# uma-pi1/kge

Measured on NVIDIA H100. Metric: triples scored/sec 1vsAll ComplEx d=512, higher is better.
Workload: dtype f32 (fp16 hi/lo split products hi*hi + hi*lo + lo*hi on wgmma, fp32 accumulate)

## Files before the change

kge_b200/csrc/capi.cu:

```cuda
#include <cstdarg>
#include <cstdio>
#include <cstring>
#include <cstdlib>
#include "fold.cuh"
#include "tc_common.cuh"

namespace b200kge {

static thread_local char g_err[512] = "";
static thread_local int64_t g_launches = 0;

void set_error(const char* fmt, ...) {
  va_list ap;
  va_start(ap, fmt);
  vsnprintf(g_err, sizeof(g_err), fmt, ap);
  va_end(ap);
}
void count_launch(int n) { g_launches += n; }

int check_cuda(cudaError_t e, const char* what) {
  if (e == cudaSuccess) return 0;
  if (e == cudaErrorMemoryAllocation)
    set_error("CUDA out of memory (%s)", what);
  else
    set_error("CUDA error %d (%s) at %s", (int)e, cudaGetErrorString(e), what);
  return B200KGE_ERR_CUDA;
}

static thread_local int g_prof_on = 0;
static thread_local cudaEvent_t g_ev0 = nullptr, g_ev1 = nullptr;
static thread_local int g_prof_valid = 0;

void profile_begin(cudaStream_t st) {
  if (!g_prof_on) return;
  if (!g_ev0) { cudaEventCreate(&g_ev0); cudaEventCreate(&g_ev1); }
  cudaEventRecord(g_ev0, st);
}
void profile_end(cudaStream_t st) {
  if (!g_prof_on || !g_ev0) return;
  cudaEventRecord(g_ev1, st);
  g_prof_valid = 1;
}

namespace {

struct Arena {
  uint8_t* base;
  size_t cap, off;
  void* take(size_t bytes) {
    size_t a = (off + 255) & ~size_t(255);
    if (a + bytes > cap) return nullptr;
    off = a + bytes;
    return base + a;
  }
};

inline int64_t round_up(int64_t x, int64_t m) { return (x + m - 1) / m * m; }

int validate_model(int model, const Rows& ent_like, const Rows& rel_like) {
  if (model < 0 || model > B200KGE_ROTATE) { set_error("unknown model %d", model); return B200KGE_ERR_INVALID; }
  const int D = ent_like.dim;
  if (D <= 0) { set_error("entity dim must be positive"); return B200KGE_ERR_INVALID; }
  if ((model == B200KGE_COMPLEX || model == B200KGE_SIMPLE || model == B200KGE_CP || model == B200KGE_ROTATE) && (D & 1)) {
    set_error("model %d requires embeddings of even dimensionality (got %d)", model, D);
    return B200KGE_ERR_INVALID;
  }
  const int want = relation_dim(model, D);
  if (rel_like.dim != want) {
    set_error("relation dim %d does not match model %d with entity dim %d (expected %d)", rel_like.dim, model, D, want);
    return B200KGE_ERR_INVALID;
  }
  return 0;
}

int validate_norm(int model, float l_norm) {
  if ((model == B200KGE_TRANSE || model == B200KGE_ROTATE) && !(l_norm > 0.f && l_norm < 1e30f)) {
    set_error("l_norm must be a positive finite number (got %g)", (double)l_norm);
    return B200KGE_ERR_INVALID;
  }
  return 0;
}

int check_tables(int model, float l_norm, const b200kge_rows_t* ent, const b200kge_rows_t* rel) {
  if (!ent || !rel) { set_error("null operand"); return B200KGE_ERR_INVALID; }
  if (ent->idx || rel->idx) { set_error("ent/rel must be plain tables (idx == NULL)"); return B200KGE_ERR_INVALID; }
  int rc = validate_model(model, to_rows(ent), to_rows(rel));
  return rc ? rc : validate_norm(model, l_norm);
}

int check_loss_kind(int loss_kind) {
  if (loss_kind != B200KGE_LOSS_BCE && loss_kind != B200KGE_LOSS_KL) { set_error("unknown loss kind %d", loss_kind); return B200KGE_ERR_INVALID; }
  return 0;
}

int check_grad_ld(const b200kge_rows_t* ent, int64_t lde, const b200kge_rows_t* rel, int64_t ldr) {
  if (lde < ent->dim || ldr < rel->dim) { set_error("gradient leading dimensions are smaller than the table widths"); return B200KGE_ERR_INVALID; }
  return 0;
}

EpiParams empty_epi() {
  EpiParams P;
  memset(&P, 0, sizeof(P));
  return P;
}

bool take_planes(Arena& ws, SplitSet& S) {
  S.hi = ws.take((size_t)S.rows * S.Kp * 2);
  S.lo = ws.take((size_t)S.rows * S.Kp * 2);
  S.inv_scale = (float*)ws.take((size_t)S.rows_pad * 4);
  return S.hi && S.lo && S.inv_scale;
}
size_t planes_bytes(int64_t rows, int64_t rows_pad, int64_t Kp) {
  return 2 * ((size_t)rows * Kp * 2 + 256) + (size_t)rows_pad * 4 + 256;
}

int gemm_planes(const SplitSet& A, const SplitSet& B, float* C, int64_t ldc, cudaStream_t st) {
  EpiParams P = empty_epi();
  P.out = C; P.ldo = ldc;
  if (A.Kp > 512) {
    P.accumulate_out = 1;
    cudaError_t e = cudaMemset2DAsync(C, (size_t)ldc * 4, 0, (size_t)B.rows * 4, (size_t)A.rows, st);
    if (e != cudaSuccess) return check_cuda(e, "cudaMemset2DAsync(gemm output)");
  }
  return launch_pairwise_tc3(EPI_STORE, A, B, P, st);
}

struct Block {
  int model, combine;
  const Rows* q0; const Rows* q1;
  const Rows* p;
  const Rows* cand;
  int64_t n;
  const float* Qpre = nullptr;
  bool same_fold = false;
};

int fold_block(const Block& B, int64_t ldq, Arena& ws, cudaStream_t st, const float** Q) {
  *Q = B.Qpre;
  if (*Q) return 0;
  const int64_t n = B.n;
  float* Qw = (float*)ws.take((size_t)(B.q1 ? 2 * n : n) * ldq * 4);
  if (!Qw) { set_error("workspace too small for folded queries"); return B200KGE_ERR_WORKSPACE; }
  int rc = launch_fold_queries(B.model, B.combine, *B.q0, *B.p, n, 0, Qw, ldq, st);
  if (rc) return rc;
  if (B.q1 && (rc = launch_fold_queries(B.model, B.same_fold ? B.combine : 1 - B.combine, *B.q1, *B.p, n, n, Qw, ldq, st)))
    return rc;
  *Q = Qw;
  return 0;
}

int take_partials(int epi_kind, int64_t nq, int nch, EpiParams& P, Arena& ws, int* nchunks_out, float** part_out) {
  const int loss_epi = epi_loss_base(epi_kind);
  if (loss_epi == EPI_BCE || loss_epi == EPI_KL) {
    const int F = (loss_epi == EPI_BCE) ? 2 : 5;
    P.part = (float*)ws.take((size_t)nq * nch * F * 4);
    if (!P.part) { set_error("workspace too small for loss partials"); return B200KGE_ERR_WORKSPACE; }
    if (part_out) *part_out = P.part;
  }
  P.nchunks = nch;
  if (nchunks_out) *nchunks_out = nch;
  return 0;
}

int run_block(const Block& B, float l_norm, int precision, int epi_kind, EpiParams P, Arena& ws,
              cudaStream_t st, int* nchunks_out, float** part_out = nullptr) {
  const int64_t n = B.n, nq = B.q1 ? 2 * n : n, m = B.cand->rows;
  const int D = B.q0->dim;
  Folded f0 = folded_problem(B.model, B.combine, D, l_norm);
  Folded f1 = f0;
  if (B.q1 && !B.same_fold) f1 = folded_problem(B.model, 1 - B.combine, D, l_norm);
  const bool cols_differ = B.q1 && (f0.col_off != f1.col_off);
  const int K = f0.K;
  const int64_t ldq = round_up(K, 32);

  int tc_kind = 0;
  if (f0.pair_op == PAIR_DOT && precision != B200KGE_PREC_FP32 && !cols_differ) {
    if (precision == B200KGE_PREC_AUTO) {
      if (K >= 32 && K <= 1024 && n >= 16 && m < (1ll << 31)) tc_kind = 3;
    } else if (precision == B200KGE_PREC_F16X3) {
      if (K < 16 || m >= (1ll << 31)) { set_error("the pre-split tensor-core path needs K >= 16"); return B200KGE_ERR_UNSUPPORTED; }
      tc_kind = 3;
    } else {
      if (!tc_supported(f0.pair_op, K, *B.cand, f0.col_off)) { set_error("tensor-core path needs K>=32, 16-byte aligned tables with ld%%4==0"); return B200KGE_ERR_UNSUPPORTED; }
      tc_kind = 1;
    }
  } else if (precision != B200KGE_PREC_AUTO && precision != B200KGE_PREC_FP32) {
    if (f0.pair_op != PAIR_DOT) { set_error("tensor-core precision modes apply to dot-product scorers only"); return B200KGE_ERR_UNSUPPORTED; }
  }

  if (epi_kind == EPI_RANK_EVAL) {
    if (B.cand->idx || tc_kind == 1) {
      set_error("the evaluation ranking runs on the pre-split tensor-core or the CUDA-core kernel over a plain table");
      return B200KGE_ERR_UNSUPPORTED;
    }
  } else if (P.csr_off && (cols_differ || B.cand->idx || tc_kind == 1 || (tc_kind == 0 && epi_kind != EPI_RANK))) {
    set_error("this CSR side input is not consumed by the kernel serving this call (losses: pre-split tensor-core path; "
              "rank: that path or the CUDA-core kernel; plain candidate table)");
    return B200KGE_ERR_UNSUPPORTED;
  }

  if (cols_differ) {
    Block h0 = B; h0.q1 = nullptr;
    Block h1 = B; h1.q0 = B.q1; h1.q1 = nullptr; h1.combine = 1 - B.combine;
    EpiParams P0 = P, P1 = P;
    P0.n_rows_out = 0; P1.n_rows_out = 0;
    if (epi_kind == EPI_STORE) { P1.out = P.out + P.col_block; }
    else if (epi_kind == EPI_RANK_EVAL) {
      P1.true_score += n; P1.csr_skip += n; P1.csr_off += n; P1.own_score += n; P1.rank += n; P1.ties += n;
      if (P1.csr2_off) P1.csr2_off += n;
    }
    else { set_error("stacked fused epilogues are not available for CP"); return B200KGE_ERR_UNSUPPORTED; }
    int rc = run_block(h0, l_norm, precision, epi_kind, P0, ws, st, nchunks_out);
    if (rc) return rc;
    return run_block(h1, l_norm, precision, epi_kind, P1, ws, st, nchunks_out);
  }

  const float* Q = nullptr;
  int rc = fold_block(B, ldq, ws, st, &Q);
  if (rc) return rc;
  if (tc_kind == 3) {
    const int Kp = (int)round_up(K, 64);
    SplitSet SQ{Q, ldq, nullptr, 0, nq, nq, K, Kp, nullptr, nullptr, nullptr};
    SplitSet ST{B.cand->base, B.cand->ld, B.cand->idx, f0.col_off, m, m + 32, K, Kp, nullptr, nullptr, nullptr};
    if (!take_planes(ws, SQ) || !take_planes(ws, ST)) {
      set_error("workspace too small for the pre-split operand planes");
      return B200KGE_ERR_WORKSPACE;
    }
    if ((rc = take_partials(epi_kind, nq, tc_nchunks(nq, m), P, ws, nchunks_out, part_out))) return rc;
    if ((rc = launch_presplit(ST, SQ, st))) return rc;
    return launch_pairwise_tc3(epi_kind, SQ, ST, P, st);
  }
  if (tc_kind == 1) {
    const int passes = (precision == B200KGE_PREC_TF32) ? 1 : (precision == B200KGE_PREC_3XTF32 ? 3 : 2);
    const float* T = B.cand->base + f0.col_off;
    int64_t ldt = B.cand->ld;
    if (B.cand->idx) {
      float* G = (float*)ws.take((size_t)m * ldq * 4);
      if (!G) { set_error("workspace too small to gather the candidate subset"); return B200KGE_ERR_WORKSPACE; }
      if ((rc = launch_gather_rows(*B.cand, f0.col_off, K, G, ldq, st))) return rc;
      T = G; ldt = ldq;
    }
    if ((rc = take_partials(epi_kind, nq, tc_nchunks(nq, m), P, ws, nchunks_out, part_out))) return rc;
    return launch_pairwise_tc(epi_kind, passes, Q, ldq, nq, T, ldt, m, K, P, st);
  }
  if ((rc = take_partials(epi_kind, nq, pairwise_simt_nchunks(nq, m), P, ws, nchunks_out, part_out))) return rc;
  return launch_pairwise_simt(epi_kind, f0.pair_op, l_norm, Q, ldq, nq, *B.cand, f0.col_off, K, P, st);
}

int check_1vsN_args(int model, int combine, const b200kge_rows_t* q, const b200kge_rows_t* p,
                    const b200kge_rows_t* cand, int64_t n) {
  if (!q || !p || !cand) { set_error("null operand"); return B200KGE_ERR_INVALID; }
  if (combine != B200KGE_SP_ && combine != B200KGE__PO) {
    set_error("cannot handle combine=%d", combine);
    return B200KGE_ERR_INVALID;
  }
  if (n < 0 || q->rows < n || p->rows < n) { set_error("operand has fewer than n=%lld rows", (long long)n); return B200KGE_ERR_INVALID; }
  if (cand->dim != q->dim) { set_error("candidate dim %d != query entity dim %d", cand->dim, q->dim); return B200KGE_ERR_INVALID; }
  return validate_model(model, to_rows(q), to_rows(p));
}

__global__ void unpack_triples_kernel(const int64_t* __restrict__ tri, int64_t n, int64_t* s, int64_t* p,
                                      int64_t* o, int64_t* labels2n) {
  int64_t i = blockIdx.x * (int64_t)blockDim.x + threadIdx.x;
  if (i < n) {
    const int64_t a = tri[3 * i], b = tri[3 * i + 1], c = tri[3 * i + 2];
    s[i] = a; p[i] = b; o[i] = c;
    labels2n[i] = c;
    labels2n[n + i] = a;
  }
}

int unpack_triples(const int64_t* triples, int64_t n, int64_t* sidx, int64_t* pidx, int64_t* oidx, int64_t* lab,
                   const Rows& E, const Rows& R, Rows& S, Rows& O, Rows& P, cudaStream_t st) {
  unpack_triples_kernel<<<(unsigned)((n + 255) / 256), 256, 0, st>>>(triples, n, sidx, pidx, oidx, lab);
  B2K_LAUNCH_CHECK("unpack_triples_kernel");
  S = E; S.idx = sidx; S.rows = n;
  O = E; O.idx = oidx; O.rows = n;
  P = R; P.idx = pidx; P.rows = n;
  return 0;
}

__global__ void pack_triples_kernel(const int64_t* __restrict__ q, const int64_t* __restrict__ p, int64_t n, int combine,
                                    int64_t* __restrict__ tri) {
  const int64_t i = blockIdx.x * (int64_t)blockDim.x + threadIdx.x;
  if (i >= n) return;
  tri[3 * i + 1] = p[i];
  tri[3 * i + (combine == B200KGE_SP_ ? 0 : 2)] = q[i];
  tri[3 * i + (combine == B200KGE_SP_ ? 2 : 0)] = 0;
}

__global__ void offset_index_kernel(const int64_t* __restrict__ idx, int64_t n, int64_t off, int64_t* __restrict__ out) {
  const int64_t i = blockIdx.x * (int64_t)blockDim.x + threadIdx.x;
  if (i < n) out[i] = idx[i] + off;
}

int check_reciprocal(const b200kge_rows_t* rel, int64_t num_rel) {
  if (num_rel <= 0 || rel->rows != 2 * num_rel) {
    set_error("reciprocal relations need rel->rows == 2 * num_relations (got %lld rows, num_relations %lld)",
              (long long)rel->rows, (long long)num_rel);
    return B200KGE_ERR_INVALID;
  }
  return 0;
}

__global__ void __launch_bounds__(128)
shard_gather_rows_kernel(Rows shard, int64_t lo, const int64_t* __restrict__ idx, float* __restrict__ out, int64_t ldo) {
  const int64_t i = blockIdx.x;
  const int64_t g = idx[i] - lo;
  const bool mine = g >= 0 && g < shard.rows;
  const float* __restrict__ src = shard.base + (mine ? g : 0) * shard.ld;
  float* __restrict__ dst = out + i * ldo;
  for (int k = threadIdx.x; k < shard.dim; k += blockDim.x) dst[k] = mine ? src[k] : 0.f;
}

}
}

using namespace b200kge;

extern "C" {

int b200kge_version(void) { return B200KGE_VERSION; }
const char* b200kge_last_error(void) { return g_err; }
int64_t b200kge_launch_count(int reset) {
  int64_t v = g_launches;
  if (reset) g_launches = 0;
  return v;
}

int b200kge_profile_enable(int on) { g_prof_on = on; g_prof_valid = 0; return 0; }
int b200kge_profile_last_ms(float* ms) {
  if (!ms) { set_error("null operand"); return B200KGE_ERR_INVALID; }
  if (!g_prof_valid) { set_error("no profiled kernel yet"); return B200KGE_ERR_INVALID; }
  B2K_CUDA(cudaEventSynchronize(g_ev1));
  B2K_CUDA(cudaEventElapsedTime(ms, g_ev0, g_ev1));
  return 0;
}

int b200kge_device_ok(void) {
  int dev = 0, major = 0, minor = 0;
  if (cudaGetDevice(&dev) != cudaSuccess ||
      cudaDeviceGetAttribute(&major, cudaDevAttrComputeCapabilityMajor, dev) != cudaSuccess ||
      cudaDeviceGetAttribute(&minor, cudaDevAttrComputeCapabilityMinor, dev) != cudaSuccess) {
    cudaGetLastError();
    set_error("no CUDA device available: libb200kge has no CPU fallback");
    return B200KGE_ERR_NO_DEVICE;
  }
  if (major != 9 || minor != 0) {
    set_error("device compute capability %d.%d is not sm_90 (H100)", major, minor);
    return B200KGE_ERR_NO_DEVICE;
  }
  return 0;
}

size_t b200kge_workspace_bytes(int model, int64_t n, int64_t m, int32_t D, int cand_has_idx) {
  (void)model;
  const int64_t ldq = round_up(D, 32);
  const int64_t nq = 2 * n;
  size_t b = 0;
  b += 2 * ((size_t)nq * ldq * 4 + 256);
  if (cand_has_idx) b += (size_t)m * ldq * 4 + 256;
  int64_t nch = pairwise_simt_nchunks(nq, m);
  if (nch < 320) nch = 320;
  b += (size_t)nq * nch * 5 * 4 + 256;
  b += (size_t)n * 3 * 8 + (size_t)n * 5 * 8 + 4096;
  {
    const int64_t Kp = round_up(D, 64);
    b += 2 * ((size_t)nq * Kp * 2 + 256) + 2 * ((size_t)m * Kp * 2 + 256) + (size_t)(nq + m + 32) * 4 + 512;
  }
  return b + 4096;
}

int b200kge_score_spo(int model, float l_norm, const b200kge_rows_t* s, const b200kge_rows_t* p,
                      const b200kge_rows_t* o, int64_t n, float* out, b200kge_stream_t stream) {
  if (!s || !p || !o || (!out && n > 0)) { set_error("null operand"); return B200KGE_ERR_INVALID; }
  int rc = validate_model(model, to_rows(s), to_rows(p)); if (rc) return rc;
  if ((rc = validate_norm(model, l_norm))) return rc;
  if (s->rows < n || p->rows < n || o->rows < n) { set_error("operand has fewer than n rows"); return B200KGE_ERR_INVALID; }
  return launch_spo(model, l_norm, to_rows(s), to_rows(p), to_rows(o), n, out, 1, (cudaStream_t)stream);
}

int b200kge_score_1vsN(int model, int combine, float l_norm, int precision,
                       const b200kge_rows_t* q, const b200kge_rows_t* p,
                       const b200kge_rows_t* cand, int64_t n, float* out, int64_t ldo,
                       void* workspace, size_t workspace_bytes, b200kge_stream_t stream) {
  int rc = check_1vsN_args(model, combine, q, p, cand, n); if (rc) return rc;
  if ((rc = validate_norm(model, l_norm))) return rc;
  Rows Q = to_rows(q), Pr = to_rows(p), C = to_rows(cand);
  Arena ws{(uint8_t*)workspace, workspace_bytes, 0};
  EpiParams P = empty_epi();
  P.out = out; P.ldo = ldo;
  Block B{model, combine, &Q, nullptr, &Pr, &C, n};
  return run_block(B, l_norm, precision, EPI_STORE, P, ws, (cudaStream_t)stream, nullptr);
}

int b200kge_score_sp_po(int model, float l_norm, int precision, const b200kge_rows_t* s,
                        const b200kge_rows_t* p, const b200kge_rows_t* o,
                        const b200kge_rows_t* cand, int64_t n, float* out, int64_t ldo,
                        void* workspace, size_t workspace_bytes, b200kge_stream_t stream) {
  int rc = check_1vsN_args(model, B200KGE_SP_, s, p, cand, n); if (rc) return rc;
  if ((rc = check_1vsN_args(model, B200KGE__PO, o, p, cand, n))) return rc;
  if ((rc = validate_norm(model, l_norm))) return rc;
  Rows Sr = to_rows(s), Pr = to_rows(p), Or = to_rows(o), C = to_rows(cand);
  Arena ws{(uint8_t*)workspace, workspace_bytes, 0};
  EpiParams P = empty_epi();
  P.out = out; P.ldo = ldo; P.n_rows_out = n; P.col_block = cand->rows;
  Block B{model, B200KGE_SP_, &Sr, &Or, &Pr, &C, n};
  return run_block(B, l_norm, precision, EPI_STORE, P, ws, (cudaStream_t)stream, nullptr);
}

int b200kge_score_sp_po_bcast(int model, float l_norm, int precision, const b200kge_rows_t* s,
                              const b200kge_rows_t* p, const b200kge_rows_t* o, const b200kge_rows_t* cand,
                              int64_t n, float* out, float* const* peer_out, int n_peers, int64_t ldo,
                              int64_t col_block, void* workspace, size_t workspace_bytes,
                              b200kge_stream_t stream) {
  int rc = check_1vsN_args(model, B200KGE_SP_, s, p, cand, n); if (rc) return rc;
  if ((rc = check_1vsN_args(model, B200KGE__PO, o, p, cand, n))) return rc;
  if ((rc = validate_norm(model, l_norm))) return rc;
  if (n_peers < 0 || n_peers > 7 || (n_peers > 0 && !peer_out)) { set_error("0..7 peer buffers"); return B200KGE_ERR_INVALID; }
  if (col_block < cand->rows) { set_error("col_block smaller than the number of candidates"); return B200KGE_ERR_INVALID; }
  Rows Sr = to_rows(s), Pr = to_rows(p), Or = to_rows(o), C = to_rows(cand);
  Arena ws{(uint8_t*)workspace, workspace_bytes, 0};
  EpiParams P = empty_epi();
  P.out = out; P.ldo = ldo; P.n_rows_out = n; P.col_block = col_block;
  P.n_peers = n_peers;
  for (int g = 0; g < n_peers; ++g) P.out_peer[g] = peer_out[g];
  if (model == B200KGE_CP) { set_error("the broadcast store is not offered for CP"); return B200KGE_ERR_UNSUPPORTED; }
  Block B{model, B200KGE_SP_, &Sr, &Or, &Pr, &C, n};
  return run_block(B, l_norm, precision, EPI_STORE, P, ws, (cudaStream_t)stream, nullptr);
}

int b200kge_score_1vsN_loss(int model, int combine, float l_norm, int precision,
                            const b200kge_rows_t* q, const b200kge_rows_t* p,
                            const b200kge_rows_t* cand, int64_t n, const b200kge_labels_t* labels,
                            int loss_kind, float offset, float* loss_out, float* row_loss_out,
                            void* workspace, size_t workspace_bytes, b200kge_stream_t stream) {
  int rc = check_1vsN_args(model, combine, q, p, cand, n); if (rc) return rc;
  if ((rc = validate_norm(model, l_norm))) return rc;
  if (!labels || (!labels->idx) == (!labels->dense)) { set_error("exactly one of labels.idx / labels.dense must be given"); return B200KGE_ERR_INVALID; }
  if ((rc = check_loss_kind(loss_kind))) return rc;
  if (!loss_out) { set_error("loss_out is null"); return B200KGE_ERR_INVALID; }
  cudaStream_t st = (cudaStream_t)stream;
  Rows Q = to_rows(q), Pr = to_rows(p), C = to_rows(cand);
  Arena ws{(uint8_t*)workspace, workspace_bytes, 0};
  EpiParams P = empty_epi();
  P.label_idx = labels->idx; P.label_dense = labels->dense; P.ldl = labels->ldl;
  P.offset = (loss_kind == B200KGE_LOSS_BCE) ? offset : 0.f;
  Block B{model, combine, &Q, nullptr, &Pr, &C, n};
  int nch = 0;
  const int epi = (loss_kind == B200KGE_LOSS_BCE) ? EPI_BCE : EPI_KL;
  float* part = nullptr;
  rc = run_block(B, l_norm, precision, epi, P, ws, st, &nch, &part);
  if (rc) return rc;
  if (n == 0 || C.rows == 0) { B2K_CUDA(cudaMemsetAsync(loss_out, 0, 4, st)); return 0; }
  void* scratch = ws.take(1024);
  if (!scratch) { set_error("workspace too small"); return B200KGE_ERR_WORKSPACE; }
  return launch_loss_finalize(loss_kind, part, nch, n, loss_out, row_loss_out, 1.0f, 0, scratch, 0, st);
}

int b200kge_score_1vsN_rank(int model, int combine, float l_norm, int precision,
                            const b200kge_rows_t* q, const b200kge_rows_t* p,
                            const b200kge_rows_t* cand, int64_t n, const float* true_score,
                            const float* filter, int64_t ldf, float rtol, float atol,
                            int64_t* rank, int64_t* ties, void* workspace, size_t workspace_bytes,
                            b200kge_stream_t stream) {
  int rc = check_1vsN_args(model, combine, q, p, cand, n); if (rc) return rc;
  if ((rc = validate_norm(model, l_norm))) return rc;
  if (!true_score || !rank || !ties) { set_error("null rank operand"); return B200KGE_ERR_INVALID; }
  Rows Q = to_rows(q), Pr = to_rows(p), C = to_rows(cand);
  Arena ws{(uint8_t*)workspace, workspace_bytes, 0};
  EpiParams P = empty_epi();
  P.true_score = true_score; P.filter = filter; P.ldf = ldf; P.rtol = rtol; P.atol = atol;
  P.rank = reinterpret_cast<unsigned long long*>(rank);
  P.ties = reinterpret_cast<unsigned long long*>(ties);
  Block B{model, combine, &Q, nullptr, &Pr, &C, n};
  return run_block(B, l_norm, precision, EPI_RANK, P, ws, (cudaStream_t)stream, nullptr);
}

int b200kge_rank_sp_po(int model, float l_norm, int precision, const b200kge_rows_t* s,
                       const b200kge_rows_t* p, const b200kge_rows_t* o, const b200kge_rows_t* cand,
                       int64_t n, const float* true_score, const float* filter, int64_t ldf, float rtol,
                       float atol, int64_t* rank, int64_t* ties, void* workspace, size_t workspace_bytes,
                       b200kge_stream_t stream) {
  int rc = check_1vsN_args(model, B200KGE_SP_, s, p, cand, n); if (rc) return rc;
  if ((rc = check_1vsN_args(model, B200KGE__PO, o, p, cand, n))) return rc;
  if ((rc = validate_norm(model, l_norm))) return rc;
  if (!true_score || !rank || !ties) { set_error("null rank operand"); return B200KGE_ERR_INVALID; }
  Rows Sr = to_rows(s), Pr = to_rows(p), Or = to_rows(o), C = to_rows(cand);
  Arena ws{(uint8_t*)workspace, workspace_bytes, 0};
  EpiParams P = empty_epi();
  P.true_score = true_score; P.filter = filter; P.ldf = ldf; P.rtol = rtol; P.atol = atol;
  P.rank = reinterpret_cast<unsigned long long*>(rank);
  P.ties = reinterpret_cast<unsigned long long*>(ties);
  Block B{model, B200KGE_SP_, &Sr, &Or, &Pr, &C, n};
  return run_block(B, l_norm, precision, EPI_RANK, P, ws, (cudaStream_t)stream, nullptr);
}

int b200kge_rank_sp_po_csr(int model, float l_norm, int precision, const b200kge_rows_t* s,
                           const b200kge_rows_t* p, const b200kge_rows_t* o, const b200kge_rows_t* cand,
                           int64_t n, const float* true_score, const int64_t* filter_off,
                           const int64_t* filter_col, const int64_t* own_col, float rtol, float atol,
                           int64_t* rank, int64_t* ties, void* workspace, size_t workspace_bytes,
                           b200kge_stream_t stream) {
  int rc = check_1vsN_args(model, B200KGE_SP_, s, p, cand, n); if (rc) return rc;
  if ((rc = check_1vsN_args(model, B200KGE__PO, o, p, cand, n))) return rc;
  if ((rc = validate_norm(model, l_norm))) return rc;
  if (!true_score || !rank || !ties || !filter_off) { set_error("null rank operand"); return B200KGE_ERR_INVALID; }
  Rows Sr = to_rows(s), Pr = to_rows(p), Or = to_rows(o), C = to_rows(cand);
  Arena ws{(uint8_t*)workspace, workspace_bytes, 0};
  EpiParams P = empty_epi();
  P.true_score = true_score; P.rtol = rtol; P.atol = atol;
  P.rank = reinterpret_cast<unsigned long long*>(rank);
  P.ties = reinterpret_cast<unsigned long long*>(ties);
  P.csr_off = filter_off; P.csr_col = filter_col; P.csr_skip = own_col;
  Block B{model, B200KGE_SP_, &Sr, &Or, &Pr, &C, n};
  return run_block(B, l_norm, precision, EPI_RANK, P, ws, (cudaStream_t)stream, nullptr);
}

int b200kge_rank_sp_po_eval(int model, float l_norm, int precision, const b200kge_rows_t* ent,
                            const b200kge_rows_t* rel, int64_t num_relations, const int64_t* s, const int64_t* p,
                            const int64_t* o, int64_t n, const float* true_score, const int64_t* own_col,
                            const int64_t* filter_off, const int64_t* filter_col, const int64_t* test_off,
                            const int64_t* test_col, float rtol, float atol, int64_t* rank, int64_t* ties,
                            float* own_score, void* workspace, size_t workspace_bytes, b200kge_stream_t stream) {
  if (!s || !p || !o || !true_score || !own_col || !filter_off || !rank || !ties || !own_score) {
    set_error("null rank operand");
    return B200KGE_ERR_INVALID;
  }
  if (n < 0) { set_error("negative batch size"); return B200KGE_ERR_INVALID; }
  if (num_relations < 0) { set_error("num_relations must be >= 0"); return B200KGE_ERR_INVALID; }
  int rc = check_tables(model, l_norm, ent, rel); if (rc) return rc;
  if (num_relations > 0 && (rc = check_reciprocal(rel, num_relations))) return rc;
  if (precision == B200KGE_PREC_TF32 || precision == B200KGE_PREC_3XTF32 || precision == B200KGE_PREC_TF32_BF16X2) {
    set_error("the evaluation ranking does not run the in-kernel split precision modes");
    return B200KGE_ERR_UNSUPPORTED;
  }
  if (n == 0) return 0;
  cudaStream_t st = (cudaStream_t)stream;
  const Rows E = to_rows(ent), R = to_rows(rel);
  Rows S = E, O = E, Pr = R;
  S.idx = s; S.rows = n; O.idx = o; O.rows = n; Pr.idx = p; Pr.rows = n;
  Arena ws{(uint8_t*)workspace, workspace_bytes, 0};
  EpiParams P = empty_epi();
  P.true_score = true_score; P.rtol = rtol; P.atol = atol;
  P.rank = reinterpret_cast<unsigned long long*>(rank);
  P.ties = reinterpret_cast<unsigned long long*>(ties);
  P.csr_off = filter_off; P.csr_col = filter_col; P.csr_skip = own_col;
  P.csr2_off = test_off; P.csr2_col = test_col;
  P.rank_ld = 2 * n; P.n_rank = test_off ? 3 : 2;
  P.own_score = own_score;
  Block B{model, B200KGE_SP_, &S, &O, &Pr, &E, n};
  if (num_relations > 0) {
    const Folded f = folded_problem(model, B200KGE_SP_, E.dim, l_norm);
    const int64_t ldq = round_up(f.K, 32);
    float* Q = (float*)ws.take((size_t)2 * n * ldq * 4);
    int64_t* p2 = (int64_t*)ws.take((size_t)n * 8);
    if (!Q || !p2) { set_error("workspace too small for folded queries"); return B200KGE_ERR_WORKSPACE; }
    offset_index_kernel<<<(unsigned)((n + 255) / 256), 256, 0, st>>>(p, n, num_relations, p2);
    B2K_LAUNCH_CHECK("offset_index_kernel");
    Rows P2 = R; P2.idx = p2; P2.rows = n;
    if ((rc = launch_fold_queries(model, B200KGE_SP_, S, Pr, n, 0, Q, ldq, st))) return rc;
    if ((rc = launch_fold_queries(model, B200KGE_SP_, O, P2, n, n, Q, ldq, st))) return rc;
    B.Qpre = Q;
    B.same_fold = true;
  }
  return run_block(B, l_norm, precision, EPI_RANK_EVAL, P, ws, st, nullptr);
}

int b200kge_shard_gather_rows(const b200kge_rows_t* shard, int64_t lo, const int64_t* idx, int64_t n,
                              float* out, int64_t ldo, b200kge_stream_t stream) {
  if (!shard || (!idx && n > 0) || (!out && n > 0)) { set_error("null operand"); return B200KGE_ERR_INVALID; }
  if (shard->idx) { set_error("shard must be a plain table (idx == NULL)"); return B200KGE_ERR_INVALID; }
  if (ldo < shard->dim) { set_error("output row stride smaller than the row width"); return B200KGE_ERR_INVALID; }
  if (n <= 0) return 0;
  shard_gather_rows_kernel<<<(unsigned)n, 128, 0, (cudaStream_t)stream>>>(to_rows(shard), lo, idx, out, ldo);
  B2K_LAUNCH_CHECK("shard_gather_rows_kernel");
  return 0;
}

int b200kge_loss_dense(const float* scores, int64_t lds, int64_t n, int64_t m,
                       const b200kge_labels_t* labels, int loss_kind, float offset,
                       float* loss_out, float* row_loss_out, void* workspace,
                       size_t workspace_bytes, b200kge_stream_t stream) {
  if (!scores || !labels || !loss_out) { set_error("null operand"); return B200KGE_ERR_INVALID; }
  if ((!labels->idx) == (!labels->dense)) { set_error("exactly one of labels.idx / labels.dense must be given"); return B200KGE_ERR_INVALID; }
  if (loss_kind >= B200KGE_LOSS_BCE_MEAN && loss_kind <= B200KGE_LOSS_SE) { set_error("loss kind %d is row-wise with one positive per row: use b200kge_ns_loss", loss_kind); return B200KGE_ERR_UNSUPPORTED; }
  int rc = check_loss_kind(loss_kind); if (rc) return rc;
  cudaStream_t st = (cudaStream_t)stream;
  if (n == 0 || m == 0) { B2K_CUDA(cudaMemsetAsync(loss_out, 0, 4, st)); return 0; }
  Arena ws{(uint8_t*)workspace, workspace_bytes, 0};
  const int nch = loss_dense_nchunks(m);
  const int F = (loss_kind == B200KGE_LOSS_BCE) ? 2 : 5;
  EpiParams P = empty_epi();
  P.label_idx = labels->idx; P.label_dense = labels->dense; P.ldl = labels->ldl;
  P.offset = (loss_kind == B200KGE_LOSS_BCE) ? offset : 0.f;
  P.nchunks = nch;
  P.part = (float*)ws.take((size_t)n * nch * F * 4);
  if (!P.part) { set_error("workspace too small for loss partials (need %zu bytes)", (size_t)n * nch * F * 4); return B200KGE_ERR_WORKSPACE; }
  void* scratch = ws.take(1024);
  if (!scratch) { set_error("workspace too small"); return B200KGE_ERR_WORKSPACE; }
  if ((rc = launch_loss_dense(loss_kind, scores, lds, n, m, P, st))) return rc;
  return launch_loss_finalize(loss_kind, P.part, nch, n, loss_out, row_loss_out, 1.0f, 0, scratch, 0, st);
}

int b200kge_rank_dense(const float* scores, int64_t lds, int64_t n, int64_t m,
                       const float* true_score, const float* filter, int64_t ldf, float rtol,
                       float atol, int64_t* rank, int64_t* ties, b200kge_stream_t stream) {
  if (!scores || !true_score || !rank || !ties) { set_error("null operand"); return B200KGE_ERR_INVALID; }
  EpiParams P = empty_epi();
  P.true_score = true_score; P.filter = filter; P.ldf = ldf; P.rtol = rtol; P.atol = atol;
  P.rank = reinterpret_cast<unsigned long long*>(rank);
  P.ties = reinterpret_cast<unsigned long long*>(ties);
  return launch_rank_dense(scores, lds, n, m, P, (cudaStream_t)stream);
}

int b200kge_ns_score(int model, float l_norm, const b200kge_rows_t* s, const b200kge_rows_t* p,
                     const b200kge_rows_t* o, const b200kge_rows_t* slot_table, int slot,
                     const int64_t* neg, int64_t n, int64_t K, int with_positive, float* out,
                     int64_t ldo, b200kge_stream_t stream) {
  if (n == 0 || (K == 0 && !with_positive)) return 0;
  if (!s || !p || !o || !slot_table || (!neg && n * K > 0) || !out) { set_error("null operand"); return B200KGE_ERR_INVALID; }
  if (slot < 0 || slot > 2) { set_error("slot must be 0 (S), 1 (P) or 2 (O)"); return B200KGE_ERR_INVALID; }
  int rc = validate_model(model, to_rows(s), to_rows(p)); if (rc) return rc;
  if ((rc = validate_norm(model, l_norm))) return rc;
  if (slot_table->idx) { set_error("slot_table must be a plain table (idx == NULL)"); return B200KGE_ERR_INVALID; }
  if (slot_table->dim != (slot == 1 ? p->dim : s->dim)) { set_error("slot_table width does not match the slot"); return B200KGE_ERR_INVALID; }
  cudaStream_t st = (cudaStream_t)stream;
  const int col0 = with_positive ? 1 : 0;
  if (with_positive) {
    rc = launch_spo(model, l_norm, to_rows(s), to_rows(p), to_rows(o), n, out, ldo, st);
    if (rc) return rc;
  }
  return launch_ns(model, l_norm, to_rows(s), to_rows(p), to_rows(o), to_rows(slot_table), slot, neg, n, K,
                   out, ldo, col0, st);
}

int b200kge_sample_uniform(uint64_t seed, uint64_t offset, int64_t vocab, int64_t n, int64_t K, int64_t* out,
                           b200kge_stream_t stream) {
  if (vocab <= 0) { set_error("vocabulary size must be positive"); return B200KGE_ERR_INVALID; }
  if (n < 0 || K < 0 || (!out && n * K > 0)) { set_error("null operand"); return B200KGE_ERR_INVALID; }
  return launch_sample_uniform(seed, offset, vocab, n * K, out, (cudaStream_t)stream);
}

static int train_1vsall_forward_impl(int model, float l_norm, int precision,
                                     const b200kge_rows_t* ent, const b200kge_rows_t* rel,
                                     const int64_t* triples, int64_t n, int loss_kind, float offset,
                                     float* loss_out, void* workspace, size_t workspace_bytes,
                                     b200kge_stream_t stream, int64_t num_rel) {
  if (!triples || !loss_out) { set_error("null operand"); return B200KGE_ERR_INVALID; }
  int rc = check_tables(model, l_norm, ent, rel); if (rc) return rc;
  if ((rc = check_loss_kind(loss_kind))) return rc;
  cudaStream_t st = (cudaStream_t)stream;
  if (n <= 0) { B2K_CUDA(cudaMemsetAsync(loss_out, 0, 4, st)); return 0; }
  Arena ws{(uint8_t*)workspace, workspace_bytes, 0};
  Rows E = to_rows(ent), R = to_rows(rel);
  const int epi = (loss_kind == B200KGE_LOSS_BCE) ? EPI_BCE : EPI_KL;
  const float scale = 1.0f / (float)n;
  Folded f0 = folded_problem(model, B200KGE_SP_, E.dim, l_norm),
         f1 = folded_problem(model, num_rel > 0 ? B200KGE_SP_ : B200KGE__PO, E.dim, l_norm);
  const int K = f0.K;
  const bool presplit = f0.col_off == f1.col_off && f0.pair_op == PAIR_DOT && (model != B200KGE_CP || num_rel > 0) &&
                        (precision == B200KGE_PREC_AUTO || precision == B200KGE_PREC_F16X3) && K >= 32 && K <= 1024 &&
                        n >= 16 && E.rows < (1ll << 31) &&
                        ((size_t)round_up(K, 64) + (model == B200KGE_RESCAL ? E.dim : 0)) * 4 <= 48 * 1024;
  if (presplit) {
    const int64_t nq = 2 * n, m = E.rows;
    const int Kp = (int)round_up(K, 64);
    SplitSet SQ{nullptr, 0, nullptr, 0, nq, nq, K, Kp, nullptr, nullptr, nullptr};
    SplitSet ST{E.base, E.ld, nullptr, f0.col_off, m, m + 32, K, Kp, nullptr, nullptr, nullptr};
    const bool planes = take_planes(ws, SQ) && take_planes(ws, ST);
    int64_t* lab = (int64_t*)ws.take((size_t)n * 2 * 8);
    uint8_t* scratch = (uint8_t*)ws.take(1024);
    const int nch = tc_nchunks(nq, m);
    const int F = (loss_kind == B200KGE_LOSS_BCE) ? 2 : 5;
    float* part = (float*)ws.take((size_t)nq * nch * F * 4);
    if (!planes || !lab || !scratch || !part) { set_error("workspace too small"); return B200KGE_ERR_WORKSPACE; }
    unsigned int* ticket = reinterpret_cast<unsigned int*>(scratch + 512);
    if ((rc = launch_prep_split_1vsall(model, E, R, triples, n, SQ, ST, lab, ticket, st, num_rel))) return rc;
    EpiParams P = empty_epi();
    P.label_idx = lab;
    P.offset = (loss_kind == B200KGE_LOSS_BCE) ? offset : 0.f;
    P.part = part; P.nchunks = nch;
    if ((rc = launch_pairwise_tc3(epi, SQ, ST, P, st))) return rc;
    return launch_loss_finalize(loss_kind, part, nch, nq, loss_out, nullptr, scale, 0, scratch, 1, st);
  }
  if (f0.col_off == f1.col_off) {
    const int64_t ldq = round_up(f0.K, 32);
    float* Q = (float*)ws.take((size_t)(2 * n) * ldq * 4);
    int64_t* lab = (int64_t*)ws.take((size_t)n * 2 * 8);
    uint8_t* scratch = (uint8_t*)ws.take(1024);
    if (!Q || !lab || !scratch) { set_error("workspace too small"); return B200KGE_ERR_WORKSPACE; }
    rc = launch_prep_1vsall(model, E, R, triples, n, Q, ldq, lab, reinterpret_cast<unsigned int*>(scratch + 512), st,
                            num_rel);
    if (rc) return rc;
    Rows S = E; S.idx = lab; S.rows = n;
    Rows Pr = R; Pr.idx = lab; Pr.rows = n;
    EpiParams P = empty_epi();
    P.label_idx = lab;
    P.offset = (loss_kind == B200KGE_LOSS_BCE) ? offset : 0.f;
    Block B{model, B200KGE_SP_, &S, &S, &Pr, &E, n};
    B.Qpre = Q;
    B.same_fold = num_rel > 0;
    int nch = 0;
    float* part = nullptr;
    rc = run_block(B, l_norm, precision, epi, P, ws, st, &nch, &part);
    if (rc) return rc;
    return launch_loss_finalize(loss_kind, part, nch, 2 * n, loss_out, nullptr, scale, 0, scratch, 1, st);
  }
  int64_t* sidx = (int64_t*)ws.take((size_t)n * 8);
  int64_t* pidx = (int64_t*)ws.take((size_t)n * 8);
  int64_t* oidx = (int64_t*)ws.take((size_t)n * 8);
  int64_t* lab = (int64_t*)ws.take((size_t)n * 2 * 8);
  if (!sidx || !pidx || !oidx || !lab) { set_error("workspace too small"); return B200KGE_ERR_WORKSPACE; }
  Rows S, O, Pr;
  if ((rc = unpack_triples(triples, n, sidx, pidx, oidx, lab, E, R, S, O, Pr, st))) return rc;
  EpiParams P = empty_epi();
  P.label_idx = lab;
  P.offset = (loss_kind == B200KGE_LOSS_BCE) ? offset : 0.f;
  for (int dir = 0; dir < 2; ++dir) {
    Arena w2 = ws;
    EpiParams Pd = P;
    Pd.label_idx = lab + dir * n;
    Block B{model, dir, dir == 0 ? &S : &O, nullptr, &Pr, &E, n};
    int nch = 0;
    float* part = nullptr;
    rc = run_block(B, l_norm, precision, epi, Pd, w2, st, &nch, &part);
    if (rc) return rc;
    void* scratch = w2.take(1024);
    if (!scratch) { set_error("workspace too small"); return B200KGE_ERR_WORKSPACE; }
    rc = launch_loss_finalize(loss_kind, part, nch, n, loss_out, nullptr, scale, dir, scratch, 0, st);
    if (rc) return rc;
  }
  return 0;
}

int b200kge_train_1vsall_forward(int model, float l_norm, int precision,
                                 const b200kge_rows_t* ent, const b200kge_rows_t* rel,
                                 const int64_t* triples, int64_t n, int loss_kind, float offset,
                                 float* loss_out, void* workspace, size_t workspace_bytes,
                                 b200kge_stream_t stream) {
  return train_1vsall_forward_impl(model, l_norm, precision, ent, rel, triples, n, loss_kind, offset, loss_out,
                                   workspace, workspace_bytes, stream, 0);
}

int b200kge_train_1vsall_forward_host(int model, float l_norm, int precision,
                                      const b200kge_rows_t* ent, const b200kge_rows_t* rel,
                                      const int64_t* triples_host, int64_t n, int loss_kind,
                                      float offset, float* loss_host, void* workspace,
                                      size_t workspace_bytes, b200kge_stream_t stream) {
  if (!triples_host || !loss_host) { set_error("null operand"); return B200KGE_ERR_INVALID; }
  if (n <= 0) { *loss_host = 0.f; return 0; }
  cudaStream_t st = (cudaStream_t)stream;
  Arena ws{(uint8_t*)workspace, workspace_bytes, 0};
  int64_t* tri = (int64_t*)ws.take((size_t)n * 3 * 8);
  float* loss_dev = (float*)ws.take(256);
  if (!tri || !loss_dev) { set_error("workspace too small"); return B200KGE_ERR_WORKSPACE; }
  B2K_CUDA(cudaMemcpyAsync(tri, triples_host, (size_t)n * 3 * 8, cudaMemcpyHostToDevice, st));
  size_t used = (ws.off + 255) & ~size_t(255);
  int rc = b200kge_train_1vsall_forward(model, l_norm, precision, ent, rel, tri, n, loss_kind, offset, loss_dev,
                                        ws.base + used, workspace_bytes - used, stream);
  if (rc) return rc;
  B2K_CUDA(cudaMemcpyAsync(loss_host, loss_dev, 4, cudaMemcpyDeviceToHost, st));
  B2K_CUDA(cudaStreamSynchronize(st));
  return 0;
}

}

namespace {

struct GradSpec {
  const int64_t* lab = nullptr;
  int loss_kind = B200KGE_LOSS_BCE;
  float offset = 0.f;
  const int64_t* csr_off = nullptr;
  const int64_t* csr_col = nullptr;
  float csr_a = 1.f, csr_b = 0.f, inv_batch = 0.f;
  const float* G = nullptr;
  int64_t ldg = 0;
};

GradSpec csr_grad(const int64_t* q_idx, const int64_t* csr_off, const int64_t* csr_col, float label_smoothing, int64_t m,
                  int64_t batch_size, int loss_kind, float offset) {
  GradSpec g;
  g.lab = q_idx;
  g.loss_kind = loss_kind; g.offset = offset;
  g.csr_off = csr_off; g.csr_col = csr_col;
  g.csr_a = 1.0f - label_smoothing; g.csr_b = label_smoothing > 0.f ? 1.0f / (float)m : 0.f;
  g.inv_batch = 1.0f / (float)batch_size;
  return g;
}

int backward_block(int model, const Rows& E, const Rows& R, int64_t n, int dir, bool same_fold, const float* Q,
                   int64_t ldq, int col_off, int K, const GradSpec& g, float* d_ent, int64_t lde, float* dQ, Arena ws,
                   cudaStream_t st) {
  const int64_t nq = dir < 0 ? 2 * n : n, m = E.rows;
  const int64_t ldz = round_up(m, 4), Ep = round_up(m, 64), Np = round_up(nq, 64);
  const int64_t ldE = round_up(m, 4), ldN = round_up(nq, 4);
  int rc;
  SplitSet SG{nullptr, 0, nullptr, 0, nq, nq, (int)m, (int)Ep, nullptr, nullptr, nullptr};
  SplitSet SGT{nullptr, 0, nullptr, 0, m, m, (int)nq, (int)Np, nullptr, nullptr, nullptr};
  if (g.G) {
    float* Gt = (float*)ws.take((size_t)m * ldN * 4);
    if (!Gt) { set_error("workspace too small for the transposed gradient"); return B200KGE_ERR_WORKSPACE; }
    if ((rc = launch_transpose(g.G, g.ldg, nq, m, Gt, ldN, st))) return rc;
    SG.src = g.G; SG.ld = g.ldg;
    SGT.src = Gt; SGT.ld = ldN;
    if (!take_planes(ws, SG) || !take_planes(ws, SGT)) { set_error("workspace too small for the gradient planes"); return B200KGE_ERR_WORKSPACE; }
    if ((rc = launch_presplit(SGT, SG, st))) return rc;
  } else {
    float* z = (float*)ws.take((size_t)nq * ldz * 4);
    if (!z) { set_error("workspace too small for the score matrix"); return B200KGE_ERR_WORKSPACE; }
    {
      Rows S = E; S.idx = g.lab; S.rows = n;
      Rows Pr = R; Pr.idx = g.lab; Pr.rows = n;
      EpiParams P = empty_epi();
      P.out = z; P.ldo = ldz;
      Block B{model, dir <= 0 ? B200KGE_SP_ : B200KGE__PO, &S, dir < 0 ? &S : nullptr, &Pr, &E, n};
      B.Qpre = Q;
      B.same_fold = same_fold;
      if ((rc = run_block(B, 1.0f, B200KGE_PREC_AUTO, EPI_STORE, P, ws, st, nullptr))) return rc;
    }
    if (!take_planes(ws, SG) || !take_planes(ws, SGT)) { set_error("workspace too small for the gradient planes"); return B200KGE_ERR_WORKSPACE; }
    float* row_stat = nullptr;
    if (g.loss_kind == B200KGE_LOSS_KL) {
      row_stat = (float*)ws.take((size_t)nq * 2 * 4);
      if (!row_stat) { set_error("workspace too small for the row statistics"); return B200KGE_ERR_WORKSPACE; }
    }
    const float off = g.loss_kind == B200KGE_LOSS_KL ? 0.f : g.offset;
    if (g.csr_off)
      rc = launch_grad_planes_csr(z, ldz, nq, m, g.csr_off, g.csr_col, g.csr_a, g.csr_b, row_stat, off, g.inv_batch,
                                  SG.hi, SG.lo, Ep, SGT.hi, SGT.lo, Np, SG.inv_scale, SGT.inv_scale, st);
    else
      rc = launch_grad_planes(z, ldz, nq, m, g.lab, nullptr, 0, row_stat, off, 1.0f / (float)n, SG.hi, SG.lo, Ep,
                              SGT.hi, SGT.lo, Np, SG.inv_scale, SGT.inv_scale, st);
    if (rc) return rc;
  }
  float* Tt = (float*)ws.take((size_t)K * ldE * 4);
  float* Qt = (float*)ws.take((size_t)K * ldN * 4);
  if (!Tt || !Qt) { set_error("workspace too small for the transposed operands"); return B200KGE_ERR_WORKSPACE; }
  if ((rc = launch_transpose(E.base + col_off, E.ld, m, K, Tt, ldE, st))) return rc;
  if ((rc = launch_transpose(Q, ldq, nq, K, Qt, ldN, st))) return rc;
  SplitSet STt{Tt, ldE, nullptr, 0, K, K + 32, (int)m, (int)Ep, nullptr, nullptr, nullptr};
  SplitSet SQt{Qt, ldN, nullptr, 0, K, K + 32, (int)nq, (int)Np, nullptr, nullptr, nullptr};
  if (!take_planes(ws, STt) || !take_planes(ws, SQt)) { set_error("workspace too small for the operand planes"); return B200KGE_ERR_WORKSPACE; }
  if ((rc = launch_presplit(STt, SQt, st))) return rc;
  if ((rc = gemm_planes(SGT, SQt, d_ent + col_off, lde, st))) return rc;
  return gemm_planes(SG, STt, dQ, ldq, st);
}

int distance_rowgrads(int pair_op, const float* Q, int64_t ldq, int64_t nq, const Rows& T, int K, const float* W,
                      int64_t ldw, float* Wt, float* dQ, float* dT, int64_t ldt, cudaStream_t st) {
  const int64_t m = T.rows, ldN = round_up(nq, 4);
  int rc;
  if ((rc = launch_transpose(W, ldw, nq, m, Wt, ldN, st))) return rc;
  if ((rc = launch_pair_rowgrad(pair_op, Q, ldq, nq, T.base, T.ld, m, K, Wt, ldN, dQ, ldq, st))) return rc;
  return launch_pair_rowgrad(pair_op, T.base, T.ld, m, Q, ldq, nq, K, W, ldw, dT, ldt, st);
}

int distance_backward(const Block& B, float l_norm, const GradSpec& g, float* dQ, float* dT, int64_t ldt, Arena& ws,
                      cudaStream_t st) {
  const Folded f = folded_problem(B.model, B.combine, B.cand->dim, l_norm);
  const int64_t nq = B.q1 ? 2 * B.n : B.n, m = B.cand->rows, ldz = round_up(m, 4), ldN = round_up(nq, 4);
  const bool kl = g.loss_kind == B200KGE_LOSS_KL;
  float* z = (float*)ws.take((size_t)nq * ldz * 4);
  float* G = (float*)ws.take((size_t)nq * ldz * 4);
  float* Gt = (float*)ws.take((size_t)m * ldN * 4);
  float* row_stat = kl ? (float*)ws.take((size_t)nq * 2 * 4) : nullptr;
  if (!z || !G || !Gt || (kl && !row_stat)) { set_error("workspace too small"); return B200KGE_ERR_WORKSPACE; }
  EpiParams P = empty_epi();
  P.out = z; P.ldo = ldz;
  int rc;
  if ((rc = run_block(B, l_norm, B200KGE_PREC_AUTO, EPI_STORE, P, ws, st, nullptr))) return rc;
  const int64_t* lab = g.csr_off ? nullptr : g.lab;
  if (kl && (rc = launch_row_lse(z, ldz, nq, m, lab, row_stat, st))) return rc;
  if (g.csr_off)
    rc = launch_grad_csr(z, ldz, nq, m, g.csr_off, g.csr_col, g.csr_a, g.csr_b, row_stat, kl ? 0.f : g.offset,
                         g.inv_batch, f.pair_op == PAIR_L2, G, ldz, st);
  else
    rc = launch_grad_dense(z, ldz, nq, m, g.lab, row_stat, kl ? 0.f : g.offset, 1.0f / (float)B.n,
                           f.pair_op == PAIR_L2, G, ldz, st);
  if (rc) return rc;
  return distance_rowgrads(f.pair_op, B.Qpre, round_up(f.K, 32), nq, *B.cand, f.K, G, ldz, Gt, dQ, dT, ldt, st);
}

int check_distance_pair(int pair_op) {
  if (pair_op != PAIR_L1 && pair_op != PAIR_L2 && pair_op != PAIR_CMOD_L1) {
    set_error("the distance-family backward covers l_norm 1 and 2 (TransE) and 1 (RotatE)");
    return B200KGE_ERR_UNSUPPORTED;
  }
  return 0;
}

size_t backward_block_bytes(int64_t nq, int64_t m, int64_t K, int64_t ldq) {
  const int64_t Ep = round_up(m, 64), Np = round_up(nq, 64);
  size_t b = (size_t)nq * round_up(m, 4) * 4 + 256;
  b += b200kge_workspace_bytes(0, nq, m, (int32_t)K, 0);
  b += planes_bytes(nq, nq, Ep) + planes_bytes(m, m, Np);
  b += (size_t)K * round_up(m, 4) * 4 + (size_t)K * round_up(nq, 4) * 4 + 2 * (size_t)nq * ldq * 4 + (size_t)nq * 8 + 5 * 256;
  b += planes_bytes(K, K + 32, Ep) + planes_bytes(K, K + 32, Np);
  return b;
}

}

extern "C" {

size_t b200kge_gemm_nt_workspace_bytes(int64_t M, int64_t N, int64_t K) {
  const int64_t Kp = round_up(K, 64);
  return planes_bytes(M, M, Kp) + planes_bytes(N, N + 32, Kp) + 1024;
}

int b200kge_gemm_nt(const float* A, int64_t lda, const float* B, int64_t ldb, int64_t M, int64_t N, int64_t K,
                      float* C, int64_t ldc, void* workspace, size_t workspace_bytes, b200kge_stream_t stream) {
  if (!A || !B || !C) { set_error("null operand"); return B200KGE_ERR_INVALID; }
  if (M < 0 || N < 0 || K <= 0 || N >= (1ll << 31)) { set_error("bad GEMM shape"); return B200KGE_ERR_INVALID; }
  if (M == 0 || N == 0) return 0;
  cudaStream_t st = (cudaStream_t)stream;
  Arena ws{(uint8_t*)workspace, workspace_bytes, 0};
  const int Kp = (int)round_up(K, 64);
  SplitSet SA{A, lda, nullptr, 0, M, M, (int)K, Kp, nullptr, nullptr, nullptr};
  SplitSet SB{B, ldb, nullptr, 0, N, N + 32, (int)K, Kp, nullptr, nullptr, nullptr};
  if (!take_planes(ws, SA) || !take_planes(ws, SB)) { set_error("workspace too small for the operand planes"); return B200KGE_ERR_WORKSPACE; }
  int rc = launch_presplit(SB, SA, st);
  if (rc) return rc;
  return gemm_planes(SA, SB, C, ldc, st);
}

size_t b200kge_train_1vsall_backward_workspace_bytes(int model, int64_t n, int64_t E, int32_t D) {
  const int64_t K = (model == B200KGE_CP) ? D / 2 : D;
  const int64_t nq = 2 * n, ldq = round_up(K, 32);
  if (model == B200KGE_TRANSE || model == B200KGE_ROTATE)
    return 2 * (size_t)nq * ldq * 4 + (size_t)nq * 8 + 2 * (size_t)nq * round_up(E, 4) * 4 + 2 * (size_t)E * round_up(nq, 4) * 4 +
           (size_t)nq * 8 + 16 * 256 + b200kge_workspace_bytes(model, n, E, D, 0);
  return (size_t)nq * ldq * 4 + (size_t)n * 5 * 8 + 4096 + backward_block_bytes(nq, E, K, ldq);
}

static int train_1vsall_backward_impl(int model, float l_norm, const b200kge_rows_t* ent, const b200kge_rows_t* rel,
                                      const int64_t* triples, int64_t n, int loss_kind, float offset, float* d_ent,
                                      int64_t lde, float* d_rel, int64_t ldr, void* workspace, size_t workspace_bytes,
                                      b200kge_stream_t stream, int64_t num_rel) {
  if (!triples || !d_ent || !d_rel) { set_error("null operand"); return B200KGE_ERR_INVALID; }
  int rc = check_tables(model, l_norm, ent, rel); if (rc) return rc;
  if ((rc = check_loss_kind(loss_kind))) return rc;
  if ((rc = check_grad_ld(ent, lde, rel, ldr))) return rc;
  cudaStream_t st = (cudaStream_t)stream;
  Rows E = to_rows(ent), R = to_rows(rel);
  B2K_CUDA(cudaMemsetAsync(d_rel, 0, (size_t)R.rows * ldr * 4, st));
  if (n <= 0) { B2K_CUDA(cudaMemsetAsync(d_ent, 0, (size_t)E.rows * lde * 4, st)); return 0; }
  Arena ws{(uint8_t*)workspace, workspace_bytes, 0};
  if (model == B200KGE_TRANSE || model == B200KGE_ROTATE) {
    Folded f = folded_problem(model, B200KGE_SP_, E.dim, l_norm);
    if ((rc = check_distance_pair(f.pair_op))) return rc;
    const int64_t nq = 2 * n, ldq = round_up(f.K, 32);
    float* Q = (float*)ws.take((size_t)nq * ldq * 4);
    float* dQ = (float*)ws.take((size_t)nq * ldq * 4);
    int64_t* lab = (int64_t*)ws.take((size_t)nq * 8);
    if (!Q || !dQ || !lab) { set_error("workspace too small"); return B200KGE_ERR_WORKSPACE; }
    if ((rc = launch_prep_1vsall(model, E, R, triples, n, Q, ldq, lab, nullptr, st, num_rel))) return rc;
    Rows S = E; S.idx = lab; S.rows = n;
    Rows Pr = R; Pr.idx = lab; Pr.rows = n;
    Block B{model, B200KGE_SP_, &S, &S, &Pr, &E, n};
    B.Qpre = Q;
    B.same_fold = num_rel > 0;
    GradSpec g;
    g.lab = lab; g.loss_kind = loss_kind; g.offset = offset;
    if ((rc = distance_backward(B, l_norm, g, dQ, d_ent, lde, ws, st))) return rc;
    return launch_unfold_distance(model, E, R, triples, n, -1, dQ, ldq, d_ent, lde, d_rel, ldr, st, num_rel);
  }
  Folded f0 = folded_problem(model, B200KGE_SP_, E.dim, 1.0f),
         f1 = folded_problem(model, num_rel > 0 ? B200KGE_SP_ : B200KGE__PO, E.dim, 1.0f);
  const int64_t ldq = round_up(f0.K, 32);
  GradSpec g;
  g.loss_kind = loss_kind; g.offset = offset;
  if (f0.col_off == f1.col_off) {
    float* Q = (float*)ws.take((size_t)(2 * n) * ldq * 4);
    int64_t* lab = (int64_t*)ws.take((size_t)n * 2 * 8);
    if (!Q || !lab) { set_error("workspace too small"); return B200KGE_ERR_WORKSPACE; }
    float* dQ = (float*)ws.take((size_t)(2 * n) * ldq * 4);
    if (!dQ) { set_error("workspace too small"); return B200KGE_ERR_WORKSPACE; }
    if ((rc = launch_prep_1vsall(model, E, R, triples, n, Q, ldq, lab, nullptr, st, num_rel))) return rc;
    if (f0.col_off > 0) B2K_CUDA(cudaMemset2DAsync(d_ent, (size_t)lde * 4, 0, (size_t)f0.col_off * 4, (size_t)E.rows, st));
    g.lab = lab;
    if ((rc = backward_block(model, E, R, n, -1, num_rel > 0, Q, ldq, f0.col_off, f0.K, g, d_ent, lde, dQ, ws, st))) return rc;
    return launch_unfold(model, E, R, triples, n, -1, dQ, ldq, d_ent, lde, d_rel, ldr, st, num_rel);
  }
  int64_t* sidx = (int64_t*)ws.take((size_t)n * 8);
  int64_t* pidx = (int64_t*)ws.take((size_t)n * 8);
  int64_t* oidx = (int64_t*)ws.take((size_t)n * 8);
  int64_t* lab = (int64_t*)ws.take((size_t)n * 2 * 8);
  float* Q = (float*)ws.take((size_t)n * ldq * 4);
  float* dQ2 = (float*)ws.take((size_t)(2 * n) * ldq * 4);
  if (!sidx || !pidx || !oidx || !lab || !Q || !dQ2) { set_error("workspace too small"); return B200KGE_ERR_WORKSPACE; }
  Rows S, O, Pr;
  if ((rc = unpack_triples(triples, n, sidx, pidx, oidx, lab, E, R, S, O, Pr, st))) return rc;
  for (int dir = 0; dir < 2; ++dir) {
    const Folded& f = dir == 0 ? f0 : f1;
    if ((rc = launch_fold_queries(model, dir, dir == 0 ? S : O, Pr, n, 0, Q, ldq, st))) return rc;
    g.lab = lab + dir * n;
    if ((rc = backward_block(model, E, R, n, dir, false, Q, ldq, f.col_off, f.K, g, d_ent, lde,
                             dQ2 + (size_t)dir * n * ldq, ws, st))) return rc;
  }
  for (int dir = 0; dir < 2; ++dir)
    if ((rc = launch_unfold(model, E, R, triples, n, dir, dQ2 + (size_t)dir * n * ldq, ldq, d_ent, lde, d_rel, ldr, st))) return rc;
  return 0;
}

int b200kge_train_1vsall_backward(int model, float l_norm, const b200kge_rows_t* ent, const b200kge_rows_t* rel,
                                    const int64_t* triples, int64_t n, int loss_kind, float offset, float* d_ent,
                                    int64_t lde, float* d_rel, int64_t ldr, void* workspace, size_t workspace_bytes,
                                    b200kge_stream_t stream) {
  return train_1vsall_backward_impl(model, l_norm, ent, rel, triples, n, loss_kind, offset, d_ent, lde, d_rel, ldr,
                                    workspace, workspace_bytes, stream, 0);
}


size_t b200kge_score_1vsN_backward_workspace_bytes(int model, int64_t n, int64_t E, int32_t D) {
  const int64_t K = (model == B200KGE_CP) ? D / 2 : D;
  const int64_t ldq = round_up(K, 32);
  if (model == B200KGE_TRANSE || model == B200KGE_ROTATE)
    return 2 * (size_t)n * ldq * 4 + (size_t)n * 4 * 8 + 2 * (size_t)n * round_up(E, 4) * 4 + (size_t)E * round_up(n, 4) * 4 +
           16 * 256 + b200kge_workspace_bytes(model, n, E, D, 0);
  return 2 * (size_t)n * ldq * 4 + (size_t)n * 4 * 8 + (size_t)E * round_up(n, 4) * 4 + 8192 + backward_block_bytes(n, E, K, ldq);
}

int b200kge_score_1vsN_backward(int model, int combine, float l_norm, const b200kge_rows_t* ent, const b200kge_rows_t* rel,
                                const int64_t* q_idx, const int64_t* p_idx, int64_t n, const float* grad_scores,
                                int64_t ldg, float* d_ent, int64_t lde, float* d_rel, int64_t ldr, void* workspace,
                                size_t workspace_bytes, b200kge_stream_t stream) {
  if (!q_idx || !p_idx || !grad_scores || !d_ent || !d_rel) { set_error("null operand"); return B200KGE_ERR_INVALID; }
  if (combine != B200KGE_SP_ && combine != B200KGE__PO) { set_error("cannot handle combine=%d", combine); return B200KGE_ERR_INVALID; }
  int rc = check_tables(model, l_norm, ent, rel); if (rc) return rc;
  if ((rc = check_grad_ld(ent, lde, rel, ldr))) return rc;
  if (ldg < ent->rows) { set_error("grad_scores is narrower than the entity table"); return B200KGE_ERR_INVALID; }
  const bool distance = (model == B200KGE_TRANSE || model == B200KGE_ROTATE);
  cudaStream_t st = (cudaStream_t)stream;
  Rows E = to_rows(ent), R = to_rows(rel);
  Folded f = folded_problem(model, combine, E.dim, l_norm);
  if (distance && (rc = check_distance_pair(f.pair_op))) return rc;
  B2K_CUDA(cudaMemsetAsync(d_rel, 0, (size_t)R.rows * ldr * 4, st));
  B2K_CUDA(cudaMemsetAsync(d_ent, 0, (size_t)E.rows * lde * 4, st));
  if (n <= 0) return 0;
  Arena ws{(uint8_t*)workspace, workspace_bytes, 0};
  const int64_t ldq = round_up(f.K, 32);
  float* Q = (float*)ws.take((size_t)n * ldq * 4);
  float* dQ = (float*)ws.take((size_t)n * ldq * 4);
  int64_t* tri = (int64_t*)ws.take((size_t)n * 3 * 8);
  if (!Q || !dQ || !tri) { set_error("workspace too small"); return B200KGE_ERR_WORKSPACE; }
  pack_triples_kernel<<<(unsigned)((n + 255) / 256), 256, 0, st>>>(q_idx, p_idx, n, combine, tri);
  B2K_LAUNCH_CHECK("pack_triples_kernel");
  Rows A = E; A.idx = q_idx; A.rows = n;
  Rows Pr = R; Pr.idx = p_idx; Pr.rows = n;
  if ((rc = launch_fold_queries(model, combine, A, Pr, n, 0, Q, ldq, st))) return rc;
  if (distance) {
    const int64_t m = E.rows, ldz = round_up(m, 4), ldN = round_up(n, 4);
    const float* W = grad_scores;
    int64_t ldw = ldg;
    if (f.pair_op == PAIR_L2) {
      float* z = (float*)ws.take((size_t)n * ldz * 4);
      float* Wd = (float*)ws.take((size_t)n * ldz * 4);
      if (!z || !Wd) { set_error("workspace too small"); return B200KGE_ERR_WORKSPACE; }
      EpiParams P = empty_epi();
      P.out = z; P.ldo = ldz;
      Block B{model, combine, &A, nullptr, &Pr, &E, n};
      B.Qpre = Q;
      if ((rc = run_block(B, l_norm, B200KGE_PREC_AUTO, EPI_STORE, P, ws, st, nullptr))) return rc;
      if ((rc = launch_div_scores(grad_scores, ldg, z, ldz, n, m, Wd, ldz, st))) return rc;
      W = Wd; ldw = ldz;
    }
    float* Wt = (float*)ws.take((size_t)m * ldN * 4);
    if (!Wt) { set_error("workspace too small"); return B200KGE_ERR_WORKSPACE; }
    if ((rc = distance_rowgrads(f.pair_op, Q, ldq, n, E, f.K, W, ldw, Wt, dQ, d_ent, lde, st))) return rc;
    return launch_unfold_distance(model, E, R, tri, n, combine, dQ, ldq, d_ent, lde, d_rel, ldr, st);
  }
  GradSpec g;
  g.G = grad_scores; g.ldg = ldg;
  if ((rc = backward_block(model, E, R, n, combine, false, Q, ldq, f.col_off, f.K, g, d_ent, lde, dQ, ws, st))) return rc;
  return launch_unfold(model, E, R, tri, n, combine, dQ, ldq, d_ent, lde, d_rel, ldr, st);
}

int b200kge_score_1vsN_loss_csr_backward_norm(int model, int combine, float l_norm, const b200kge_rows_t* ent,
                                              const b200kge_rows_t* rel, const int64_t* q_idx, const int64_t* p_idx,
                                              int64_t n, const int64_t* csr_off, const int64_t* csr_col,
                                              float label_smoothing, int loss_kind, float offset, int64_t batch_size,
                                              float* d_ent, int64_t lde, float* d_rel, int64_t ldr, void* workspace,
                                              size_t workspace_bytes, b200kge_stream_t stream) {
  if (!q_idx || !p_idx || !csr_off || !d_ent || !d_rel) { set_error("null operand"); return B200KGE_ERR_INVALID; }
  if (combine != B200KGE_SP_ && combine != B200KGE__PO) { set_error("cannot handle combine=%d", combine); return B200KGE_ERR_INVALID; }
  int rc = check_tables(model, l_norm, ent, rel); if (rc) return rc;
  const bool distance = (model == B200KGE_TRANSE || model == B200KGE_ROTATE);
  Folded f = folded_problem(model, combine, ent->dim, distance ? l_norm : 1.0f);
  if (distance && (rc = check_distance_pair(f.pair_op))) return rc;
  if ((rc = check_loss_kind(loss_kind))) return rc;
  if (batch_size <= 0 || !(label_smoothing >= 0.f && label_smoothing < 1.f)) { set_error("bad batch_size / label_smoothing"); return B200KGE_ERR_INVALID; }
  if ((rc = check_grad_ld(ent, lde, rel, ldr))) return rc;
  cudaStream_t st = (cudaStream_t)stream;
  Rows E = to_rows(ent), R = to_rows(rel);
  B2K_CUDA(cudaMemsetAsync(d_rel, 0, (size_t)R.rows * ldr * 4, st));
  B2K_CUDA(cudaMemsetAsync(d_ent, 0, (size_t)E.rows * lde * 4, st));
  if (n <= 0) return 0;
  Arena ws{(uint8_t*)workspace, workspace_bytes, 0};
  const int64_t ldq = round_up(f.K, 32);
  float* Q = (float*)ws.take((size_t)n * ldq * 4);
  float* dQ = (float*)ws.take((size_t)n * ldq * 4);
  int64_t* tri = (int64_t*)ws.take((size_t)n * 3 * 8);
  if (!Q || !dQ || !tri) { set_error("workspace too small"); return B200KGE_ERR_WORKSPACE; }
  pack_triples_kernel<<<(unsigned)((n + 255) / 256), 256, 0, st>>>(q_idx, p_idx, n, combine, tri);
  B2K_LAUNCH_CHECK("pack_triples_kernel");
  Rows A = E; A.idx = q_idx; A.rows = n;
  Rows Pr = R; Pr.idx = p_idx; Pr.rows = n;
  if ((rc = launch_fold_queries(model, combine, A, Pr, n, 0, Q, ldq, st))) return rc;
  const GradSpec g = csr_grad(q_idx, csr_off, csr_col, label_smoothing, E.rows, batch_size, loss_kind, offset);
  if (distance) {
    Block B{model, combine, &A, nullptr, &Pr, &E, n};
    B.Qpre = Q;
    if ((rc = distance_backward(B, l_norm, g, dQ, d_ent, lde, ws, st))) return rc;
    return launch_unfold_distance(model, E, R, tri, n, combine, dQ, ldq, d_ent, lde, d_rel, ldr, st);
  }
  if ((rc = backward_block(model, E, R, n, combine, false, Q, ldq, f.col_off, f.K, g, d_ent, lde, dQ, ws, st))) return rc;
  return launch_unfold(model, E, R, tri, n, combine, dQ, ldq, d_ent, lde, d_rel, ldr, st);
}

int b200kge_score_1vsN_loss_csr_backward(int model, int combine, const b200kge_rows_t* ent, const b200kge_rows_t* rel,
                                         const int64_t* q_idx, const int64_t* p_idx, int64_t n, const int64_t* csr_off,
                                         const int64_t* csr_col, float label_smoothing, int loss_kind, float offset,
                                         int64_t batch_size, float* d_ent, int64_t lde, float* d_rel, int64_t ldr,
                                         void* workspace, size_t workspace_bytes, b200kge_stream_t stream) {
  return b200kge_score_1vsN_loss_csr_backward_norm(model, combine, 1.0f, ent, rel, q_idx, p_idx, n, csr_off, csr_col,
                                                   label_smoothing, loss_kind, offset, batch_size, d_ent, lde, d_rel,
                                                   ldr, workspace, workspace_bytes, stream);
}

int b200kge_lookup_penalty(const b200kge_rows_t* rows, const float* counts, float p, int complex_abs, float scale,
                             float* out, void* workspace, size_t workspace_bytes, b200kge_stream_t stream) {
  if (!rows || !out) { set_error("null operand"); return B200KGE_ERR_INVALID; }
  if (!(p > 0.f)) { set_error("p must be positive (got %g)", (double)p); return B200KGE_ERR_INVALID; }
  if (complex_abs && (rows->dim & 1)) { set_error("complex-space penalty needs an even embedding width"); return B200KGE_ERR_INVALID; }
  return launch_penalty(to_rows(rows), counts, p, complex_abs, scale, (float*)workspace, workspace_bytes / 4, out,
                        (cudaStream_t)stream);
}

int b200kge_normalize_rows(float* weight, int64_t ld, int64_t rows, int32_t dim, float p, b200kge_stream_t stream) {
  if (!weight && rows > 0) { set_error("null operand"); return B200KGE_ERR_INVALID; }
  return launch_normalize_rows(weight, ld, rows, dim, p, (cudaStream_t)stream);
}


int b200kge_ns_backward(int model, float l_norm, const b200kge_rows_t* ent, const b200kge_rows_t* rel,
                          const int64_t* triples, int slot, const int64_t* neg, int64_t n, int64_t K, float offset,
                          int64_t batch_size, float* d_ent, int64_t lde, float* d_rel, int64_t ldr, void* workspace,
                          size_t workspace_bytes, b200kge_stream_t stream) {
  if (!triples || (!neg && n * K > 0) || !d_ent || !d_rel) { set_error("null operand"); return B200KGE_ERR_INVALID; }
  int rc = check_tables(model, l_norm, ent, rel); if (rc) return rc;
  if (batch_size <= 0) { set_error("batch_size must be positive"); return B200KGE_ERR_INVALID; }
  if ((rc = check_grad_ld(ent, lde, rel, ldr))) return rc;
  Rows E = to_rows(ent), R = to_rows(rel);
  Folded f = folded_problem(model, B200KGE_SP_, E.dim, l_norm);
  const int64_t ldq = round_up(f.K, 32);
  Arena ws{(uint8_t*)workspace, workspace_bytes, 0};
  float* dQ = (float*)ws.take((size_t)n * ldq * 4);
  if (!dQ && n > 0) { set_error("workspace too small (need n * round_up(K,32) floats)"); return B200KGE_ERR_WORKSPACE; }
  return launch_ns_backward(model, l_norm, E, R, triples, slot, neg, n, K, offset, 1.0f / (float)batch_size, nullptr, 0,
                            d_ent, lde, d_rel, ldr, dQ, ldq, (cudaStream_t)stream);
}

int b200kge_ns_backward_grad(int model, float l_norm, const b200kge_rows_t* ent, const b200kge_rows_t* rel,
                             const int64_t* triples, int slot, const int64_t* neg, int64_t n, int64_t K,
                             const float* grad_scores, int64_t ldg, float* d_ent, int64_t lde, float* d_rel,
                             int64_t ldr, void* workspace, size_t workspace_bytes, b200kge_stream_t stream) {
  if (!triples || (!neg && n * K > 0) || (!grad_scores && n > 0) || !d_ent || !d_rel) { set_error("null operand"); return B200KGE_ERR_INVALID; }
  int rc = check_tables(model, l_norm, ent, rel); if (rc) return rc;
  if (ldg < K + 1) { set_error("grad_scores is narrower than the 1 + K columns of the block"); return B200KGE_ERR_INVALID; }
  if ((rc = check_grad_ld(ent, lde, rel, ldr))) return rc;
  Rows E = to_rows(ent), R = to_rows(rel);
  Folded f = folded_problem(model, B200KGE_SP_, E.dim, l_norm);
  const int64_t ldq = round_up(f.K, 32);
  Arena ws{(uint8_t*)workspace, workspace_bytes, 0};
  float* dQ = (float*)ws.take((size_t)n * ldq * 4);
  if (!dQ && n > 0) { set_error("workspace too small (need n * round_up(K,32) floats)"); return B200KGE_ERR_WORKSPACE; }
  return launch_ns_backward(model, l_norm, E, R, triples, slot, neg, n, K, 0.f, 1.f, grad_scores, ldg, d_ent, lde,
                            d_rel, ldr, dQ, ldq, (cudaStream_t)stream);
}

size_t b200kge_ns_loss_workspace_bytes(int64_t n) { return (size_t)n * 2 * 4 + 256 + 1024; }

int b200kge_ns_loss(const float* scores, int64_t lds, int64_t n, int64_t m, const int64_t* label_idx,
                    int loss_kind, float arg, float temperature, float scale, float* loss_out,
                    float* row_loss_out, float* grad_out, int64_t ldg, void* workspace,
                    size_t workspace_bytes, b200kge_stream_t stream) {
  if ((!scores && n * m > 0) || !loss_out) { set_error("null operand"); return B200KGE_ERR_INVALID; }
  if (loss_kind < B200KGE_LOSS_BCE || loss_kind > B200KGE_LOSS_SE) { set_error("unknown loss kind %d", loss_kind); return B200KGE_ERR_INVALID; }
  if (n > 0 && m < (loss_kind >= B200KGE_LOSS_BCE_MEAN && loss_kind <= B200KGE_LOSS_MARGIN_RANKING ? 2 : 1)) {
    set_error("loss kind %d needs a positive and at least one negative per row (m = %lld)", loss_kind, (long long)m);
    return B200KGE_ERR_INVALID;
  }
  if (lds < m || (grad_out && ldg < m)) { set_error("row stride smaller than the row width"); return B200KGE_ERR_INVALID; }
  cudaStream_t st = (cudaStream_t)stream;
  if (n == 0) { B2K_CUDA(cudaMemsetAsync(loss_out, 0, 4, st)); return 0; }
  Arena ws{(uint8_t*)workspace, workspace_bytes, 0};
  float* part = (float*)ws.take((size_t)n * 2 * 4);
  void* scratch = ws.take(1024);
  if (!part || !scratch) { set_error("workspace too small (need b200kge_ns_loss_workspace_bytes(n) = %zu bytes)", b200kge_ns_loss_workspace_bytes(n)); return B200KGE_ERR_WORKSPACE; }
  int rc = launch_ns_loss(loss_kind, scores, lds, n, m, label_idx, arg, temperature, scale, part, grad_out, ldg, st);
  if (rc) return rc;
  return launch_loss_finalize(B200KGE_LOSS_BCE, part, 1, n, loss_out, row_loss_out, scale, 0, scratch, 0, st);
}


size_t b200kge_score_1vsN_loss_csr_workspace_bytes(int model, int64_t n, int64_t m, int32_t D, int64_t nnz) {
  const int64_t ldq = round_up(D, 32), tot = nnz + n;
  size_t b = b200kge_workspace_bytes(model, n, m, D, 0);
  b += (size_t)n * 8 + 3 * ((size_t)tot * 8 + 256) + (size_t)tot * 4 + 4 * ((size_t)n * 4 + 256) + 2048;
  b += (size_t)n * ldq * 4 + ((size_t)((m + 1023) / 1024) + 1) * ldq * 4 + 512;
  if (model == B200KGE_TRANSE || model == B200KGE_ROTATE)
    b += (size_t)n * pairwise_simt_nchunks(n, m) * 4 + 256;
  return b;
}

int b200kge_score_1vsN_loss_csr(int model, int combine, float l_norm, int precision, const b200kge_rows_t* q,
                                  const b200kge_rows_t* p, const b200kge_rows_t* cand, int64_t n,
                                  const int64_t* csr_off, const int64_t* csr_col, int64_t nnz, float label_smoothing,
                                  int loss_kind, float offset, float* loss_out, float* row_loss_out, void* workspace,
                                  size_t workspace_bytes, b200kge_stream_t stream) {
  int rc = check_1vsN_args(model, combine, q, p, cand, n); if (rc) return rc;
  if ((rc = validate_norm(model, l_norm))) return rc;
  if (!csr_off || (!csr_col && nnz > 0) || !loss_out || nnz < 0) { set_error("null operand"); return B200KGE_ERR_INVALID; }
  if (cand->idx) { set_error("CSR labels address the columns of a plain candidate table (cand.idx must be NULL)"); return B200KGE_ERR_INVALID; }
  if ((rc = check_loss_kind(loss_kind))) return rc;
  if (!(label_smoothing >= 0.f && label_smoothing < 1.f)) { set_error("label_smoothing must be in [0, 1)"); return B200KGE_ERR_INVALID; }
  const bool dot = model <= B200KGE_RESCAL;
  cudaStream_t st = (cudaStream_t)stream;
  if (n == 0 || cand->rows == 0) { B2K_CUDA(cudaMemsetAsync(loss_out, 0, 4, st)); return 0; }
  Rows Q = to_rows(q), Pr = to_rows(p), C = to_rows(cand);
  const int64_t m = C.rows, tot = nnz + (loss_kind == B200KGE_LOSS_KL ? n : 0);
  Arena ws{(uint8_t*)workspace, workspace_bytes, 0};
  int64_t* lab = (int64_t*)ws.take((size_t)n * 8);
  int64_t* qsel = (int64_t*)ws.take((size_t)tot * 8 + 8);
  int64_t* psel = (int64_t*)ws.take((size_t)tot * 8 + 8);
  int64_t* esel = (int64_t*)ws.take((size_t)tot * 8 + 8);
  float* zpos = (float*)ws.take((size_t)tot * 4 + 8);
  float* fused = (float*)ws.take((size_t)n * 4);
  float* rows = row_loss_out ? row_loss_out : (float*)ws.take((size_t)n * 4);
  float* total = (float*)ws.take(256);
  void* scratch = ws.take(1024);
  const bool zsum_fused = label_smoothing > 0.f && !dot;
  const int zch = zsum_fused ? pairwise_simt_nchunks(n, m) : 1;
  float* zsum = zsum_fused ? (float*)ws.take((size_t)n * zch * 4) : nullptr;
  if (!lab || !qsel || !psel || !esel || !zpos || !fused || !rows || !total || !scratch || (zsum_fused && !zsum)) { set_error("workspace too small"); return B200KGE_ERR_WORKSPACE; }
  B2K_CUDA(cudaMemsetAsync(lab, loss_kind == B200KGE_LOSS_BCE ? 0xFF : 0, (size_t)n * 8, st));
  bool emitted = false;
  {
    const int epi = (loss_kind == B200KGE_LOSS_BCE) ? (zsum_fused ? EPI_BCE_ZSUM : EPI_BCE)
                                                    : (zsum_fused ? EPI_KL_ZSUM : EPI_KL);
    for (int attempt = 0; attempt < 2; ++attempt) {
      EpiParams P = empty_epi();
      P.label_idx = lab;
      P.offset = (loss_kind == B200KGE_LOSS_BCE) ? offset : 0.f;
      P.zsum_part = zsum;
      if (attempt == 0) {
        P.csr_off = csr_off; P.csr_col = csr_col; P.csr_out = zpos; P.csr_nnz = nnz;
        P.csr_extra = (loss_kind == B200KGE_LOSS_KL) ? 1 : 0;
      }
      Block B{model, combine, &Q, nullptr, &Pr, &C, n};
      int nch = 0;
      float* part = nullptr;
      Arena w2 = ws;
      rc = run_block(B, l_norm, precision, epi, P, w2, st, &nch, &part);
      if (rc == B200KGE_ERR_UNSUPPORTED && attempt == 0) continue;
      if (rc) return rc;
      emitted = (attempt == 0);
      if ((rc = launch_loss_finalize(loss_kind, part, nch, n, total, fused, 1.0f, 0, scratch, 0, st))) return rc;
      break;
    }
  }
  if (!emitted) {
    if ((rc = launch_csr_expand(csr_off, csr_col, n, nnz, loss_kind == B200KGE_LOSS_KL ? 1 : 0, Q.idx, Pr.idx, qsel, psel,
                                esel, st))) return rc;
    if (tot > 0) {
      Rows Qs = Q; Qs.idx = qsel; Qs.rows = tot;
      Rows Ps = Pr; Ps.idx = psel; Ps.rows = tot;
      Rows Es = C; Es.idx = esel; Es.rows = tot;
      if (combine == B200KGE_SP_) rc = launch_spo(model, l_norm, Qs, Ps, Es, tot, zpos, 1, st);
      else                        rc = launch_spo(model, l_norm, Es, Ps, Qs, tot, zpos, 1, st);
      if (rc) return rc;
    }
  }
  if (label_smoothing > 0.f && dot) {
    Folded f = folded_problem(model, combine, Q.dim, l_norm);
    const int64_t ldq = round_up(f.K, 32);
    float* Qf = (float*)ws.take((size_t)n * ldq * 4);
    float* cs = (float*)ws.take(((size_t)((m + 1023) / 1024) + 1) * ldq * 4);
    zsum = (float*)ws.take((size_t)n * 4);
    if (!Qf || !cs || !zsum) { set_error("workspace too small"); return B200KGE_ERR_WORKSPACE; }
    if ((rc = launch_fold_queries(model, combine, Q, Pr, n, 0, Qf, ldq, st))) return rc;
    if ((rc = launch_row_score_sums(Qf, ldq, n, C.base + f.col_off, C.ld, m, f.K, cs, zsum, st))) return rc;
  }
  const float a = 1.0f - label_smoothing, b = label_smoothing > 0.f ? 1.0f / (float)m : 0.f;
  if ((rc = launch_csr_rows(loss_kind, csr_off, csr_col, zpos, n, nnz, fused, zsum, zch, a, b, (float)m,
                            loss_kind == B200KGE_LOSS_BCE ? offset : 0.f, rows, st))) return rc;
  return launch_rows_sum(rows, n, 1.0f, loss_out, st);
}

}

namespace {

int validate_dropout(const b200kge_dropout_t* d, int64_t n, int64_t E, int D, int Dr) {
  if (!d) { set_error("null dropout key"); return B200KGE_ERR_INVALID; }
  if (!(d->p_ent >= 0.f && d->p_ent < 1.f) || !(d->p_rel >= 0.f && d->p_rel < 1.f)) {
    set_error("dropout rates must lie in [0, 1) (got %g, %g)", (double)d->p_ent, (double)d->p_rel);
    return B200KGE_ERR_INVALID;
  }
  const double lim = 281474976710656.0;
  if (d->row_base < 0 || (double)(d->row_base + n) * D > lim || (double)(d->row_base + n) * Dr > lim ||
      (double)E * D > lim) {
    set_error("dropout rows out of range: row_base >= 0 and row * dim + k < 2^48 are required");
    return B200KGE_ERR_INVALID;
  }
  return 0;
}

DropMask drop_mask(float p, uint64_t seed, uint64_t call, int stream, int64_t row_base) {
  DropMask m;
  m.seed = seed; m.call = call; m.stream = stream; m.row_base = row_base;
  m.thresh = (uint64_t)floor((1.0 - (double)p) * 4294967296.0);
  m.scale = (float)(1.0 / (1.0 - (double)p));
  return m;
}

struct DirMasks { DropMask q, r, t; };
DirMasks dir_masks(const b200kge_dropout_t& d, int dir) {
  DirMasks m;
  m.q = drop_mask(d.p_ent, d.seed, d.call, dir == 0 ? B200KGE_DROP_SP_ENT : B200KGE_DROP_PO_ENT, d.row_base);
  m.r = drop_mask(d.p_rel, d.seed, d.call, dir == 0 ? B200KGE_DROP_SP_REL : B200KGE_DROP_PO_REL, d.row_base);
  m.t = drop_mask(d.p_ent, d.seed, d.call, dir == 0 ? B200KGE_DROP_SP_TABLE : B200KGE_DROP_PO_TABLE, 0);
  return m;
}

struct MaskedOps { float *Qm, *Pm, *Tm; };
bool take_masked(Arena& ws, int64_t n, int64_t E, int D, int Dr, MaskedOps& o) {
  o.Qm = (float*)ws.take((size_t)n * D * 4);
  o.Pm = (float*)ws.take((size_t)n * Dr * 4);
  o.Tm = (float*)ws.take((size_t)E * D * 4);
  return o.Qm && o.Pm && o.Tm;
}
int gather_masked(const DirMasks& m, const Rows& E, const Rows& R, const int64_t* q_idx, const int64_t* p_idx, int64_t n,
                  const MaskedOps& o, Rows& Qr, Rows& Pr, Rows& Tr, cudaStream_t st) {
  Rows qs = E; qs.idx = q_idx; qs.rows = n;
  Rows ps = R; ps.idx = p_idx; ps.rows = n;
  Rows ts = E; ts.idx = nullptr;
  int rc;
  if ((rc = launch_dropout_gather(m.q, qs, o.Qm, E.dim, st))) return rc;
  if ((rc = launch_dropout_gather(m.r, ps, o.Pm, R.dim, st))) return rc;
  if ((rc = launch_dropout_gather(m.t, ts, o.Tm, E.dim, st))) return rc;
  Qr = Rows{o.Qm, nullptr, n, E.dim, E.dim};
  Pr = Rows{o.Pm, nullptr, n, R.dim, R.dim};
  Tr = Rows{o.Tm, nullptr, E.rows, E.dim, E.dim};
  return 0;
}

size_t masked_bytes(int model, int64_t n, int64_t E, int32_t D) {
  const int64_t Dr = relation_dim(model, D), ldq = round_up(D, 32);
  return 2 * ((size_t)E * D * 4 + 256)
         + 2 * ((size_t)n * D * 4 + (size_t)n * Dr * 4 + 512)
         + 2 * ((size_t)n * ldq * 4 + 256)
         + (size_t)n * 10 * 8 + 5 * 256
         + (size_t)n * 2 * 4 + 4096;
}

struct BackBufs { MaskedOps o; float *Q, *dQ, *dT, *dQe, *dPr; int64_t* tri; };
bool take_back(Arena& ws, int64_t n, int64_t E, int D, int Dr, int64_t ldq, BackBufs& b) {
  if (!take_masked(ws, n, E, D, Dr, b.o)) return false;
  b.Q = (float*)ws.take((size_t)n * ldq * 4);
  b.dQ = (float*)ws.take((size_t)n * ldq * 4);
  b.dT = (float*)ws.take((size_t)E * D * 4);
  b.dQe = (float*)ws.take((size_t)n * D * 4);
  b.dPr = (float*)ws.take((size_t)n * Dr * 4);
  b.tri = (int64_t*)ws.take((size_t)n * 3 * 8);
  return b.Q && b.dQ && b.dT && b.dQe && b.dPr && b.tri;
}

int dropout_backward_dir(int model, float l_norm, int dir, int mask_dir, const Rows& E, const Rows& R, const int64_t* q_idx,
                         const int64_t* p_idx, int64_t n, const b200kge_dropout_t& d, const GradSpec& g,
                         const BackBufs& b, Arena ws, float* d_ent, int64_t lde, float* d_rel, int64_t ldr, cudaStream_t st) {
  const DirMasks m = dir_masks(d, mask_dir);
  const Folded f = folded_problem(model, dir, E.dim, l_norm);
  const int64_t ldq = round_up(f.K, 32), mE = E.rows;
  const int D = E.dim, Dr = R.dim;
  Rows Qr, Pr, Tr;
  int rc = gather_masked(m, E, R, q_idx, p_idx, n, b.o, Qr, Pr, Tr, st);
  if (rc) return rc;
  if ((rc = launch_fold_queries(model, dir, Qr, Pr, n, 0, b.Q, ldq, st))) return rc;
  B2K_CUDA(cudaMemsetAsync(b.dQe, 0, (size_t)n * D * 4, st));
  B2K_CUDA(cudaMemsetAsync(b.dPr, 0, (size_t)n * Dr * 4, st));
  if (f.pair_op == PAIR_DOT) {
    if ((rc = backward_block(model, Tr, Pr, n, dir, false, b.Q, ldq, f.col_off, f.K, g, b.dT, D, b.dQ, ws, st))) return rc;
    if ((rc = launch_unfold(model, Qr, Pr, b.tri, n, dir, b.dQ, ldq, b.dQe, D, b.dPr, Dr, st))) return rc;
  } else {
    Block B{model, dir, &Qr, nullptr, &Pr, &Tr, n};
    B.Qpre = b.Q;
    if ((rc = distance_backward(B, l_norm, g, b.dQ, b.dT, D, ws, st))) return rc;
    if ((rc = launch_unfold_distance(model, Qr, Pr, b.tri, n, dir, b.dQ, ldq, b.dQe, D, b.dPr, Dr, st))) return rc;
  }
  if ((rc = launch_dropout_add_cols(m.t, b.dT, D, mE, D, f.col_off, f.col_off + f.K, d_ent, lde, st))) return rc;
  if ((rc = launch_dropout_scatter(m.q, b.dQe, D, n, D, q_idx, d_ent, lde, st))) return rc;
  return launch_dropout_scatter(m.r, b.dPr, Dr, n, Dr, p_idx, d_rel, ldr, st);
}

Arena rest_of(const Arena& ws) {
  const size_t used = (ws.off + 255) & ~size_t(255);
  return Arena{ws.base + used, used < ws.cap ? ws.cap - used : 0, 0};
}

}

extern "C" {

int b200kge_dropout_mask(float p, uint64_t seed, uint64_t call, int mask_stream, int64_t row_base, int64_t rows,
                         int32_t dim, uint8_t* out, b200kge_stream_t stream) {
  if (!out && rows > 0 && dim > 0) { set_error("null operand"); return B200KGE_ERR_INVALID; }
  if (rows < 0 || dim < 0 || mask_stream < 0 || mask_stream >= (1 << 18)) { set_error("bad mask shape or stream"); return B200KGE_ERR_INVALID; }
  b200kge_dropout_t d{p, 0.f, seed, call, row_base};
  int rc = validate_dropout(&d, rows, 0, dim, 0); if (rc) return rc;
  return launch_dropout_mask(drop_mask(p, seed, call, mask_stream, row_base), rows, dim, out, (cudaStream_t)stream);
}

size_t b200kge_train_1vsall_dropout_workspace_bytes(int model, int64_t n, int64_t E, int32_t D) {
  size_t dir = b200kge_score_1vsN_backward_workspace_bytes(model, n, E, D) + (size_t)n * 2 * 4 + 1024;
  const size_t fwd = b200kge_workspace_bytes(model, n, E, D, 0);
  return masked_bytes(model, n, E, D) + (dir > fwd ? dir : fwd);
}

static int train_1vsall_forward_dropout_impl(int model, float l_norm, int precision, const b200kge_rows_t* ent,
                                             const b200kge_rows_t* rel, const int64_t* triples, int64_t n,
                                             int loss_kind, float offset, const b200kge_dropout_t* drop,
                                             float* loss_out, void* workspace, size_t workspace_bytes,
                                             cudaStream_t st, int64_t num_rel) {
  if (!triples || !loss_out) { set_error("null operand"); return B200KGE_ERR_INVALID; }
  int rc = check_tables(model, l_norm, ent, rel); if (rc) return rc;
  if ((rc = check_loss_kind(loss_kind))) return rc;
  if ((rc = validate_dropout(drop, n > 0 ? n : 0, ent->rows, ent->dim, rel->dim))) return rc;
  if (n <= 0) { B2K_CUDA(cudaMemsetAsync(loss_out, 0, 4, st)); return 0; }
  Arena ws{(uint8_t*)workspace, workspace_bytes, 0};
  Rows E = to_rows(ent), R = to_rows(rel);
  int64_t* sidx = (int64_t*)ws.take((size_t)n * 8);
  int64_t* pidx = (int64_t*)ws.take((size_t)n * 8);
  int64_t* oidx = (int64_t*)ws.take((size_t)n * 8);
  int64_t* pinv = num_rel > 0 ? (int64_t*)ws.take((size_t)n * 8) : nullptr;
  int64_t* lab = (int64_t*)ws.take((size_t)n * 2 * 8);
  float* dir_loss = (float*)ws.take(256);
  MaskedOps o;
  if (!sidx || !pidx || !oidx || (num_rel > 0 && !pinv) || !lab || !dir_loss ||
      !take_masked(ws, n, E.rows, E.dim, R.dim, o)) {
    set_error("workspace too small (see b200kge_train_1vsall_%s_workspace_bytes)", num_rel > 0 ? "reciprocal" : "dropout");
    return B200KGE_ERR_WORKSPACE;
  }
  Rows S, O, P;
  if ((rc = unpack_triples(triples, n, sidx, pidx, oidx, lab, E, R, S, O, P, st))) return rc;
  if (num_rel > 0) {
    offset_index_kernel<<<(unsigned)((n + 255) / 256), 256, 0, st>>>(pidx, n, num_rel, pinv);
    B2K_LAUNCH_CHECK("offset_index_kernel");
  }
  const Arena rest = rest_of(ws);
  for (int dir = 0; dir < 2; ++dir) {
    Rows Qr, Pr, Tr;
    if ((rc = gather_masked(dir_masks(*drop, dir), E, R, dir == 0 ? sidx : oidx, dir == 1 && pinv ? pinv : pidx, n, o,
                            Qr, Pr, Tr, st))) return rc;
    const b200kge_rows_t q{Qr.base, nullptr, n, Qr.ld, Qr.dim}, p{Pr.base, nullptr, n, Pr.ld, Pr.dim},
        c{Tr.base, nullptr, Tr.rows, Tr.ld, Tr.dim};
    const b200kge_labels_t labels{lab + dir * n, nullptr, 0};
    if ((rc = b200kge_score_1vsN_loss(model, num_rel > 0 ? B200KGE_SP_ : dir, l_norm, precision, &q, &p, &c, n, &labels,
                                      loss_kind, offset, dir_loss + dir, nullptr, rest.base, rest.cap, st))) return rc;
  }
  return launch_rows_sum(dir_loss, 2, 1.0f / (float)n, loss_out, st);
}

static int train_1vsall_backward_dropout_impl(int model, float l_norm, const b200kge_rows_t* ent,
                                              const b200kge_rows_t* rel, const int64_t* triples, int64_t n,
                                              int loss_kind, float offset, const b200kge_dropout_t* drop, float* d_ent,
                                              int64_t lde, float* d_rel, int64_t ldr, void* workspace,
                                              size_t workspace_bytes, cudaStream_t st, int64_t num_rel) {
  if (!triples || !d_ent || !d_rel) { set_error("null operand"); return B200KGE_ERR_INVALID; }
  int rc = check_tables(model, l_norm, ent, rel); if (rc) return rc;
  if ((rc = check_loss_kind(loss_kind))) return rc;
  if ((rc = check_grad_ld(ent, lde, rel, ldr))) return rc;
  if ((rc = validate_dropout(drop, n > 0 ? n : 0, ent->rows, ent->dim, rel->dim))) return rc;
  const Folded f = folded_problem(model, B200KGE_SP_, ent->dim, l_norm);
  if (f.pair_op != PAIR_DOT && (rc = check_distance_pair(f.pair_op))) return rc;
  Rows E = to_rows(ent), R = to_rows(rel);
  B2K_CUDA(cudaMemsetAsync(d_rel, 0, (size_t)R.rows * ldr * 4, st));
  B2K_CUDA(cudaMemsetAsync(d_ent, 0, (size_t)E.rows * lde * 4, st));
  if (n <= 0) return 0;
  Arena ws{(uint8_t*)workspace, workspace_bytes, 0};
  int64_t* sidx = (int64_t*)ws.take((size_t)n * 8);
  int64_t* pidx = (int64_t*)ws.take((size_t)n * 8);
  int64_t* oidx = (int64_t*)ws.take((size_t)n * 8);
  int64_t* pinv = num_rel > 0 ? (int64_t*)ws.take((size_t)n * 8) : nullptr;
  int64_t* lab = (int64_t*)ws.take((size_t)n * 2 * 8);
  BackBufs b;
  if (!sidx || !pidx || !oidx || (num_rel > 0 && !pinv) || !lab ||
      !take_back(ws, n, E.rows, E.dim, R.dim, round_up(f.K, 32), b)) {
    set_error("workspace too small (see b200kge_train_1vsall_%s_workspace_bytes)", num_rel > 0 ? "reciprocal" : "dropout");
    return B200KGE_ERR_WORKSPACE;
  }
  Rows S, O, P;
  if ((rc = unpack_triples(triples, n, sidx, pidx, oidx, lab, E, R, S, O, P, st))) return rc;
  if (num_rel > 0) {
    offset_index_kernel<<<(unsigned)((n + 255) / 256), 256, 0, st>>>(pidx, n, num_rel, pinv);
    B2K_LAUNCH_CHECK("offset_index_kernel");
  }
  if ((rc = launch_identity_triples(n, b.tri, st))) return rc;
  const Arena rest = rest_of(ws);
  GradSpec g;
  g.loss_kind = loss_kind; g.offset = offset;
  for (int dir = 0; dir < 2; ++dir) {
    g.lab = lab + dir * n;
    if ((rc = dropout_backward_dir(model, l_norm, num_rel > 0 ? B200KGE_SP_ : dir, dir, E, R, dir == 0 ? sidx : oidx,
                                   dir == 1 && pinv ? pinv : pidx, n, *drop, g, b, rest, d_ent, lde, d_rel, ldr, st)))
      return rc;
  }
  return 0;
}

int b200kge_train_1vsall_forward_dropout(int model, float l_norm, int precision, const b200kge_rows_t* ent,
                                         const b200kge_rows_t* rel, const int64_t* triples, int64_t n, int loss_kind,
                                         float offset, const b200kge_dropout_t* drop, float* loss_out, void* workspace,
                                         size_t workspace_bytes, b200kge_stream_t stream) {
  return train_1vsall_forward_dropout_impl(model, l_norm, precision, ent, rel, triples, n, loss_kind, offset, drop,
                                           loss_out, workspace, workspace_bytes, (cudaStream_t)stream, 0);
}

int b200kge_train_1vsall_backward_dropout(int model, float l_norm, const b200kge_rows_t* ent, const b200kge_rows_t* rel,
                                          const int64_t* triples, int64_t n, int loss_kind, float offset,
                                          const b200kge_dropout_t* drop, float* d_ent, int64_t lde, float* d_rel,
                                          int64_t ldr, void* workspace, size_t workspace_bytes, b200kge_stream_t stream) {
  return train_1vsall_backward_dropout_impl(model, l_norm, ent, rel, triples, n, loss_kind, offset, drop, d_ent, lde,
                                            d_rel, ldr, workspace, workspace_bytes, (cudaStream_t)stream, 0);
}

size_t b200kge_train_1vsall_reciprocal_workspace_bytes(int model, int64_t n, int64_t E, int32_t D) {
  const size_t fwd = b200kge_workspace_bytes(model, n, E, D, 0);
  const size_t bwd = b200kge_train_1vsall_backward_workspace_bytes(model, n, E, D);
  const size_t drop = b200kge_train_1vsall_dropout_workspace_bytes(model, n, E, D) + (size_t)n * 8 + 256;
  const size_t m = fwd > bwd ? fwd : bwd;
  return m > drop ? m : drop;
}

int b200kge_train_1vsall_reciprocal_forward(int model, float l_norm, int precision, const b200kge_rows_t* ent,
                                            const b200kge_rows_t* rel, int64_t num_relations, const int64_t* triples,
                                            int64_t n, int loss_kind, float offset, const b200kge_dropout_t* drop,
                                            float* loss_out, void* workspace, size_t workspace_bytes,
                                            b200kge_stream_t stream) {
  if (!ent || !rel || !triples || !loss_out) { set_error("null operand"); return B200KGE_ERR_INVALID; }
  int rc = check_reciprocal(rel, num_relations); if (rc) return rc;
  if (!drop)
    return train_1vsall_forward_impl(model, l_norm, precision, ent, rel, triples, n, loss_kind, offset, loss_out,
                                     workspace, workspace_bytes, stream, num_relations);
  return train_1vsall_forward_dropout_impl(model, l_norm, precision, ent, rel, triples, n, loss_kind, offset, drop,
                                           loss_out, workspace, workspace_bytes, (cudaStream_t)stream, num_relations);
}

int b200kge_train_1vsall_reciprocal_backward(int model, float l_norm, const b200kge_rows_t* ent,
                                             const b200kge_rows_t* rel, int64_t num_relations, const int64_t* triples,
                                             int64_t n, int loss_kind, float offset, const b200kge_dropout_t* drop,
                                             float* d_ent, int64_t lde, float* d_rel, int64_t ldr, void* workspace,
                                             size_t workspace_bytes, b200kge_stream_t stream) {
  if (!ent || !rel || !triples || !d_ent || !d_rel) { set_error("null operand"); return B200KGE_ERR_INVALID; }
  int rc = check_reciprocal(rel, num_relations); if (rc) return rc;
  if (!drop)
    return train_1vsall_backward_impl(model, l_norm, ent, rel, triples, n, loss_kind, offset, d_ent, lde, d_rel, ldr,
                                      workspace, workspace_bytes, stream, num_relations);
  return train_1vsall_backward_dropout_impl(model, l_norm, ent, rel, triples, n, loss_kind, offset, drop, d_ent, lde,
                                            d_rel, ldr, workspace, workspace_bytes, (cudaStream_t)stream, num_relations);
}

size_t b200kge_score_1vsN_loss_csr_dropout_workspace_bytes(int model, int64_t n, int64_t E, int32_t D, int64_t nnz) {
  const size_t fwd = b200kge_score_1vsN_loss_csr_workspace_bytes(model, n, E, D, nnz);
  const size_t bwd = b200kge_score_1vsN_backward_workspace_bytes(model, n, E, D) + 1024;
  return masked_bytes(model, n, E, D) + (fwd > bwd ? fwd : bwd);
}

int b200kge_score_1vsN_loss_csr_dropout_dir(int model, int combine, int mask_dir, float l_norm, int precision,
                                            const b200kge_rows_t* ent, const b200kge_rows_t* rel, const int64_t* q_idx,
                                            const int64_t* p_idx, int64_t n, const int64_t* csr_off,
                                            const int64_t* csr_col, int64_t nnz, float label_smoothing, int loss_kind,
                                            float offset, const b200kge_dropout_t* drop, float* loss_out,
                                            float* row_loss_out, void* workspace, size_t workspace_bytes,
                                            b200kge_stream_t stream) {
  if ((!q_idx && n > 0) || (!p_idx && n > 0) || !loss_out) { set_error("null operand"); return B200KGE_ERR_INVALID; }
  if (combine != B200KGE_SP_ && combine != B200KGE__PO) { set_error("cannot handle combine=%d", combine); return B200KGE_ERR_INVALID; }
  if (mask_dir != B200KGE_SP_ && mask_dir != B200KGE__PO) { set_error("bad mask direction %d", mask_dir); return B200KGE_ERR_INVALID; }
  int rc = check_tables(model, 1.0f, ent, rel); if (rc) return rc;
  if ((rc = validate_dropout(drop, n > 0 ? n : 0, ent->rows, ent->dim, rel->dim))) return rc;
  cudaStream_t st = (cudaStream_t)stream;
  if (n <= 0) { B2K_CUDA(cudaMemsetAsync(loss_out, 0, 4, st)); return 0; }
  Arena ws{(uint8_t*)workspace, workspace_bytes, 0};
  Rows E = to_rows(ent), R = to_rows(rel);
  MaskedOps o;
  if (!take_masked(ws, n, E.rows, E.dim, R.dim, o)) {
    set_error("workspace too small (see b200kge_score_1vsN_loss_csr_dropout_workspace_bytes)");
    return B200KGE_ERR_WORKSPACE;
  }
  Rows Qr, Pr, Tr;
  if ((rc = gather_masked(dir_masks(*drop, mask_dir), E, R, q_idx, p_idx, n, o, Qr, Pr, Tr, st))) return rc;
  const b200kge_rows_t q{Qr.base, nullptr, n, Qr.ld, Qr.dim}, p{Pr.base, nullptr, n, Pr.ld, Pr.dim},
      c{Tr.base, nullptr, Tr.rows, Tr.ld, Tr.dim};
  const Arena rest = rest_of(ws);
  return b200kge_score_1vsN_loss_csr(model, combine, l_norm, precision, &q, &p, &c, n, csr_off, csr_col, nnz,
                                     label_smoothing, loss_kind, offset, loss_out, row_loss_out, rest.base, rest.cap,
                                     stream);
}

int b200kge_score_1vsN_loss_csr_dropout(int model, int combine, float l_norm, int precision, const b200kge_rows_t* ent,
                                        const b200kge_rows_t* rel, const int64_t* q_idx, const int64_t* p_idx, int64_t n,
                                        const int64_t* csr_off, const int64_t* csr_col, int64_t nnz,
                                        float label_smoothing, int loss_kind, float offset,
                                        const b200kge_dropout_t* drop, float* loss_out, float* row_loss_out,
                                        void* workspace, size_t workspace_bytes, b200kge_stream_t stream) {
  return b200kge_score_1vsN_loss_csr_dropout_dir(model, combine, combine, l_norm, precision, ent, rel, q_idx, p_idx, n,
                                                 csr_off, csr_col, nnz, label_smoothing, loss_kind, offset, drop,
                                                 loss_out, row_loss_out, workspace, workspace_bytes, stream);
}

int b200kge_score_1vsN_loss_csr_backward_dropout_norm(int model, int combine, int mask_dir, float l_norm,
                                                      const b200kge_rows_t* ent, const b200kge_rows_t* rel,
                                                      const int64_t* q_idx, const int64_t* p_idx, int64_t n,
                                                      const int64_t* csr_off, const int64_t* csr_col,
                                                      float label_smoothing, int loss_kind, float offset,
                                                      int64_t batch_size, const b200kge_dropout_t* drop, float* d_ent,
                                                      int64_t lde, float* d_rel, int64_t ldr, void* workspace,
                                                      size_t workspace_bytes, b200kge_stream_t stream) {
  if (!q_idx || !p_idx || !csr_off || !d_ent || !d_rel) { set_error("null operand"); return B200KGE_ERR_INVALID; }
  if (combine != B200KGE_SP_ && combine != B200KGE__PO) { set_error("cannot handle combine=%d", combine); return B200KGE_ERR_INVALID; }
  if (mask_dir != B200KGE_SP_ && mask_dir != B200KGE__PO) { set_error("bad mask direction %d", mask_dir); return B200KGE_ERR_INVALID; }
  int rc = check_tables(model, l_norm, ent, rel); if (rc) return rc;
  const bool distance = (model == B200KGE_TRANSE || model == B200KGE_ROTATE);
  if (!distance) l_norm = 1.0f;
  const Folded f = folded_problem(model, combine, ent->dim, l_norm);
  if (distance && (rc = check_distance_pair(f.pair_op))) return rc;
  if ((rc = check_loss_kind(loss_kind))) return rc;
  if (batch_size <= 0 || !(label_smoothing >= 0.f && label_smoothing < 1.f)) { set_error("bad batch_size / label_smoothing"); return B200KGE_ERR_INVALID; }
  if ((rc = check_grad_ld(ent, lde, rel, ldr))) return rc;
  if ((rc = validate_dropout(drop, n > 0 ? n : 0, ent->rows, ent->dim, rel->dim))) return rc;
  cudaStream_t st = (cudaStream_t)stream;
  Rows E = to_rows(ent), R = to_rows(rel);
  B2K_CUDA(cudaMemsetAsync(d_rel, 0, (size_t)R.rows * ldr * 4, st));
  B2K_CUDA(cudaMemsetAsync(d_ent, 0, (size_t)E.rows * lde * 4, st));
  if (n <= 0) return 0;
  Arena ws{(uint8_t*)workspace, workspace_bytes, 0};
  BackBufs b;
  if (!take_back(ws, n, E.rows, E.dim, R.dim, round_up(f.K, 32), b)) {
    set_error("workspace too small (see b200kge_score_1vsN_loss_csr_dropout_workspace_bytes)");
    return B200KGE_ERR_WORKSPACE;
  }
  if ((rc = launch_identity_triples(n, b.tri, st))) return rc;
  const GradSpec g = csr_grad(q_idx, csr_off, csr_col, label_smoothing, E.rows, batch_size, loss_kind, offset);
  return dropout_backward_dir(model, l_norm, combine, mask_dir, E, R, q_idx, p_idx, n, *drop, g, b, rest_of(ws), d_ent,
                              lde, d_rel, ldr, st);
}

int b200kge_score_1vsN_loss_csr_backward_dropout_dir(int model, int combine, int mask_dir, const b200kge_rows_t* ent,
                                                     const b200kge_rows_t* rel, const int64_t* q_idx,
                                                     const int64_t* p_idx, int64_t n, const int64_t* csr_off,
                                                     const int64_t* csr_col, float label_smoothing, int loss_kind,
                                                     float offset, int64_t batch_size, const b200kge_dropout_t* drop,
                                                     float* d_ent, int64_t lde, float* d_rel, int64_t ldr,
                                                     void* workspace, size_t workspace_bytes, b200kge_stream_t stream) {
  return b200kge_score_1vsN_loss_csr_backward_dropout_norm(model, combine, mask_dir, 1.0f, ent, rel, q_idx, p_idx, n,
                                                           csr_off, csr_col, label_smoothing, loss_kind, offset,
                                                           batch_size, drop, d_ent, lde, d_rel, ldr, workspace,
                                                           workspace_bytes, stream);
}

int b200kge_score_1vsN_loss_csr_backward_dropout(int model, int combine, const b200kge_rows_t* ent,
                                                 const b200kge_rows_t* rel, const int64_t* q_idx, const int64_t* p_idx,
                                                 int64_t n, const int64_t* csr_off, const int64_t* csr_col,
                                                 float label_smoothing, int loss_kind, float offset, int64_t batch_size,
                                                 const b200kge_dropout_t* drop, float* d_ent, int64_t lde, float* d_rel,
                                                 int64_t ldr, void* workspace, size_t workspace_bytes,
                                                 b200kge_stream_t stream) {
  return b200kge_score_1vsN_loss_csr_backward_dropout_dir(model, combine, combine, ent, rel, q_idx, p_idx, n, csr_off,
                                                          csr_col, label_smoothing, loss_kind, offset, batch_size, drop,
                                                          d_ent, lde, d_rel, ldr, workspace, workspace_bytes, stream);
}

}

namespace {

int validate_ns_dropout(int model, float l_norm, const b200kge_rows_t* ent, const b200kge_rows_t* rel,
                        const int64_t* triples, int slot, const int64_t* neg, int64_t n, int64_t K, int impl,
                        const b200kge_dropout_t* drop) {
  if ((!triples && n > 0) || (!neg && n * K > 0)) { set_error("null operand"); return B200KGE_ERR_INVALID; }
  if (n < 0 || K < 0) { set_error("negative sizes"); return B200KGE_ERR_INVALID; }
  int rc = check_tables(model, l_norm, ent, rel); if (rc) return rc;
  if (impl != B200KGE_NS_TRIPLE && impl != B200KGE_NS_BATCH) { set_error("impl must be B200KGE_NS_TRIPLE or B200KGE_NS_BATCH"); return B200KGE_ERR_INVALID; }
  if (slot != 0 && slot != 2) { set_error("negative-sampling dropout covers the S and O slots"); return B200KGE_ERR_UNSUPPORTED; }
  if ((model == B200KGE_TRANSE && l_norm != 1.0f && l_norm != 2.0f) || (model == B200KGE_ROTATE && l_norm != 1.0f)) {
    set_error("negative-sampling dropout covers l_norm 1 and 2 (TransE) / 1 (RotatE)");
    return B200KGE_ERR_UNSUPPORTED;
  }
  const int D = ent->dim;
  const bool halves = model == B200KGE_COMPLEX || model == B200KGE_SIMPLE || model == B200KGE_CP || model == B200KGE_ROTATE;
  if (D % (halves ? 8 : 4) != 0) {
    set_error("negative-sampling dropout needs D %% %d == 0 (got %d)", halves ? 8 : 4, D);
    return B200KGE_ERR_UNSUPPORTED;
  }
  if (!drop) { set_error("null dropout key"); return B200KGE_ERR_INVALID; }
  if (impl == B200KGE_NS_BATCH && model != B200KGE_RESCAL && D > 1024) {
    set_error("negative-sampling dropout with `batch` covers D <= 1024 (got %d)", D);
    return B200KGE_ERR_UNSUPPORTED;
  }
  if ((rc = validate_dropout(drop, n, ent->rows, D, rel->dim))) return rc;
  const double lim = 281474976710656.0;
  const double top = ((double)drop->row_base + (double)n) * (double)(K > 0 ? K : 1);
  if (impl == B200KGE_NS_TRIPLE && (top * ent->dim > lim || top * rel->dim > lim)) {
    set_error("dropout rows out of range: row * dim + k < 2^48 is required");
    return B200KGE_ERR_INVALID;
  }
  return 0;
}

NsDropKeys ns_drop_keys(const b200kge_dropout_t& d) {
  NsDropKeys k;
  k.ent = drop_mask(d.p_ent, d.seed, d.call, 0, 0);
  k.rel = drop_mask(d.p_rel, d.seed, d.call, 0, 0);
  k.row_base = d.row_base;
  return k;
}

}

extern "C" {

int b200kge_ns_score_dropout(int model, float l_norm, const b200kge_rows_t* ent, const b200kge_rows_t* rel,
                             const int64_t* triples, int slot, const int64_t* neg, int64_t n, int64_t K, int impl,
                             const b200kge_dropout_t* drop, float* out, int64_t ldo, b200kge_stream_t stream) {
  int rc = validate_ns_dropout(model, l_norm, ent, rel, triples, slot, neg, n, K, impl, drop); if (rc) return rc;
  if (n == 0) return 0;
  if (!out) { set_error("null operand"); return B200KGE_ERR_INVALID; }
  if (ldo < K + 1) { set_error("out is narrower than the 1 + K columns of the block"); return B200KGE_ERR_INVALID; }
  return launch_ns_dropout(model, l_norm, to_rows(ent), to_rows(rel), triples, slot, neg, n, K, impl, ns_drop_keys(*drop),
                           nullptr, 0, out, ldo, nullptr, 0, nullptr, 0, nullptr, 0, (cudaStream_t)stream);
}

size_t b200kge_ns_dropout_workspace_bytes(int model, int64_t n, int64_t K, int32_t D) {
  (void)K;
  return (n > 0 && D > 0) ? ns_dropout_workspace_bytes(model, n, D) : 0;
}

int b200kge_ns_backward_dropout(int model, float l_norm, const b200kge_rows_t* ent, const b200kge_rows_t* rel,
                                const int64_t* triples, int slot, const int64_t* neg, int64_t n, int64_t K, int impl,
                                const b200kge_dropout_t* drop, const float* grad_scores, int64_t ldg, float* d_ent,
                                int64_t lde, float* d_rel, int64_t ldr, void* workspace, size_t workspace_bytes,
                                b200kge_stream_t stream) {
  int rc = validate_ns_dropout(model, l_norm, ent, rel, triples, slot, neg, n, K, impl, drop); if (rc) return rc;
  if (n == 0) return 0;
  if (!grad_scores || !d_ent || !d_rel) { set_error("null operand"); return B200KGE_ERR_INVALID; }
  if (ldg < K + 1) { set_error("grad_scores is narrower than the 1 + K columns of the block"); return B200KGE_ERR_INVALID; }
  if ((rc = check_grad_ld(ent, lde, rel, ldr))) return rc;
  return launch_ns_dropout(model, l_norm, to_rows(ent), to_rows(rel), triples, slot, neg, n, K, impl, ns_drop_keys(*drop),
                           grad_scores, ldg, nullptr, 0, d_ent, lde, d_rel, ldr, workspace, workspace_bytes,
                           (cudaStream_t)stream);
}

}
```

kge_b200/csrc/pairwise_tc.cu:

```cuda
#include "tc_common.cuh"

namespace b200kge {

namespace {

enum Mode : int { MODE_F16X3 = 0, MODE_TF32 = 1, MODE_TF32X3 = 2, MODE_MIXED = 3 };

constexpr int TM = 128;
constexpr int TN = 128;
constexpr int NSTAGE = 3;
constexpr int STAGE_BYTES = 64 * 1024;
constexpr int BOX_BYTES = 16 * 1024;
constexpr int STATE_BYTES = 256 * 4 * (int)sizeof(RowState<EPI_KL>);
static_assert(sizeof(RowState<EPI_RANK_EVAL>) <= sizeof(RowState<EPI_KL>), "row state slots are sized for KL");
constexpr int SMEM_BYTES = 1024  + NSTAGE * STAGE_BYTES + 256  + STATE_BYTES;
static_assert(SMEM_BYTES <= 227 * 1024, "exceeds the H100's 227 KB of shared memory per block");

template <int MODE> struct ModeCfg {
  static constexpr bool SPLIT = MODE == MODE_TF32X3 || MODE == MODE_MIXED;
  static constexpr bool PP = !SPLIT;
  static constexpr int MH = PP ? 2 : 1;
  static constexpr int NTHREADS = (SPLIT ? 4 : 3) * 128;
  static constexpr int TK = MODE == MODE_F16X3 ? 64 : 32;
  static constexpr uint32_t TX = MODE == MODE_F16X3 ? 4 * BOX_BYTES : 2 * BOX_BYTES;
  static constexpr uint32_t STAGE_CONSUMERS = PP ? 4 : 8;
};

struct TcParams {
  int64_t nq, m;
  int nk;
  int q_tiles, e_tiles;
  int ksplit;
  int kseg;
  int64_t items;
  int grid;
  int nsl;
  const float* q_scale;
  const float* t_scale;
  EpiParams epi;
};

struct Item { int qt, et, k0, k1; };
__device__ __forceinline__ Item item_at(const TcParams& p, int64_t i) {
  Item it;
  int ks = 0;
  if (p.ksplit > 1) { ks = (int)(i % p.ksplit); i /= p.ksplit; }
  it.qt = (int)(i / p.e_tiles);
  it.et = (int)(i - (int64_t)it.qt * p.e_tiles);
  it.k0 = ks * p.kseg;
  it.k1 = it.k0 + p.kseg < p.nk ? it.k0 + p.kseg : p.nk;
  return it;
}

template <int MODE>
__device__ __forceinline__ void mma_chunk(float (&d)[64], uint32_t st, int h) {
  const uint32_t a = st + (uint32_t)h * (BOX_BYTES / 2), b = st + BOX_BYTES;
  if constexpr (MODE == MODE_F16X3) {
#pragma unroll
    for (int k = 0; k < 4; ++k) {
      const uint32_t o = k * 32;
      ptx::wgmma_f16(d, ptx::wg_desc_sw128(a + o), ptx::wg_desc_sw128(b + o));
      ptx::wgmma_f16(d, ptx::wg_desc_sw128(a + o), ptx::wg_desc_sw128(b + 2 * BOX_BYTES + o));
      ptx::wgmma_f16(d, ptx::wg_desc_sw128(a + 2 * BOX_BYTES + o), ptx::wg_desc_sw128(b + o));
    }
  } else {
#pragma unroll
    for (int k = 0; k < 4; ++k)
      ptx::wgmma_tf32(d, ptx::wg_desc_sw128(a + k * 32), ptx::wg_desc_sw128(b + k * 32));
    if constexpr (MODE == MODE_TF32X3) {
#pragma unroll
      for (int k = 0; k < 4; ++k) {
        ptx::wgmma_tf32(d, ptx::wg_desc_sw128(a + 2 * BOX_BYTES + k * 32), ptx::wg_desc_sw128(b + k * 32));
        ptx::wgmma_tf32(d, ptx::wg_desc_sw128(a + k * 32), ptx::wg_desc_sw128(b + 2 * BOX_BYTES + k * 32));
      }
    } else if constexpr (MODE == MODE_MIXED) {
      const uint32_t hq = st + 2 * BOX_BYTES + (uint32_t)h * (BOX_BYTES / 4);
      const uint32_t lq = hq + BOX_BYTES / 2;
      const uint32_t th = st + 3 * BOX_BYTES, tl = th + BOX_BYTES / 2;
#pragma unroll
      for (int k = 0; k < 2; ++k) {
        ptx::wgmma_bf16(d, ptx::wg_desc_sw64(lq + k * 32), ptx::wg_desc_sw64(th + k * 32));
        ptx::wgmma_bf16(d, ptx::wg_desc_sw64(hq + k * 32), ptx::wg_desc_sw64(tl + k * 32));
      }
    }
  }
}

template <int EPI, int MODE>
__global__ void __launch_bounds__(ModeCfg<MODE>::NTHREADS, 1)
pairwise_tc_kernel(const __grid_constant__ CUtensorMap tmQ, const __grid_constant__ CUtensorMap tmT,
                   const __grid_constant__ CUtensorMap tmQl, const __grid_constant__ CUtensorMap tmTl,
                   const TcParams prm) {
  using C = ModeCfg<MODE>;
  extern __shared__ uint8_t smem_raw[];
  uint8_t* smem = reinterpret_cast<uint8_t*>((reinterpret_cast<uintptr_t>(smem_raw) + 1023) & ~uintptr_t(1023));
  uint64_t* bars = reinterpret_cast<uint64_t*>(smem + NSTAGE * STAGE_BYTES);
  uint64_t* full = bars;
  uint64_t* split = bars + NSTAGE;
  uint64_t* empty = bars + 2 * NSTAGE;
  uint64_t* turn = bars + 3 * NSTAGE;

  const int warp = threadIdx.x >> 5, lane = threadIdx.x & 31;
  const int64_t i0 = (int64_t)blockIdx.x * prm.items / prm.grid, i1 = (int64_t)(blockIdx.x + 1) * prm.items / prm.grid;

  if (threadIdx.x == 0) {
    ptx::prefetch_tensormap(&tmQ);
    ptx::prefetch_tensormap(&tmT);
    if constexpr (MODE == MODE_F16X3) {
      ptx::prefetch_tensormap(&tmQl);
      ptx::prefetch_tensormap(&tmTl);
    }
    for (int s = 0; s < NSTAGE; ++s) {
      ptx::mbar_init(&full[s], 1);
      ptx::mbar_init(&split[s], 4);
      ptx::mbar_init(&empty[s], C::STAGE_CONSUMERS);
    }
    ptx::mbar_init(&turn[0], 1);
    ptx::mbar_init(&turn[1], 1);
    ptx::fence_barrier_init();
  }
  __syncthreads();

  if (warp < 4) {
    if constexpr (C::PP) ptx::setmaxnreg_dec<40>();
    if (warp == 0 && lane == 0) {
      uint32_t c = 0;
      for (int64_t i = i0; i < i1; ++i) {
        const Item it = item_at(prm, i);
        for (int kc = it.k0; kc < it.k1; ++kc, ++c) {
          const int s = (int)(c % NSTAGE);
          ptx::mbar_wait_bounded(&empty[s], ((c / NSTAGE) & 1) ^ 1);
          uint8_t* sp = smem + s * STAGE_BYTES;
          ptx::mbar_arrive_expect_tx(&full[s], C::TX);
          ptx::tma_load_2d(sp, &tmQ, &full[s], kc * C::TK, it.qt * TM);
          ptx::tma_load_2d(sp + BOX_BYTES, &tmT, &full[s], kc * C::TK, it.et * TN);
          if constexpr (MODE == MODE_F16X3) {
            ptx::tma_load_2d(sp + 2 * BOX_BYTES, &tmQl, &full[s], kc * C::TK, it.qt * TM);
            ptx::tma_load_2d(sp + 3 * BOX_BYTES, &tmTl, &full[s], kc * C::TK, it.et * TN);
          }
        }
      }
    }
  } else if (warp >= 12) {
    if constexpr (C::SPLIT) {
      const int t = threadIdx.x - 12 * 32;
      uint32_t c = 0;
      for (int64_t i = i0; i < i1; ++i) {
        const Item it = item_at(prm, i);
        for (int kc = it.k0; kc < it.k1; ++kc, ++c) {
          const int s = (int)(c % NSTAGE);
          ptx::mbar_wait_bounded(&full[s], (c / NSTAGE) & 1);
          const uint32_t sp = ptx::smem_u32(smem + s * STAGE_BYTES);
          if constexpr (MODE == MODE_TF32X3) {
            tc::split_tile<BOX_BYTES, 128>(sp, sp + 2 * BOX_BYTES, t);
            tc::split_tile<BOX_BYTES, 128>(sp + BOX_BYTES, sp + 3 * BOX_BYTES, t);
          } else {
            tc::split_tile_bf16<TM, 128>(sp, sp + 2 * BOX_BYTES, sp + 2 * BOX_BYTES + BOX_BYTES / 2, t);
            tc::split_tile_bf16<TN, 128>(sp + BOX_BYTES, sp + 3 * BOX_BYTES, sp + 3 * BOX_BYTES + BOX_BYTES / 2, t);
          }
          ptx::fence_proxy_async_smem();
          __syncwarp();
          if (lane == 0) ptx::mbar_arrive(&split[s]);
        }
      }
    }
  } else {
    if constexpr (C::PP) ptx::setmaxnreg_inc<232>();
    const int g = (warp - 4) >> 2;
    const int tg = threadIdx.x & 127, q = tg & 3;
    const int row_in_tile = (C::PP ? 0 : 64 * g) + 16 * (tg >> 5) + ((tg & 31) >> 2);
    const EpiParams& P = prm.epi;
    RowState<EPI>* st = reinterpret_cast<RowState<EPI>*>(smem + NSTAGE * STAGE_BYTES + 256) + (threadIdx.x - 128);
#pragma unroll
    for (int rr = 0; rr < 2 * C::MH; ++rr) st[256 * rr].init();
    uint32_t c = 0;
    for (int64_t i = i0; i < i1; ++i) {
      const Item it = item_at(prm, i);
      const int nkc = it.k1 - it.k0;
      if (!C::PP || (int)((i - i0) & 1) == g) {
        const uint32_t k = (uint32_t)((i - i0) >> 1);
        if (C::PP && (g == 1 || k > 0)) ptx::mbar_wait_bounded(&turn[g], (g == 1 ? k : k - 1) & 1);
        float d[C::MH][64];
#pragma unroll
        for (int h = 0; h < C::MH; ++h)
#pragma unroll
          for (int e = 0; e < 64; ++e) d[h][e] = 0.f;
        for (int kk = 0; kk < nkc; ++kk) {
          const uint32_t cc = c + kk;
          const int s = (int)(cc % NSTAGE);
          ptx::mbar_wait_bounded(&full[s], (cc / NSTAGE) & 1);
          if constexpr (C::SPLIT) ptx::mbar_wait_bounded(&split[s], (cc / NSTAGE) & 1);
          ptx::wg_fence();
#pragma unroll
          for (int h = 0; h < C::MH; ++h) mma_chunk<MODE>(d[h], ptx::smem_u32(smem + s * STAGE_BYTES), C::PP ? h : g);
          ptx::wg_commit();
          if (kk > 0) {
            ptx::wg_wait<1>();
            __syncwarp();
            if (lane == 0) ptx::mbar_arrive(&empty[(cc - 1) % NSTAGE]);
          }
        }
        if (C::PP && tg == 0) ptx::mbar_arrive(&turn[g ^ 1]);
        ptx::wg_wait<0>();
        __syncwarp();
        if (lane == 0) ptx::mbar_arrive(&empty[(c + nkc - 1) % NSTAGE]);

        const int64_t e0 = (int64_t)it.et * TN;
        if constexpr (MODE == MODE_F16X3) {
          float qs[2 * C::MH];
#pragma unroll
          for (int rr = 0; rr < 2 * C::MH; ++rr) {
            const int64_t row = (int64_t)it.qt * TM + row_in_tile + 64 * (rr >> 1) + 8 * (rr & 1);
            qs[rr] = row < prm.nq ? __ldg(prm.q_scale + row) : 0.f;
          }
#pragma unroll
          for (int j = 0; j < 16; ++j) {
            const int64_t col = e0 + 2 * q + 8 * j;
            const float2 ts = col < prm.m ? __ldg(reinterpret_cast<const float2*>(prm.t_scale + col)) : make_float2(0.f, 0.f);
#pragma unroll
            for (int rr = 0; rr < 2 * C::MH; ++rr) {
              float* a = &d[rr >> 1][4 * j + 2 * (rr & 1)];
              a[0] = a[0] * (qs[rr] * ts.x);
              a[1] = a[1] * (qs[rr] * ts.y);
            }
          }
        }
#pragma unroll
        for (int rr = 0; rr < 2 * C::MH; ++rr) {
          const int64_t row = (int64_t)it.qt * TM + row_in_tile + 64 * (rr >> 1) + 8 * (rr & 1);
          if (row < prm.nq) {
            float v[32];
#pragma unroll
            for (int j = 0; j < 16; ++j) {
              v[2 * j] = d[rr >> 1][4 * j + 2 * (rr & 1)];
              v[2 * j + 1] = d[rr >> 1][4 * j + 2 * (rr & 1) + 1];
            }
            RowState<EPI> rs = st[256 * rr];
            tc::epi_row<EPI>(P, rs, v, row, e0, prm.m, q);
            st[256 * rr] = rs;
          }
        }
      }
      c += nkc;
      if constexpr (EPI != EPI_STORE) {
        const bool ends_qt = (i + 1) % prm.e_tiles == 0;
        if (ends_qt || i + 1 == i1) {
          const int qt = (int)(i / prm.e_tiles);
          const int64_t first = (((int64_t)qt * prm.e_tiles + 1) * prm.grid - 1) / prm.items;
          const int j = (int)(blockIdx.x - first);
          const int h = C::PP ? g : (q >> 1);
          const bool writer = C::PP ? q == 0 : (q & 1) == 0;
#pragma unroll
          for (int rr = 0; rr < 2 * C::MH; ++rr) {
            RowState<EPI> rs = st[256 * rr];
            epi_lane_reduce<EPI>(rs, C::PP ? 4 : 2);
            const int64_t row = (int64_t)qt * TM + row_in_tile + 64 * (rr >> 1) + 8 * (rr & 1);
            if (writer && row < prm.nq) {
              epi_flush<EPI>(P, rs, row, 2 * j + h);
              if constexpr (EPI != EPI_RANK && EPI != EPI_RANK_EVAL) {
                if (ends_qt) {
                  RowState<EPI> z;
                  z.init();
                  for (int jj = j + 1; jj < prm.nsl; ++jj) epi_flush<EPI>(P, z, row, 2 * jj + h);
                }
              }
            }
            st[256 * rr].init();
          }
        }
      }
    }
  }
}

using tc::num_sms;

void schedule(int64_t nq, int64_t m, int ksplit, TcParams& prm) {
  prm.q_tiles = (int)((nq + TM - 1) / TM);
  if (prm.q_tiles < 1) prm.q_tiles = 1;
  prm.e_tiles = (int)((m + TN - 1) / TN);
  prm.ksplit = ksplit;
  prm.items = (int64_t)prm.q_tiles * prm.e_tiles * ksplit;
  prm.grid = prm.items < num_sms() ? (int)prm.items : num_sms();
  const int64_t per = prm.items / prm.grid;
  const int64_t nsl = (prm.e_tiles + per - 1) / per + 1;
  prm.nsl = nsl < prm.grid ? (int)nsl : prm.grid;
}

template <int EPI, int MODE>
int launch_k(const CUtensorMap (&maps)[4], const TcParams& prm, cudaStream_t st) {
  auto kern = pairwise_tc_kernel<EPI, MODE>;
  cudaError_t e = cudaFuncSetAttribute(kern, cudaFuncAttributeMaxDynamicSharedMemorySize, SMEM_BYTES);
  if (e != cudaSuccess) return check_cuda(e, "cudaFuncSetAttribute(pairwise_tc_kernel)");
  profile_begin(st);
  kern<<<prm.grid, ModeCfg<MODE>::NTHREADS, SMEM_BYTES, st>>>(maps[0], maps[1], maps[2], maps[3], prm);
  profile_end(st);
  B2K_LAUNCH_CHECK("pairwise_tc_kernel");
  return 0;
}

template <int MODE>
int launch_mode(int epi_kind, const CUtensorMap (&maps)[4], const TcParams& prm, cudaStream_t st) {
  switch (epi_kind) {
    case EPI_STORE: return launch_k<EPI_STORE, MODE>(maps, prm, st);
    case EPI_BCE:   return launch_k<EPI_BCE, MODE>(maps, prm, st);
    case EPI_KL:    return launch_k<EPI_KL, MODE>(maps, prm, st);
    case EPI_RANK:  return launch_k<EPI_RANK, MODE>(maps, prm, st);
    case EPI_RANK_EVAL:
      if constexpr (MODE == MODE_F16X3) return launch_k<EPI_RANK_EVAL, MODE>(maps, prm, st);
      break;
  }
  set_error("bad epilogue kind %d", epi_kind);
  return B200KGE_ERR_INVALID;
}

}

bool tc_supported(int pair_op, int K, const Rows& cand, int col_off) {
  if (pair_op != PAIR_DOT) return false;
  if (K < 32) return false;
  if (cand.ld % 4 != 0 || col_off % 4 != 0) return false;
  if ((reinterpret_cast<uintptr_t>(cand.base) & 15) != 0) return false;
  if (cand.rows >= (1ll << 31)) return false;
  return true;
}

int tc_nchunks(int64_t nq, int64_t m) {
  TcParams prm;
  schedule(nq, m, 1, prm);
  return 2 * prm.nsl;
}

int launch_pairwise_tc(int epi_kind, int passes, const float* Q, int64_t ldq,
                       int64_t nq, const float* T, int64_t ldt, int64_t m, int K,
                       const EpiParams& P, cudaStream_t st) {
  if (nq == 0 || m == 0) return 0;
  CUtensorMap maps[4];
  int rc;
  if ((rc = tc::make_map(&maps[0], Q, nq, K, ldq, 32, TM))) return rc;
  if ((rc = tc::make_map(&maps[1], T, m, K, ldt, 32, TN))) return rc;
  maps[2] = maps[0]; maps[3] = maps[1];
  TcParams prm;
  prm.nq = nq; prm.m = m; prm.nk = (K + 31) / 32;
  schedule(nq, m, 1, prm);
  prm.kseg = prm.nk;
  prm.q_scale = nullptr; prm.t_scale = nullptr;
  prm.epi = P;
  prm.epi.nchunks = 2 * prm.nsl;
  if (passes == 3) return launch_mode<MODE_TF32X3>(epi_kind, maps, prm, st);
  if (passes == 2) return launch_mode<MODE_MIXED>(epi_kind, maps, prm, st);
  return launch_mode<MODE_TF32>(epi_kind, maps, prm, st);
}

int launch_pairwise_tc3(int epi_kind, const SplitSet& Q, const SplitSet& T, const EpiParams& P, cudaStream_t st) {
  const int64_t nq = Q.rows, m = T.rows;
  if (nq == 0 || m == 0) return 0;
  if (Q.Kp != T.Kp || Q.Kp % 64 != 0) { set_error("operand planes disagree on the padded reduction length"); return B200KGE_ERR_INVALID; }
  TcParams prm;
  prm.nq = nq; prm.m = m; prm.nk = Q.Kp / 64;
  prm.kseg = prm.nk;
  if (P.accumulate_out) {
    if (epi_kind != EPI_STORE) { set_error("split-K accumulation is a GEMM (store) mode"); return B200KGE_ERR_INVALID; }
    prm.kseg = 8;
  }
  schedule(nq, m, (prm.nk + prm.kseg - 1) / prm.kseg, prm);
  prm.q_scale = Q.inv_scale; prm.t_scale = T.inv_scale;
  CUtensorMap maps[4];
  int rc;
  if ((rc = tc::make_map_f16(&maps[0], Q.hi, nq, Q.Kp, Q.Kp, TM))) return rc;
  if ((rc = tc::make_map_f16(&maps[1], T.hi, m, T.Kp, T.Kp, TN))) return rc;
  if ((rc = tc::make_map_f16(&maps[2], Q.lo, nq, Q.Kp, Q.Kp, TM))) return rc;
  if ((rc = tc::make_map_f16(&maps[3], T.lo, m, T.Kp, T.Kp, TN))) return rc;
  prm.epi = P;
  prm.epi.nchunks = 2 * prm.nsl;
  return launch_mode<MODE_F16X3>(epi_kind, maps, prm, st);
}

}
```

kge_b200/csrc/presplit.cu:

```cuda
#include <cuda_fp16.h>
#include "fold.cuh"
#include "tc_common.cuh"

namespace b200kge {

namespace {

constexpr int PS_WARPS = 8;

__device__ __forceinline__ void presplit_row(const SplitSet& S, int64_t r, int lane) {
  if (r >= S.rows) {
    if (r < S.rows_pad && lane == 0) S.inv_scale[r] = 0.f;
    return;
  }
  const int64_t src_row = S.idx ? S.idx[r] : r;
  const float* __restrict__ x = S.src + src_row * S.ld + S.col_off;
  const int K = S.K, Kp = S.Kp;
  const bool vec = (K % 4 == 0) && ((reinterpret_cast<uintptr_t>(x) & 15) == 0);
  float amax = 0.f;
  bool bad = false;
  if (vec) {
    for (int k = lane * 4; k < K; k += 128) {
      const float4 v = __ldg(reinterpret_cast<const float4*>(x + k));
      amax = fmaxf(amax, fmaxf(fmaxf(fabsf(v.x), fabsf(v.y)), fmaxf(fabsf(v.z), fabsf(v.w))));
      bad |= !(isfinite(v.x) && isfinite(v.y) && isfinite(v.z) && isfinite(v.w));
    }
  } else {
    for (int k = lane; k < K; k += 32) {
      const float v = __ldg(x + k);
      amax = fmaxf(amax, fabsf(v));
      bad |= !isfinite(v);
    }
  }
#pragma unroll
  for (int o = 16; o > 0; o >>= 1) amax = fmaxf(amax, __shfl_xor_sync(0xffffffffu, amax, o));
  bad = __any_sync(0xffffffffu, bad);
  int e = 13;
  if (amax > 0.f && !bad) {
    e = ilogbf(amax);
    e = e < -60 ? -60 : (e > 60 ? 60 : e);
  }
  const float mul = scalbnf(1.f, 13 - e), inv = scalbnf(1.f, e - 13);
  __half* __restrict__ hi = reinterpret_cast<__half*>(S.hi) + r * Kp;
  __half* __restrict__ lo = reinterpret_cast<__half*>(S.lo) + r * Kp;
  if (vec) {
    for (int k = lane * 4; k < Kp; k += 128) {
      float4 v = make_float4(0.f, 0.f, 0.f, 0.f);
      if (k < K) v = __ldg(reinterpret_cast<const float4*>(x + k));
      const float s[4] = {v.x * mul, v.y * mul, v.z * mul, v.w * mul};
      __half h[4], l[4];
#pragma unroll
      for (int i = 0; i < 4; ++i) {
        h[i] = __float2half_rn(s[i]);
        l[i] = __float2half_rn(s[i] - __half2float(h[i]));
      }
      uint2 ph, pl;
      ph.x = (uint32_t)__half_as_ushort(h[0]) | ((uint32_t)__half_as_ushort(h[1]) << 16);
      ph.y = (uint32_t)__half_as_ushort(h[2]) | ((uint32_t)__half_as_ushort(h[3]) << 16);
      pl.x = (uint32_t)__half_as_ushort(l[0]) | ((uint32_t)__half_as_ushort(l[1]) << 16);
      pl.y = (uint32_t)__half_as_ushort(l[2]) | ((uint32_t)__half_as_ushort(l[3]) << 16);
      *reinterpret_cast<uint2*>(hi + k) = ph;
      *reinterpret_cast<uint2*>(lo + k) = pl;
    }
  } else {
    for (int k = lane; k < Kp; k += 32) {
      const float s = (k < K) ? __ldg(x + k) * mul : 0.f;
      const __half h = __float2half_rn(s);
      hi[k] = h;
      lo[k] = __float2half_rn(s - __half2float(h));
    }
  }
  if (lane == 0) S.inv_scale[r] = inv;
}

__global__ void __launch_bounds__(PS_WARPS * 32)
presplit_kernel(const SplitSet A, const SplitSet B, const int blocks_a) {
  const int warp = threadIdx.x >> 5, lane = threadIdx.x & 31;
  if ((int)blockIdx.x < blocks_a) presplit_row(A, (int64_t)blockIdx.x * PS_WARPS + warp, lane);
  else presplit_row(B, (int64_t)(blockIdx.x - blocks_a) * PS_WARPS + warp, lane);
}

__global__ void __launch_bounds__(PS_WARPS * 32)
presplit_longrow_kernel(const SplitSet A, const SplitSet B, const int rows_a) {
  __shared__ float red[PS_WARPS];
  __shared__ int bad_any;
  const bool first = (int)blockIdx.x < rows_a;
  const SplitSet& S = first ? A : B;
  const int64_t r = first ? blockIdx.x : blockIdx.x - rows_a;
  const int warp = threadIdx.x >> 5, lane = threadIdx.x & 31;
  if (r >= S.rows) {
    if (threadIdx.x == 0) S.inv_scale[r] = 0.f;
    return;
  }
  const int64_t src_row = S.idx ? S.idx[r] : r;
  const float* __restrict__ x = S.src + src_row * S.ld + S.col_off;
  const int K = S.K, Kp = S.Kp;
  if (threadIdx.x == 0) bad_any = 0;
  float amax = 0.f;
  bool bad = false;
  for (int k = threadIdx.x; k < K; k += blockDim.x) {
    const float v = __ldg(x + k);
    amax = fmaxf(amax, fabsf(v));
    bad |= !isfinite(v);
  }
#pragma unroll
  for (int o = 16; o > 0; o >>= 1) amax = fmaxf(amax, __shfl_xor_sync(0xffffffffu, amax, o));
  __syncthreads();
  if (__any_sync(0xffffffffu, bad) && lane == 0) bad_any = 1;
  if (lane == 0) red[warp] = amax;
  __syncthreads();
  amax = red[0];
#pragma unroll
  for (int w = 1; w < PS_WARPS; ++w) amax = fmaxf(amax, red[w]);
  int e = 13;
  if (amax > 0.f && !bad_any) {
    e = ilogbf(amax);
    e = e < -60 ? -60 : (e > 60 ? 60 : e);
  }
  const float mul = scalbnf(1.f, 13 - e);
  __half2* __restrict__ hi = reinterpret_cast<__half2*>(reinterpret_cast<__half*>(S.hi) + r * Kp);
  __half2* __restrict__ lo = reinterpret_cast<__half2*>(reinterpret_cast<__half*>(S.lo) + r * Kp);
  for (int k = threadIdx.x * 2; k < Kp; k += blockDim.x * 2) {
    const float s0 = (k < K) ? __ldg(x + k) * mul : 0.f, s1 = (k + 1 < K) ? __ldg(x + k + 1) * mul : 0.f;
    const __half h0 = __float2half_rn(s0), h1 = __float2half_rn(s1);
    hi[k >> 1] = __halves2half2(h0, h1);
    lo[k >> 1] = __halves2half2(__float2half_rn(s0 - __half2float(h0)), __float2half_rn(s1 - __half2float(h1)));
  }
  if (threadIdx.x == 0) S.inv_scale[r] = scalbnf(1.f, e - 13);
}

constexpr int PQ_THREADS = PS_WARPS * 32;

template <int MODEL, bool RECIP>
__global__ void __launch_bounds__(PQ_THREADS)
prep_split_1vsall_kernel(Rows ent, Rows rel, const int64_t* __restrict__ tri, int64_t n, const SplitSet Qs,
                         const SplitSet Ts, int64_t* __restrict__ labels2n, unsigned int* ticket, int K,
                         int64_t num_rel) {
  extern __shared__ float sh[];
  const int64_t b = blockIdx.x;
  const int warp = threadIdx.x >> 5, lane = threadIdx.x & 31;
  if (b >= 2 * n) {
    presplit_row(Ts, (b - 2 * n) * PS_WARPS + warp, lane);
    return;
  }
  __shared__ float red[PS_WARPS];
  __shared__ int bad_any;
  const bool first = b < n;
  const bool sp = RECIP || first;
  const int64_t i = first ? b : b - n;
  const int64_t si = tri[3 * i], pi = tri[3 * i + 1], oi = tri[3 * i + 2];
  const float* __restrict__ a = ent.base + (first ? si : oi) * ent.ld;
  const float* __restrict__ p = rel.base + (RECIP && !first ? pi + num_rel : pi) * rel.ld;
  const int D = ent.dim, h = D >> 1, Kp = Qs.Kp;
  if (threadIdx.x == 0) {
    labels2n[b] = first ? oi : si;
    bad_any = 0;
  }
  if (b == 0 && ticket && threadIdx.x == 0) *ticket = 0u;
  float* q = sh;
  if constexpr (MODEL == B200KGE_RESCAL) {
    float* sh_a = sh + Kp;
    for (int k = threadIdx.x; k < D; k += blockDim.x) sh_a[k] = a[k];
    __syncthreads();
    fold_rescal_block(sp, sh_a, p, D, [&](int k, float v) { q[k] = v; });
  } else {
    for (int k = threadIdx.x; k < K; k += blockDim.x) q[k] = fold_element<MODEL>(sp, a, p, k, h);
  }
  for (int k = K + threadIdx.x; k < Kp; k += blockDim.x) q[k] = 0.f;
  __syncthreads();
  float amax = 0.f;
  bool bad = false;
  for (int k = threadIdx.x; k < K; k += blockDim.x) { const float v = q[k]; amax = fmaxf(amax, fabsf(v)); bad |= !isfinite(v); }
#pragma unroll
  for (int o = 16; o > 0; o >>= 1) amax = fmaxf(amax, __shfl_xor_sync(0xffffffffu, amax, o));
  if (__any_sync(0xffffffffu, bad) && lane == 0) bad_any = 1;
  if (lane == 0) red[warp] = amax;
  __syncthreads();
  amax = red[0];
#pragma unroll
  for (int w = 1; w < PS_WARPS; ++w) amax = fmaxf(amax, red[w]);
  int e = 13;
  if (amax > 0.f && !bad_any) {
    e = ilogbf(amax);
    e = e < -60 ? -60 : (e > 60 ? 60 : e);
  }
  const float mul = scalbnf(1.f, 13 - e);
  __half* __restrict__ hi = reinterpret_cast<__half*>(Qs.hi) + b * Kp;
  __half* __restrict__ lo = reinterpret_cast<__half*>(Qs.lo) + b * Kp;
  for (int k = threadIdx.x * 4; k < Kp; k += blockDim.x * 4) {
    __half hh[4], ll[4];
#pragma unroll
    for (int j = 0; j < 4; ++j) {
      const float sv = q[k + j] * mul;
      hh[j] = __float2half_rn(sv);
      ll[j] = __float2half_rn(sv - __half2float(hh[j]));
    }
    uint2 ph, pl;
    ph.x = (uint32_t)__half_as_ushort(hh[0]) | ((uint32_t)__half_as_ushort(hh[1]) << 16);
    ph.y = (uint32_t)__half_as_ushort(hh[2]) | ((uint32_t)__half_as_ushort(hh[3]) << 16);
    pl.x = (uint32_t)__half_as_ushort(ll[0]) | ((uint32_t)__half_as_ushort(ll[1]) << 16);
    pl.y = (uint32_t)__half_as_ushort(ll[2]) | ((uint32_t)__half_as_ushort(ll[3]) << 16);
    *reinterpret_cast<uint2*>(hi + k) = ph;
    *reinterpret_cast<uint2*>(lo + k) = pl;
  }
  if (threadIdx.x == 0) Qs.inv_scale[b] = scalbnf(1.f, e - 13);
}

}

int launch_prep_split_1vsall(int model, const Rows& ent, const Rows& rel, const int64_t* triples, int64_t n,
                             const SplitSet& Qs, const SplitSet& Ts, int64_t* labels2n, unsigned int* ticket,
                             cudaStream_t st, int64_t num_rel) {
  if (n == 0) return 0;
  const int D = ent.dim;
  const int K = (model == B200KGE_CP) ? D / 2 : D;
  const int64_t tb = (Ts.rows_pad + PS_WARPS - 1) / PS_WARPS;
  if (2 * n + tb >= (1ll << 31)) { set_error("too many rows for the fused prologue"); return B200KGE_ERR_INVALID; }
  const size_t smem = ((size_t)Qs.Kp + (model == B200KGE_RESCAL ? D : 0)) * sizeof(float);
  if (smem > 48 * 1024) { set_error("embedding too wide for the fused prologue"); return B200KGE_ERR_UNSUPPORTED; }
  dim3 grid((unsigned)(2 * n + tb)), block(PQ_THREADS);
#define B2K_PS(M) case M: prep_split_1vsall_kernel<M, false><<<grid, block, smem, st>>>(ent, rel, triples, n, Qs, Ts, labels2n, ticket, K, 0); break;
#define B2K_PS_R(M) case M: prep_split_1vsall_kernel<M, true><<<grid, block, smem, st>>>(ent, rel, triples, n, Qs, Ts, labels2n, ticket, K, num_rel); break;
  if (num_rel > 0) {
    switch (model) {
      B2K_PS_R(B200KGE_COMPLEX) B2K_PS_R(B200KGE_DISTMULT) B2K_PS_R(B200KGE_SIMPLE) B2K_PS_R(B200KGE_CP)
      B2K_PS_R(B200KGE_RESCAL)
      default: set_error("model %d has no fused pre-split prologue", model); return B200KGE_ERR_UNSUPPORTED;
    }
  } else {
    switch (model) {
      B2K_PS(B200KGE_COMPLEX) B2K_PS(B200KGE_DISTMULT) B2K_PS(B200KGE_SIMPLE) B2K_PS(B200KGE_RESCAL)
      default: set_error("model %d has no fused pre-split prologue", model); return B200KGE_ERR_UNSUPPORTED;
    }
  }
#undef B2K_PS
#undef B2K_PS_R
  B2K_LAUNCH_CHECK("prep_split_1vsall_kernel");
  return 0;
}

int launch_presplit(const SplitSet& A, const SplitSet& B, cudaStream_t st) {
  const int64_t ba = (A.rows_pad + PS_WARPS - 1) / PS_WARPS, bb = (B.rows_pad + PS_WARPS - 1) / PS_WARPS;
  if (ba + bb == 0) return 0;
  if (ba + bb >= (1ll << 31)) { set_error("too many rows for the operand split"); return B200KGE_ERR_INVALID; }
  if ((A.K >= 4096 || (B.rows_pad > 0 && B.K >= 4096)) && A.rows_pad + B.rows_pad < (1ll << 31)) {
    presplit_longrow_kernel<<<(unsigned)(A.rows_pad + B.rows_pad), PS_WARPS * 32, 0, st>>>(A, B, (int)A.rows_pad);
    B2K_LAUNCH_CHECK("presplit_longrow_kernel");
    return 0;
  }
  presplit_kernel<<<(unsigned)(ba + bb), PS_WARPS * 32, 0, st>>>(A, B, (int)ba);
  B2K_LAUNCH_CHECK("presplit_kernel");
  return 0;
}

}
```

kge_b200/csrc/ptx.cuh:

```cuda
#pragma once
#include <cuda.h>
#include <cuda_runtime.h>
#include <stdint.h>

namespace b200kge {
namespace ptx {

__device__ __forceinline__ uint32_t smem_u32(const void* p) {
  return static_cast<uint32_t>(__cvta_generic_to_shared(p));
}

__device__ __forceinline__ bool elect_one() {
  uint32_t pred;
  asm volatile(
      "{\n\t.reg .pred p;\n\t"
      "elect.sync _|p, 0xffffffff;\n\t"
      "selp.u32 %0, 1, 0, p;\n\t}"
      : "=r"(pred));
  return pred != 0;
}

__device__ __forceinline__ void mbar_init(uint64_t* bar, uint32_t count) {
  asm volatile("mbarrier.init.shared::cta.b64 [%0], %1;" ::"r"(smem_u32(bar)), "r"(count) : "memory");
}
__device__ __forceinline__ void fence_barrier_init() {
  asm volatile("fence.mbarrier_init.release.cluster;" ::: "memory");
}
__device__ __forceinline__ void mbar_arrive(uint64_t* bar) {
  asm volatile("mbarrier.arrive.shared::cta.b64 _, [%0];" ::"r"(smem_u32(bar)) : "memory");
}
__device__ __forceinline__ void mbar_arrive_expect_tx(uint64_t* bar, uint32_t bytes) {
  asm volatile("mbarrier.arrive.expect_tx.shared::cta.b64 _, [%0], %1;" ::"r"(smem_u32(bar)), "r"(bytes)
               : "memory");
}
__device__ __forceinline__ bool mbar_try_wait(uint64_t* bar, uint32_t parity) {
  uint32_t ok;
  asm volatile(
      "{\n\t.reg .pred p;\n\t"
      "mbarrier.try_wait.parity.shared::cta.b64 p, [%1], %2;\n\t"
      "selp.u32 %0, 1, 0, p;\n\t}"
      : "=r"(ok) : "r"(smem_u32(bar)), "r"(parity) : "memory");
  return ok != 0;
}
__device__ __forceinline__ void mbar_wait_bounded(uint64_t* bar, uint32_t parity) {
  for (uint32_t polls = 0; !mbar_try_wait(bar, parity); ++polls)
    if (polls > (1u << 24)) __trap();
}

__device__ __forceinline__ void fence_proxy_async_smem() {
  asm volatile("fence.proxy.async.shared::cta;" ::: "memory");
}
__device__ __forceinline__ void bar_sync(uint32_t id, uint32_t nthreads) {
  asm volatile("bar.sync %0, %1;" ::"r"(id), "r"(nthreads) : "memory");
}

template <uint32_t N>
__device__ __forceinline__ void setmaxnreg_dec() { asm volatile("setmaxnreg.dec.sync.aligned.u32 %0;" ::"n"(N)); }
template <uint32_t N>
__device__ __forceinline__ void setmaxnreg_inc() { asm volatile("setmaxnreg.inc.sync.aligned.u32 %0;" ::"n"(N)); }

__device__ __forceinline__ void prefetch_tensormap(const CUtensorMap* m) {
  asm volatile("prefetch.tensormap [%0];" ::"l"(reinterpret_cast<uint64_t>(m)) : "memory");
}
__device__ __forceinline__ void tma_load_2d(void* smem_dst, const CUtensorMap* m, uint64_t* bar,
                                            int32_t c0, int32_t c1) {
  asm volatile(
      "cp.async.bulk.tensor.2d.shared::cluster.global.tile.mbarrier::complete_tx::bytes"
      " [%0], [%1, {%3, %4}], [%2];"
      ::"r"(smem_u32(smem_dst)), "l"(reinterpret_cast<uint64_t>(m)), "r"(smem_u32(bar)), "r"(c0), "r"(c1)
      : "memory");
}

__device__ __forceinline__ uint64_t wg_desc_sw128(uint32_t smem_addr) {
  return (uint64_t)((smem_addr & 0x3FFFFu) >> 4) | ((uint64_t)1 << 16) | ((uint64_t)(1024 >> 4) << 32) |
         ((uint64_t)1 << 62);
}
__device__ __forceinline__ uint64_t wg_desc_sw64(uint32_t smem_addr) {
  return (uint64_t)((smem_addr & 0x3FFFFu) >> 4) | ((uint64_t)1 << 16) | ((uint64_t)(512 >> 4) << 32) |
         ((uint64_t)2 << 62);
}

__device__ __forceinline__ void wg_fence() { asm volatile("wgmma.fence.sync.aligned;" ::: "memory"); }
__device__ __forceinline__ void wg_commit() { asm volatile("wgmma.commit_group.sync.aligned;" ::: "memory"); }
template <int N>
__device__ __forceinline__ void wg_wait() { asm volatile("wgmma.wait_group.sync.aligned %0;" ::"n"(N) : "memory"); }

#define B2K_WG_D64                                                                                               \
  "{%0, %1, %2, %3, %4, %5, %6, %7, %8, %9, %10, %11, %12, %13, %14, %15, "                                     \
  "%16, %17, %18, %19, %20, %21, %22, %23, %24, %25, %26, %27, %28, %29, %30, %31, "                            \
  "%32, %33, %34, %35, %36, %37, %38, %39, %40, %41, %42, %43, %44, %45, %46, %47, "                            \
  "%48, %49, %50, %51, %52, %53, %54, %55, %56, %57, %58, %59, %60, %61, %62, %63}"
#define B2K_WG_OUT64(d)                                                                                          \
  "+f"(d[0]), "+f"(d[1]), "+f"(d[2]), "+f"(d[3]), "+f"(d[4]), "+f"(d[5]), "+f"(d[6]), "+f"(d[7]),              \
  "+f"(d[8]), "+f"(d[9]), "+f"(d[10]), "+f"(d[11]), "+f"(d[12]), "+f"(d[13]), "+f"(d[14]), "+f"(d[15]),        \
  "+f"(d[16]), "+f"(d[17]), "+f"(d[18]), "+f"(d[19]), "+f"(d[20]), "+f"(d[21]), "+f"(d[22]), "+f"(d[23]),      \
  "+f"(d[24]), "+f"(d[25]), "+f"(d[26]), "+f"(d[27]), "+f"(d[28]), "+f"(d[29]), "+f"(d[30]), "+f"(d[31]),      \
  "+f"(d[32]), "+f"(d[33]), "+f"(d[34]), "+f"(d[35]), "+f"(d[36]), "+f"(d[37]), "+f"(d[38]), "+f"(d[39]),      \
  "+f"(d[40]), "+f"(d[41]), "+f"(d[42]), "+f"(d[43]), "+f"(d[44]), "+f"(d[45]), "+f"(d[46]), "+f"(d[47]),      \
  "+f"(d[48]), "+f"(d[49]), "+f"(d[50]), "+f"(d[51]), "+f"(d[52]), "+f"(d[53]), "+f"(d[54]), "+f"(d[55]),      \
  "+f"(d[56]), "+f"(d[57]), "+f"(d[58]), "+f"(d[59]), "+f"(d[60]), "+f"(d[61]), "+f"(d[62]), "+f"(d[63])

__device__ __forceinline__ void wgmma_f16(float (&d)[64], uint64_t adesc, uint64_t bdesc) {
  asm volatile("{\n\t.reg .pred p;\n\tsetp.ne.b32 p, 1, 0;\n\t"
               "wgmma.mma_async.sync.aligned.m64n128k16.f32.f16.f16 " B2K_WG_D64 ", %64, %65, p, 1, 1, 0, 0;\n\t}"
               : B2K_WG_OUT64(d) : "l"(adesc), "l"(bdesc) : "memory");
}
__device__ __forceinline__ void wgmma_bf16(float (&d)[64], uint64_t adesc, uint64_t bdesc) {
  asm volatile("{\n\t.reg .pred p;\n\tsetp.ne.b32 p, 1, 0;\n\t"
               "wgmma.mma_async.sync.aligned.m64n128k16.f32.bf16.bf16 " B2K_WG_D64 ", %64, %65, p, 1, 1, 0, 0;\n\t}"
               : B2K_WG_OUT64(d) : "l"(adesc), "l"(bdesc) : "memory");
}
__device__ __forceinline__ void wgmma_tf32(float (&d)[64], uint64_t adesc, uint64_t bdesc) {
  asm volatile("{\n\t.reg .pred p;\n\tsetp.ne.b32 p, 1, 0;\n\t"
               "wgmma.mma_async.sync.aligned.m64n128k8.f32.tf32.tf32 " B2K_WG_D64 ", %64, %65, p, 1, 1;\n\t}"
               : B2K_WG_OUT64(d) : "l"(adesc), "l"(bdesc) : "memory");
}
#undef B2K_WG_D64
#undef B2K_WG_OUT64

}
}
```

kge_b200/csrc/tc_common.cuh:

```cuda
#pragma once
#include <cuda.h>
#include <cstdlib>
#include "common.cuh"
#include "ptx.cuh"

namespace b200kge {
namespace tc {

__device__ __forceinline__ float tf32_rna(float x) {
  uint32_t u;
  asm("cvt.rna.tf32.f32 %0, %1;" : "=r"(u) : "f"(x));
  return __uint_as_float(u);
}

__device__ __forceinline__ float4 trunc_tf32_4(const float4 v) {
  return make_float4(__uint_as_float(__float_as_uint(v.x) & 0xFFFFE000u), __uint_as_float(__float_as_uint(v.y) & 0xFFFFE000u),
                     __uint_as_float(__float_as_uint(v.z) & 0xFFFFE000u), __uint_as_float(__float_as_uint(v.w) & 0xFFFFE000u));
}
__device__ __forceinline__ float4 split_lo4(const float4 v) {
  float4 l;
  l.x = tf32_rna(v.x - __uint_as_float(__float_as_uint(v.x) & 0xFFFFE000u));
  l.y = tf32_rna(v.y - __uint_as_float(__float_as_uint(v.y) & 0xFFFFE000u));
  l.z = tf32_rna(v.z - __uint_as_float(__float_as_uint(v.z) & 0xFFFFE000u));
  l.w = tf32_rna(v.w - __uint_as_float(__float_as_uint(v.w) & 0xFFFFE000u));
  return l;
}

__device__ __forceinline__ float4 lds128(uint32_t addr) {
  float4 v;
  asm volatile("ld.shared.v4.f32 {%0, %1, %2, %3}, [%4];" : "=f"(v.x), "=f"(v.y), "=f"(v.z), "=f"(v.w) : "r"(addr));
  return v;
}
__device__ __forceinline__ void sts128(uint32_t addr, const float4 v) {
  asm volatile("st.shared.v4.f32 [%0], {%1, %2, %3, %4};" ::"r"(addr), "f"(v.x), "f"(v.y), "f"(v.z), "f"(v.w) : "memory");
}

template <int NBYTES, int NTHR>
__device__ __forceinline__ void split_tile(uint32_t src, uint32_t dst, int t) {
  constexpr int PER = NBYTES / 16 / NTHR;
  static_assert(PER * NTHR * 16 == NBYTES, "tile must divide evenly");
  float4 v[PER];
#pragma unroll
  for (int i = 0; i < PER; ++i) v[i] = lds128(src + (uint32_t)(t + i * NTHR) * 16u);
#pragma unroll
  for (int i = 0; i < PER; ++i) {
    sts128(dst + (uint32_t)(t + i * NTHR) * 16u, split_lo4(v[i]));
    sts128(src + (uint32_t)(t + i * NTHR) * 16u, trunc_tf32_4(v[i]));
  }
}

__device__ __forceinline__ uint32_t pack_bf16x2(float a, float b) {
  uint32_t r;
  asm("cvt.rn.bf16x2.f32 %0, %1, %2;" : "=r"(r) : "f"(b), "f"(a));
  return r;
}
template <int ROWS, int NTHR>
__device__ __forceinline__ void split_tile_bf16(uint32_t src, uint32_t dst_hi, uint32_t dst_lo, int t) {
  constexpr int ITEMS = ROWS * 4, PER = ITEMS / NTHR, RSTEP = NTHR / 4;
  static_assert(PER * NTHR == ITEMS && RSTEP % 8 == 0, "tile must divide evenly; row step keeps the swizzle phase");
  const int r0 = t >> 2, c = t & 3;
  const uint32_t s0 = src + (uint32_t)r0 * 128u + (uint32_t)(((2 * c) ^ (r0 & 7)) * 16);
  const uint32_t s1 = src + (uint32_t)r0 * 128u + (uint32_t)(((2 * c + 1) ^ (r0 & 7)) * 16);
  const uint32_t doff = (uint32_t)r0 * 64u + (uint32_t)((c ^ ((r0 >> 1) & 3)) * 16);
  float4 v0[PER], v1[PER];
#pragma unroll
  for (int i = 0; i < PER; ++i) {
    v0[i] = lds128(s0 + (uint32_t)(i * RSTEP * 128));
    v1[i] = lds128(s1 + (uint32_t)(i * RSTEP * 128));
  }
#pragma unroll
  for (int i = 0; i < PER; ++i) {
    const float x[8] = {v0[i].x, v0[i].y, v0[i].z, v0[i].w, v1[i].x, v1[i].y, v1[i].z, v1[i].w};
    float lo[8];
#pragma unroll
    for (int k = 0; k < 8; ++k) lo[k] = x[k] - __uint_as_float(__float_as_uint(x[k]) & 0xFFFFE000u);
    const uint32_t roff = (uint32_t)(i * RSTEP * 128);
    sts128(s0 + roff, trunc_tf32_4(v0[i]));
    sts128(s1 + roff, trunc_tf32_4(v1[i]));
    const uint32_t off = doff + (uint32_t)(i * RSTEP * 64);
    asm volatile("st.shared.v4.b32 [%0], {%1, %2, %3, %4};" ::"r"(dst_hi + off), "r"(pack_bf16x2(x[0], x[1])),
                 "r"(pack_bf16x2(x[2], x[3])), "r"(pack_bf16x2(x[4], x[5])), "r"(pack_bf16x2(x[6], x[7])) : "memory");
    asm volatile("st.shared.v4.b32 [%0], {%1, %2, %3, %4};" ::"r"(dst_lo + off), "r"(pack_bf16x2(lo[0], lo[1])),
                 "r"(pack_bf16x2(lo[2], lo[3])), "r"(pack_bf16x2(lo[4], lo[5])), "r"(pack_bf16x2(lo[6], lo[7])) : "memory");
  }
}


constexpr float LOG2E = 1.4426950408889634f, LN2 = 0.6931471805599453f;

__device__ __forceinline__ float fast_ex2(float x) {
  float y;
  asm("ex2.approx.ftz.f32 %0, %1;" : "=f"(y) : "f"(x));
  return y;
}

__device__ __forceinline__ constexpr int frag_col(int k) { return 8 * (k >> 1) + (k & 1); }

__device__ __forceinline__ int frag_elem(int tc, int q) {
  return ((tc >> 1) & 3) == q ? 2 * (tc >> 3) + (tc & 1) : -1;
}

__device__ __forceinline__ float frag_get(const float (&v)[32], int k) {
  float x = 0.f;
#pragma unroll
  for (int i = 0; i < 32; ++i)
    if (i == k) x = v[i];
  return x;
}

template <int EPI, bool FULL>
__device__ __forceinline__ void epi_row_body(const EpiParams& P, RowState<EPI>& st, const float (&v)[32], int64_t row,
                                             int64_t e0, int64_t c0, int nvalid, int q) {
  if constexpr (EPI == EPI_BCE) {
    const float off = P.offset;
    float amax = 0.f, alg = 0.f;
#pragma unroll
    for (int k = 0; k < 32; ++k) {
      if (FULL || frag_col(k) < nvalid) {
        const float z = v[k] + off;
        const float e = fast_ex2(-fabsf(z) * LOG2E);
        alg += __log2f(1.0f + e);
        amax += fmaxf(z, 0.f);
      }
    }
    st.a += fmaf(alg, LN2, amax);
    if (P.label_dense) {
      const float* __restrict__ y = P.label_dense + row * P.ldl + c0;
      float b = 0.f;
#pragma unroll
      for (int k = 0; k < 32; ++k)
        if (FULL || frag_col(k) < nvalid) b = fmaf(__ldg(y + frag_col(k)), v[k] + off, b);
      st.b += b;
    } else if (P.label_idx) {
      const int64_t lab = P.label_idx[row];
      const int k = (lab >= e0 && lab < e0 + 128 && (FULL || lab - c0 < nvalid)) ? frag_elem((int)(lab - e0), q) : -1;
      if (k >= 0) st.b += frag_get(v, k) + off;
    }
  } else if constexpr (EPI == EPI_KL) {
    float cm = B2K_NEG_HUGE;
#pragma unroll
    for (int k = 0; k < 32; ++k)
      if (FULL || frag_col(k) < nvalid) cm = fmaxf(cm, v[k]);
    const float mn = fmaxf(st.m, cm);
    const float mn2 = mn * LOG2E;
    float acc = 0.f;
#pragma unroll
    for (int k = 0; k < 32; ++k)
      if (FULL || frag_col(k) < nvalid) acc += fast_ex2(fmaf(v[k], LOG2E, -mn2));
    st.s = fmaf(st.s, fast_ex2((st.m - mn) * LOG2E), acc);
    st.m = mn;
    if (P.label_dense) {
      const float* __restrict__ y = P.label_dense + row * P.ldl + c0;
#pragma unroll
      for (int k = 0; k < 32; ++k) {
        if (FULL || frag_col(k) < nvalid) {
          const float yy = __ldg(y + frag_col(k));
          if (yy != 0.f) {
            st.y_sum += yy;
            st.yx = fmaf(yy, v[k], st.yx);
            st.ylogy = fmaf(yy, __logf(yy), st.ylogy);
          }
        }
      }
    } else if (P.label_idx) {
      const int64_t lab = P.label_idx[row];
      const int k = (lab >= e0 && lab < e0 + 128 && (FULL || lab - c0 < nvalid)) ? frag_elem((int)(lab - e0), q) : -1;
      if (k >= 0) { st.y_sum += 1.0f; st.yx += frag_get(v, k); }
    }
  } else if constexpr (EPI == EPI_RANK || EPI == EPI_RANK_EVAL) {
    const float t = epi_row_aux<EPI_RANK>(P, row);
    const float allowed = __fadd_rn(P.atol, fabsf(__fmul_rn(P.rtol, t)));
    const float* __restrict__ f = (EPI == EPI_RANK && P.filter) ? P.filter + row * P.ldf + c0 : nullptr;
    unsigned int gt = 0, cl = 0;
#pragma unroll
    for (int k = 0; k < 32; ++k) {
      if (FULL || frag_col(k) < nvalid) {
        float x = v[k];
        if (f) x = __fsub_rn(x, __ldg(f + frag_col(k)));
        if (isnan(x)) x = -INFINITY;
        const float actual = fabsf(__fsub_rn(x, t));
        const bool close = (x == t) || (isfinite(actual) && actual <= allowed);
        cl += close ? 1u : 0u;
        gt += (!close && x > t) ? 1u : 0u;
      }
    }
    st.greater += gt;
    st.close += cl;
  } else if constexpr (EPI == EPI_STORE) {
    int64_t r = row, cb = 0;
    if (P.n_rows_out > 0 && r >= P.n_rows_out) { r -= P.n_rows_out; cb = P.col_block; }
    const int64_t at = r * P.ldo + cb + c0;
    auto put = [&](float* __restrict__ p) {
      const bool vec = (reinterpret_cast<uintptr_t>(p) & 7) == 0;
#pragma unroll
      for (int j = 0; j < 16; ++j) {
        if (vec && (FULL || 8 * j + 1 < nvalid)) {
          *reinterpret_cast<float2*>(p + 8 * j) = make_float2(v[2 * j], v[2 * j + 1]);
        } else {
          if (FULL || 8 * j < nvalid) p[8 * j] = v[2 * j];
          if (FULL || 8 * j + 1 < nvalid) p[8 * j + 1] = v[2 * j + 1];
        }
      }
    };
    if (P.accumulate_out) {
      float* __restrict__ p = P.out + at;
#pragma unroll
      for (int k = 0; k < 32; ++k)
        if (FULL || frag_col(k) < nvalid) atomicAdd(p + frag_col(k), v[k]);
    } else {
      put(P.out + at);
      for (int g = 0; g < P.n_peers; ++g) put(P.out_peer[g] + at);
    }
  }
}

__device__ __forceinline__ void rank_eval_row(const EpiParams& P, const float (&v)[32], int64_t row, int64_t e0, int64_t m,
                                              int q) {
  const float t = epi_row_aux<EPI_RANK_EVAL>(P, row);
  const int64_t lim = e0 + 128 < m ? e0 + 128 : m;
  const int64_t own = __ldg(P.csr_skip + row);
  if (own >= e0 && own < lim) {
    const int k = frag_elem((int)(own - e0), q);
    if (k >= 0) P.own_score[row] = frag_get(v, k);
  }
  RankFix fix;
#pragma unroll
  for (int list = 0; list < 2; ++list) {
    const int64_t* __restrict__ off = list ? P.csr2_off : P.csr_off;
    const int64_t* __restrict__ col = list ? P.csr2_col : P.csr_col;
    if (!off) continue;
    const int64_t end = __ldg(off + row + 1);
    for (int64_t cur = csr_lower_bound(col, __ldg(off + row), end, e0); cur < end; ++cur) {
      const int64_t cj = __ldg(col + cur);
      if (cj >= lim) break;
      const int k = frag_elem((int)(cj - e0), q);
      if (k >= 0 && cj != own) fix.add(list == 1, frag_get(v, k), t, P.rtol, P.atol);
    }
  }
  fix.commit(P, row);
}

template <int EPI>
__device__ __forceinline__ void epi_row(const EpiParams& P, RowState<EPI>& st, float (&v)[32], int64_t row,
                                        int64_t e0, int64_t m, int q) {
  const int64_t c0 = e0 + 2 * q;
  if constexpr (EPI == EPI_RANK_EVAL) {
    if (e0 + 128 <= m) epi_row_body<EPI, true>(P, st, v, row, e0, c0, 128, q);
    else               epi_row_body<EPI, false>(P, st, v, row, e0, c0, (int)(m - c0), q);
    rank_eval_row(P, v, row, e0, m, q);
    return;
  }
  if constexpr (EPI != EPI_STORE) {
    if (P.csr_off) {
      const int64_t end = __ldg(P.csr_off + row + 1);
      const int64_t lim = e0 + 128 < m ? e0 + 128 : m;
      const int64_t skip = (EPI == EPI_RANK && P.csr_skip) ? __ldg(P.csr_skip + row) : -1;
      for (int64_t cur = csr_lower_bound(P.csr_col, __ldg(P.csr_off + row), end, e0); cur < end; ++cur) {
        const int64_t cj = __ldg(P.csr_col + cur);
        if (cj >= lim) break;
        const int k = frag_elem((int)(cj - e0), q);
        if (k < 0) continue;
        if constexpr (EPI == EPI_RANK) {
          if (cj != skip) {
#pragma unroll
            for (int i = 0; i < 32; ++i)
              if (i == k) v[i] = -INFINITY;
          }
        } else {
          P.csr_out[cur] = frag_get(v, k);
        }
      }
    }
    if constexpr (EPI == EPI_BCE || EPI == EPI_KL) {
      if (P.csr_extra && e0 == 0 && q == 0) P.csr_out[P.csr_nnz + row] = v[0];
    }
  }
  if (e0 + 128 <= m) epi_row_body<EPI, true>(P, st, v, row, e0, c0, 128, q);
  else               epi_row_body<EPI, false>(P, st, v, row, e0, c0, (int)(m - c0), q);
}

typedef CUresult (*EncodeTiledFn)(CUtensorMap*, CUtensorMapDataType, cuuint32_t, void*, const cuuint64_t*,
                                  const cuuint64_t*, const cuuint32_t*, const cuuint32_t*,
                                  CUtensorMapInterleave, CUtensorMapSwizzle, CUtensorMapL2promotion,
                                  CUtensorMapFloatOOBfill);

inline EncodeTiledFn get_encode_fn() {
  static EncodeTiledFn fn = nullptr;
  if (!fn) {
    void* p = nullptr;
    cudaDriverEntryPointQueryResult qres;
    if (cudaGetDriverEntryPoint("cuTensorMapEncodeTiled", &p, cudaEnableDefault, &qres) == cudaSuccess &&
        qres == cudaDriverEntryPointSuccess)
      fn = reinterpret_cast<EncodeTiledFn>(p);
  }
  return fn;
}

inline int make_map(CUtensorMap* map, const float* base, int64_t rows, int64_t cols, int64_t ld, int box_cols,
                    int box_rows) {
  EncodeTiledFn fn = get_encode_fn();
  if (!fn) { set_error("cuTensorMapEncodeTiled not available from the driver"); return B200KGE_ERR_CUDA; }
  cuuint64_t dims[2] = {(cuuint64_t)cols, (cuuint64_t)rows};
  cuuint64_t strides[1] = {(cuuint64_t)ld * 4};
  cuuint32_t box[2] = {(cuuint32_t)box_cols, (cuuint32_t)box_rows};
  cuuint32_t estr[2] = {1, 1};
  CUtensorMapSwizzle sw = (box_cols * 4 == 128) ? CU_TENSOR_MAP_SWIZZLE_128B : CU_TENSOR_MAP_SWIZZLE_64B;
  CUresult r = fn(map, CU_TENSOR_MAP_DATA_TYPE_FLOAT32, 2, const_cast<float*>(base), dims, strides, box, estr,
                  CU_TENSOR_MAP_INTERLEAVE_NONE, sw, CU_TENSOR_MAP_L2_PROMOTION_L2_256B,
                  CU_TENSOR_MAP_FLOAT_OOB_FILL_NONE);
  if (r != CUDA_SUCCESS) {
    set_error("cuTensorMapEncodeTiled failed (%d) rows=%lld cols=%lld ld=%lld", (int)r, (long long)rows,
              (long long)cols, (long long)ld);
    return B200KGE_ERR_CUDA;
  }
  return 0;
}

inline int make_map_f16(CUtensorMap* map, const void* base, int64_t rows, int64_t cols, int64_t ld, int box_rows,
                        int box_cols = 64) {
  EncodeTiledFn fn = get_encode_fn();
  if (!fn) { set_error("cuTensorMapEncodeTiled not available from the driver"); return B200KGE_ERR_CUDA; }
  cuuint64_t dims[2] = {(cuuint64_t)cols, (cuuint64_t)rows};
  cuuint64_t strides[1] = {(cuuint64_t)ld * 2};
  cuuint32_t box[2] = {(cuuint32_t)box_cols, (cuuint32_t)box_rows};
  cuuint32_t estr[2] = {1, 1};
  CUresult r = fn(map, CU_TENSOR_MAP_DATA_TYPE_FLOAT16, 2, const_cast<void*>(base), dims, strides, box, estr,
                  CU_TENSOR_MAP_INTERLEAVE_NONE, box_cols == 64 ? CU_TENSOR_MAP_SWIZZLE_128B : CU_TENSOR_MAP_SWIZZLE_64B,
                  CU_TENSOR_MAP_L2_PROMOTION_L2_256B,
                  CU_TENSOR_MAP_FLOAT_OOB_FILL_NONE);
  if (r != CUDA_SUCCESS) {
    set_error("cuTensorMapEncodeTiled(f16) failed (%d) rows=%lld cols=%lld ld=%lld", (int)r, (long long)rows,
              (long long)cols, (long long)ld);
    return B200KGE_ERR_CUDA;
  }
  return 0;
}

inline int num_sms() {
  static int n = 0;
  if (!n) {
    int dev = 0;
    cudaGetDevice(&dev);
    cudaDeviceGetAttribute(&n, cudaDevAttrMultiProcessorCount, dev);
    if (n <= 0) n = 132;
  }
  return n;
}

}

struct SplitSet {
  const float* src; int64_t ld; const int64_t* idx; int col_off;
  int64_t rows, rows_pad;
  int K, Kp;
  void* hi; void* lo; float* inv_scale;
};
int launch_presplit(const SplitSet& A, const SplitSet& B, cudaStream_t st);
int launch_prep_split_1vsall(int model, const Rows& ent, const Rows& rel, const int64_t* triples, int64_t n,
                             const SplitSet& Qs, const SplitSet& Ts, int64_t* labels2n, unsigned int* ticket,
                             cudaStream_t st, int64_t num_rel = 0);
int launch_pairwise_tc3(int epi_kind, const SplitSet& Q, const SplitSet& T, const EpiParams& P, cudaStream_t st);

int launch_transpose(const float* src, int64_t lds, int64_t R, int64_t C, float* dst, int64_t ldd, cudaStream_t st);
int launch_grad_planes(const float* z, int64_t ldz, int64_t nq, int64_t E, const int64_t* label_idx,
                       const float* label_dense, int64_t ldl, float* row_stat, float offset, float inv_n, void* g_hi, void* g_lo,
                       int64_t Ep, void* gt_hi, void* gt_lo, int64_t Np, float* g_scale, float* gt_scale,
                       cudaStream_t st);
int launch_pair_rowgrad(int pair_op, const float* A, int64_t lda, int64_t ra, const float* B, int64_t ldb, int64_t rb, int K,
                        const float* Wt, int64_t ldwt, float* dA, int64_t ldda, cudaStream_t st);
int launch_grad_dense(const float* z, int64_t ldz, int64_t nq, int64_t E, const int64_t* label_idx, const float* row_stat,
                      float offset, float inv_n, int div_z, float* G, int64_t ldg, cudaStream_t st);
int launch_grad_csr(const float* z, int64_t ldz, int64_t nq, int64_t E, const int64_t* csr_off, const int64_t* csr_col,
                    float a, float b, const float* row_stat, float offset, float inv_n, int div_z, float* G, int64_t ldg,
                    cudaStream_t st);
int launch_div_scores(const float* g, int64_t ldg, const float* z, int64_t ldz, int64_t n, int64_t E, float* W, int64_t ldw,
                      cudaStream_t st);
int launch_row_lse(const float* z, int64_t ldz, int64_t nq, int64_t E, const int64_t* label_idx, float* row_stat,
                   cudaStream_t st);
int launch_unfold_distance(int model, const Rows& ent, const Rows& rel, const int64_t* triples, int64_t n, int dir,
                           const float* dQ, int64_t ldq, float* d_ent, int64_t lde, float* d_rel, int64_t ldr,
                           cudaStream_t st, int64_t num_rel = 0);
int launch_grad_planes_csr(const float* z, int64_t ldz, int64_t nq, int64_t E, const int64_t* csr_off,
                           const int64_t* csr_col, float a, float b, float* row_stat, float offset, float inv_n,
                           void* g_hi, void* g_lo, int64_t Ep, void* gt_hi, void* gt_lo, int64_t Np, float* g_scale,
                           float* gt_scale, cudaStream_t st);
int launch_csr_expand(const int64_t* off, const int64_t* col, int64_t n, int64_t nnz, int extra, const int64_t* q_idx,
                      const int64_t* p_idx, int64_t* qsel, int64_t* psel, int64_t* esel, cudaStream_t st);
int launch_csr_rows(int loss_kind, const int64_t* off, const int64_t* col, const float* zpos, int64_t n, int64_t nnz,
                    const float* fused, const float* zsum, int zsum_chunks, float a, float b, float E, float offset,
                    float* row_loss, cudaStream_t st);
int launch_rows_sum(const float* rows, int64_t n, float scale, float* out, cudaStream_t st);
int launch_row_score_sums(const float* Q, int64_t ldq, int64_t n, const float* T, int64_t ldt, int64_t E, int K,
                          float* scratch, float* zsum, cudaStream_t st);
int launch_ns_backward(int model, float l_norm, const Rows& ent, const Rows& rel, const int64_t* triples, int slot,
                       const int64_t* neg, int64_t n, int64_t K, float offset, float inv_batch, const float* G,
                       int64_t ldg, float* d_ent, int64_t lde, float* d_rel, int64_t ldr, float* dQ, int64_t ldq,
                       cudaStream_t st);
int launch_ns_loss(int loss_kind, const float* scores, int64_t lds, int64_t n, int64_t m, const int64_t* label_idx,
                   float arg, float temperature, float scale, float* part, float* G, int64_t ldg, cudaStream_t st);
int launch_penalty(const Rows& tab, const float* counts, float p, int complex_abs, float scale, float* scratch,
                   size_t scratch_floats, float* out, cudaStream_t st);
int launch_normalize_rows(float* w, int64_t ld, int64_t rows, int dim, float p, cudaStream_t st);
int launch_unfold(int model, const Rows& ent, const Rows& rel, const int64_t* triples, int64_t n, int dir,
                  const float* dQ, int64_t ldq, float* d_ent, int64_t lde, float* d_rel, int64_t ldr, cudaStream_t st,
                  int64_t num_rel = 0);

}
```

Before: 153.2 billion.

## Overlap entity-table fp16 split conversion with the 1vsAll tensor-core sweep

The prep kernel now converts only the first portion of entity rows into fp16 hi/lo planes. Idle producer warps inside the pairwise wgmma kernel convert the remaining rows, staging them through bulk async copies into shared memory. Per-tile ready counters with release/acquire fences gate the TMA loads of late tiles, and the kernel launches cooperatively to guarantee co-residency. The work is rescheduled into q-tile by entity-tile-group sweep units, so table conversion overlaps with matmul work instead of running as a separate serial pass. This adds spin-waiting, extra shared memory and a dependency on correct cross-CTA memory ordering.

```diff
diff --git a/kge_b200/csrc/capi.cu b/kge_b200/csrc/capi.cu
--- a/kge_b200/csrc/capi.cu
+++ b/kge_b200/csrc/capi.cu
@@ -368,6 +368,7 @@
     const int64_t Kp = round_up(D, 64);
     b += 2 * ((size_t)nq * Kp * 2 + 256) + 2 * ((size_t)m * Kp * 2 + 256) + (size_t)(nq + m + 32) * 4 + 512;
   }
+  b += (size_t)(m + 127) / 128 * 4 + 256;
   return b + 4096;
 }
 
@@ -671,17 +672,21 @@
     const bool planes = take_planes(ws, SQ) && take_planes(ws, ST);
     int64_t* lab = (int64_t*)ws.take((size_t)n * 2 * 8);
     uint8_t* scratch = (uint8_t*)ws.take(1024);
-    const int nch = tc_nchunks(nq, m);
+    const TcSweep sw = tc_sweep_plan(nq, m);
+    const int nch = sw.nch;
     const int F = (loss_kind == B200KGE_LOSS_BCE) ? 2 : 5;
     float* part = (float*)ws.take((size_t)nq * nch * F * 4);
-    if (!planes || !lab || !scratch || !part) { set_error("workspace too small"); return B200KGE_ERR_WORKSPACE; }
+    unsigned int* ready = (unsigned int*)ws.take((size_t)sw.e_tiles * 4);
+    if (!planes || !lab || !scratch || !part || !ready) { set_error("workspace too small"); return B200KGE_ERR_WORKSPACE; }
     unsigned int* ticket = reinterpret_cast<unsigned int*>(scratch + 512);
-    if ((rc = launch_prep_split_1vsall(model, E, R, triples, n, SQ, ST, lab, ticket, st, num_rel))) return rc;
+    if ((rc = launch_prep_split_1vsall(model, E, R, triples, n, SQ, ST, sw.r0, ready, sw.e_tiles, lab, ticket, st,
+                                       num_rel)))
+      return rc;
     EpiParams P = empty_epi();
     P.label_idx = lab;
     P.offset = (loss_kind == B200KGE_LOSS_BCE) ? offset : 0.f;
     P.part = part; P.nchunks = nch;
-    if ((rc = launch_pairwise_tc3(epi, SQ, ST, P, st))) return rc;
+    if ((rc = launch_pairwise_tc3(epi, SQ, ST, P, st, ready))) return rc;
     return launch_loss_finalize(loss_kind, part, nch, nq, loss_out, nullptr, scale, 0, scratch, 1, st);
   }
   if (f0.col_off == f1.col_off) {
diff --git a/kge_b200/csrc/pairwise_tc.cu b/kge_b200/csrc/pairwise_tc.cu
--- a/kge_b200/csrc/pairwise_tc.cu
+++ b/kge_b200/csrc/pairwise_tc.cu
@@ -9,12 +9,17 @@
 constexpr int TM = 128;
 constexpr int TN = 128;
 constexpr int NSTAGE = 3;
+constexpr int CONV_ROWS = 4;
 constexpr int STAGE_BYTES = 64 * 1024;
 constexpr int BOX_BYTES = 16 * 1024;
 constexpr int STATE_BYTES = 256 * 4 * (int)sizeof(RowState<EPI_KL>);
 static_assert(sizeof(RowState<EPI_RANK_EVAL>) <= sizeof(RowState<EPI_KL>), "row state slots are sized for KL");
 constexpr int SMEM_BYTES = 1024  + NSTAGE * STAGE_BYTES + 256  + STATE_BYTES;
 static_assert(SMEM_BYTES <= 227 * 1024, "exceeds the H100's 227 KB of shared memory per block");
+constexpr int CONV_BUF = 4096, CONV_SLOTS = 4;
+constexpr int CONV_OFF = NSTAGE * STAGE_BYTES + 256 + STATE_BYTES;
+constexpr int SMEM_SWEEP_BYTES = SMEM_BYTES + 3 * CONV_BUF;
+static_assert(SMEM_SWEEP_BYTES <= 227 * 1024, "exceeds the H100's 227 KB of shared memory per block");
 
 template <int MODE> struct ModeCfg {
   static constexpr bool SPLIT = MODE == MODE_TF32X3 || MODE == MODE_MIXED;
@@ -38,6 +43,11 @@
   const float* q_scale;
   const float* t_scale;
   EpiParams epi;
+  int sweep;
+  int64_t units;
+  int conv_t0;
+  unsigned int* ready;
+  SplitSet conv;
 };
 
 struct Item { int qt, et, k0, k1; };
@@ -86,7 +96,29 @@
   }
 }
 
-template <int EPI, int MODE>
+template <class F, class G>
+__device__ __forceinline__ void for_each_unit(const TcParams& p, F&& f, G&& end) {
+  int64_t li = 0;
+  for (int64_t u = blockIdx.x; u < p.units; u += p.grid) {
+    const int qt = (int)(u % p.q_tiles), gr = (int)(u / p.q_tiles);
+    const int et1 = (gr + 1) * p.sweep < p.e_tiles ? (gr + 1) * p.sweep : p.e_tiles;
+    for (int et = gr * p.sweep; et < et1; ++et, ++li) f(Item{qt, et, 0, p.nk}, li);
+    end(qt, gr);
+  }
+}
+
+__device__ __forceinline__ void wait_tile_ready(const TcParams& p, int et) {
+  const int64_t rows = p.m - (int64_t)et * TN;
+  const unsigned int need = rows < TN ? (unsigned int)rows : (unsigned int)TN;
+  for (uint32_t polls = 0; ptx::ld_relaxed(p.ready + et) < need; ++polls) {
+    if (polls > (1u << 24)) __trap();
+    __nanosleep(64);
+  }
+  ptx::fence_acq_rel_gpu();
+  ptx::fence_proxy_async_global();
+}
+
+template <int EPI, int MODE, bool SWEEP>
 __global__ void __launch_bounds__(ModeCfg<MODE>::NTHREADS, 1)
 pairwise_tc_kernel(const __grid_constant__ CUtensorMap tmQ, const __grid_constant__ CUtensorMap tmT,
                    const __grid_constant__ CUtensorMap tmQl, const __grid_constant__ CUtensorMap tmTl,
@@ -99,6 +131,7 @@
   uint64_t* split = bars + NSTAGE;
   uint64_t* empty = bars + 2 * NSTAGE;
   uint64_t* turn = bars + 3 * NSTAGE;
+  uint64_t* conv_bar = bars + 16;
 
   const int warp = threadIdx.x >> 5, lane = threadIdx.x & 31;
   const int64_t i0 = (int64_t)blockIdx.x * prm.items / prm.grid, i1 = (int64_t)(blockIdx.x + 1) * prm.items / prm.grid;
@@ -117,6 +150,8 @@
     }
     ptx::mbar_init(&turn[0], 1);
     ptx::mbar_init(&turn[1], 1);
+    if constexpr (SWEEP)
+      for (int s = 0; s < 3 * CONV_SLOTS; ++s) ptx::mbar_init(&conv_bar[s], 1);
     ptx::fence_barrier_init();
   }
   __syncthreads();
@@ -125,8 +160,7 @@
     if constexpr (C::PP) ptx::setmaxnreg_dec<40>();
     if (warp == 0 && lane == 0) {
       uint32_t c = 0;
-      for (int64_t i = i0; i < i1; ++i) {
-        const Item it = item_at(prm, i);
+      auto load = [&](const Item& it) {
         for (int kc = it.k0; kc < it.k1; ++kc, ++c) {
           const int s = (int)(c % NSTAGE);
           ptx::mbar_wait_bounded(&empty[s], ((c / NSTAGE) & 1) ^ 1);
@@ -137,6 +171,57 @@
           if constexpr (MODE == MODE_F16X3) {
             ptx::tma_load_2d(sp + 2 * BOX_BYTES, &tmQl, &full[s], kc * C::TK, it.qt * TM);
             ptx::tma_load_2d(sp + 3 * BOX_BYTES, &tmTl, &full[s], kc * C::TK, it.et * TN);
+          }
+        }
+      };
+      if constexpr (SWEEP) {
+        for_each_unit(prm, [&](const Item& it, int64_t) {
+          if (it.et >= prm.conv_t0) wait_tile_ready(prm, it.et);
+          load(it);
+        }, [](int, int) {});
+      } else {
+        for (int64_t i = i0; i < i1; ++i) load(item_at(prm, i));
+      }
+    } else if (warp > 0) {
+      if constexpr (SWEEP) {
+        SplitSet S = prm.conv;
+        const int m = (int)prm.m, base = prm.conv_t0 * TN, W = 3 * prm.grid, w = 3 * (int)blockIdx.x + warp - 1;
+        auto row_of = [&](int j) { return base + CONV_ROWS * (w + (j / CONV_ROWS) * W) + j % CONV_ROWS; };
+        const uint32_t rb = (uint32_t)S.K * 4u;
+        const bool bulk = S.K % 4 == 0 && S.ld % 4 == 0 && S.col_off % 4 == 0 && !S.idx &&
+                          (reinterpret_cast<uintptr_t>(S.src) & 15) == 0;
+        const int nbuf = bulk ? ((int)(CONV_BUF / rb) < CONV_SLOTS ? (int)(CONV_BUF / rb) : CONV_SLOTS) : 0;
+        float* buf = reinterpret_cast<float*>(smem + CONV_OFF + (warp - 1) * CONV_BUF);
+        uint64_t* mb = conv_bar + (warp - 1) * CONV_SLOTS;
+        auto issue = [&](int j) {
+          const int r = row_of(j);
+          if (r < m) {
+            const int sl = j % nbuf;
+            ptx::mbar_arrive_expect_tx(&mb[sl], rb);
+            ptx::bulk_load(buf + sl * (rb / 4), prm.conv.src + (int64_t)r * prm.conv.ld + prm.conv.col_off, rb, &mb[sl]);
+          }
+        };
+        if (bulk && lane == 0)
+          for (int j = 0; j < nbuf - 1; ++j) issue(j);
+        for (int j = 0;; ++j) {
+          const int r = row_of(j);
+          if (r >= m) break;
+          if (bulk) {
+            if (lane == 0) issue(j + nbuf - 1);
+            ptx::mbar_wait_bounded(&mb[j % nbuf], (uint32_t)(j / nbuf) & 1);
+            S.src = buf + (j % nbuf) * (rb / 4);
+            S.ld = 0;
+            S.col_off = 0;
+          }
+          presplit_row<true>(S, r, lane);
+          if (bulk) ptx::fence_proxy_async_smem();
+          const int k = (r - base) % CONV_ROWS;
+          if (k == CONV_ROWS - 1 || r + 1 == m) {
+            ptx::fence_proxy_async_global();
+            __syncwarp();
+            if (lane == 0) ptx::red_release_add(prm.ready + r / TN, (unsigned int)(k + 1));
+          } else {
+            __syncwarp();
           }
         }
       }
@@ -174,11 +259,10 @@
 #pragma unroll
     for (int rr = 0; rr < 2 * C::MH; ++rr) st[256 * rr].init();
     uint32_t c = 0;
-    for (int64_t i = i0; i < i1; ++i) {
-      const Item it = item_at(prm, i);
+    auto tile = [&](const Item& it, int64_t li) {
       const int nkc = it.k1 - it.k0;
-      if (!C::PP || (int)((i - i0) & 1) == g) {
-        const uint32_t k = (uint32_t)((i - i0) >> 1);
+      if (!C::PP || (int)(li & 1) == g) {
+        const uint32_t k = (uint32_t)(li >> 1);
         if (C::PP && (g == 1 || k > 0)) ptx::mbar_wait_bounded(&turn[g], (g == 1 ? k : k - 1) & 1);
         float d[C::MH][64];
 #pragma unroll
@@ -216,7 +300,8 @@
 #pragma unroll
           for (int j = 0; j < 16; ++j) {
             const int64_t col = e0 + 2 * q + 8 * j;
-            const float2 ts = col < prm.m ? __ldg(reinterpret_cast<const float2*>(prm.t_scale + col)) : make_float2(0.f, 0.f);
+            const float2* tsp = reinterpret_cast<const float2*>(prm.t_scale + col);
+            const float2 ts = col < prm.m ? (SWEEP ? __ldca(tsp) : __ldg(tsp)) : make_float2(0.f, 0.f);
 #pragma unroll
             for (int rr = 0; rr < 2 * C::MH; ++rr) {
               float* a = &d[rr >> 1][4 * j + 2 * (rr & 1)];
@@ -242,12 +327,9 @@
         }
       }
       c += nkc;
+    };
+    auto flush = [&](int qt, int j, bool fill) {
       if constexpr (EPI != EPI_STORE) {
-        const bool ends_qt = (i + 1) % prm.e_tiles == 0;
-        if (ends_qt || i + 1 == i1) {
-          const int qt = (int)(i / prm.e_tiles);
-          const int64_t first = (((int64_t)qt * prm.e_tiles + 1) * prm.grid - 1) / prm.items;
-          const int j = (int)(blockIdx.x - first);
           const int h = C::PP ? g : (q >> 1);
           const bool writer = C::PP ? q == 0 : (q & 1) == 0;
 #pragma unroll
@@ -258,7 +340,7 @@
             if (writer && row < prm.nq) {
               epi_flush<EPI>(P, rs, row, 2 * j + h);
               if constexpr (EPI != EPI_RANK && EPI != EPI_RANK_EVAL) {
-                if (ends_qt) {
+                if (fill) {
                   RowState<EPI> z;
                   z.init();
                   for (int jj = j + 1; jj < prm.nsl; ++jj) epi_flush<EPI>(P, z, row, 2 * jj + h);
@@ -266,6 +348,20 @@
               }
             }
             st[256 * rr].init();
+          }
+      }
+    };
+    if constexpr (SWEEP) {
+      for_each_unit(prm, tile, [&](int qt, int gr) { flush(qt, gr, false); });
+    } else {
+      for (int64_t i = i0; i < i1; ++i) {
+        tile(item_at(prm, i), i - i0);
+        if constexpr (EPI != EPI_STORE) {
+          const bool ends_qt = (i + 1) % prm.e_tiles == 0;
+          if (ends_qt || i + 1 == i1) {
+            const int qt = (int)(i / prm.e_tiles);
+            const int64_t first = (((int64_t)qt * prm.e_tiles + 1) * prm.grid - 1) / prm.items;
+            flush(qt, (int)(blockIdx.x - first), ends_qt);
           }
         }
       }
@@ -287,14 +383,40 @@
   prm.nsl = nsl < prm.grid ? (int)nsl : prm.grid;
 }
 
-template <int EPI, int MODE>
+void sweep_schedule(int64_t nq, int64_t m, TcParams& prm) {
+  schedule(nq, m, 1, prm);
+  prm.sweep = (prm.e_tiles + 159) / 160;
+  if (prm.sweep < 2) prm.sweep = 2;
+  const int groups = (prm.e_tiles + prm.sweep - 1) / prm.sweep;
+  prm.units = (int64_t)prm.q_tiles * groups;
+  prm.grid = prm.units < num_sms() ? (int)prm.units : num_sms();
+  prm.nsl = groups;
+  int64_t t0 = (prm.grid + prm.q_tiles - 1) / prm.q_tiles * (int64_t)prm.sweep;
+  const int64_t t38 = ((int64_t)prm.e_tiles * 3 + 7) / 8;
+  if (t0 < t38) t0 = t38;
+  prm.conv_t0 = t0 < prm.e_tiles ? (int)t0 : prm.e_tiles;
+}
+
+template <int EPI, int MODE, bool SWEEP = false>
 int launch_k(const CUtensorMap (&maps)[4], const TcParams& prm, cudaStream_t st) {
-  auto kern = pairwise_tc_kernel<EPI, MODE>;
-  cudaError_t e = cudaFuncSetAttribute(kern, cudaFuncAttributeMaxDynamicSharedMemorySize, SMEM_BYTES);
+  auto kern = pairwise_tc_kernel<EPI, MODE, SWEEP>;
+  constexpr int smem_bytes = SWEEP ? SMEM_SWEEP_BYTES : SMEM_BYTES;
+  cudaError_t e = cudaFuncSetAttribute(kern, cudaFuncAttributeMaxDynamicSharedMemorySize, smem_bytes);
   if (e != cudaSuccess) return check_cuda(e, "cudaFuncSetAttribute(pairwise_tc_kernel)");
+  cudaLaunchAttribute attr;
+  attr.id = cudaLaunchAttributeCooperative;
+  attr.val.cooperative = 1;
+  cudaLaunchConfig_t cfg = {};
+  cfg.gridDim = dim3((unsigned)prm.grid);
+  cfg.blockDim = dim3(ModeCfg<MODE>::NTHREADS);
+  cfg.dynamicSmemBytes = smem_bytes;
+  cfg.stream = st;
+  cfg.attrs = &attr;
+  cfg.numAttrs = (SWEEP && prm.conv_t0 < prm.e_tiles) ? 1 : 0;
   profile_begin(st);
-  kern<<<prm.grid, ModeCfg<MODE>::NTHREADS, SMEM_BYTES, st>>>(maps[0], maps[1], maps[2], maps[3], prm);
+  e = cudaLaunchKernelEx(&cfg, kern, maps[0], maps[1], maps[2], maps[3], prm);
   profile_end(st);
+  if (e != cudaSuccess) return check_cuda(e, "pairwise_tc_kernel launch");
   B2K_LAUNCH_CHECK("pairwise_tc_kernel");
   return 0;
 }
@@ -329,6 +451,13 @@
   TcParams prm;
   schedule(nq, m, 1, prm);
   return 2 * prm.nsl;
+}
+
+TcSweep tc_sweep_plan(int64_t nq, int64_t m) {
+  TcParams prm;
+  sweep_schedule(nq, m, prm);
+  const int64_t r0 = (int64_t)prm.conv_t0 * TN;
+  return TcSweep{r0 < m ? r0 : m, 2 * prm.nsl, prm.e_tiles};
 }
 
 int launch_pairwise_tc(int epi_kind, int passes, const float* Q, int64_t ldq,
@@ -352,11 +481,33 @@
   return launch_mode<MODE_TF32>(epi_kind, maps, prm, st);
 }
 
-int launch_pairwise_tc3(int epi_kind, const SplitSet& Q, const SplitSet& T, const EpiParams& P, cudaStream_t st) {
+int launch_pairwise_tc3(int epi_kind, const SplitSet& Q, const SplitSet& T, const EpiParams& P, cudaStream_t st,
+                        unsigned int* ready) {
   const int64_t nq = Q.rows, m = T.rows;
   if (nq == 0 || m == 0) return 0;
   if (Q.Kp != T.Kp || Q.Kp % 64 != 0) { set_error("operand planes disagree on the padded reduction length"); return B200KGE_ERR_INVALID; }
   TcParams prm;
+  if (ready) {
+    if (P.accumulate_out || (epi_kind != EPI_BCE && epi_kind != EPI_KL)) {
+      set_error("the sweep schedule serves the BCE / KL loss epilogues");
+      return B200KGE_ERR_INVALID;
+    }
+    prm.nq = nq; prm.m = m; prm.nk = Q.Kp / 64; prm.kseg = prm.nk;
+    sweep_schedule(nq, m, prm);
+    prm.q_scale = Q.inv_scale; prm.t_scale = T.inv_scale;
+    prm.ready = ready;
+    prm.conv = T;
+    CUtensorMap maps[4];
+    int rc;
+    if ((rc = tc::make_map_f16(&maps[0], Q.hi, nq, Q.Kp, Q.Kp, TM))) return rc;
+    if ((rc = tc::make_map_f16(&maps[1], T.hi, m, T.Kp, T.Kp, TN))) return rc;
+    if ((rc = tc::make_map_f16(&maps[2], Q.lo, nq, Q.Kp, Q.Kp, TM))) return rc;
+    if ((rc = tc::make_map_f16(&maps[3], T.lo, m, T.Kp, T.Kp, TN))) return rc;
+    prm.epi = P;
+    prm.epi.nchunks = 2 * prm.nsl;
+    return epi_kind == EPI_BCE ? launch_k<EPI_BCE, MODE_F16X3, true>(maps, prm, st)
+                               : launch_k<EPI_KL, MODE_F16X3, true>(maps, prm, st);
+  }
   prm.nq = nq; prm.m = m; prm.nk = Q.Kp / 64;
   prm.kseg = prm.nk;
   if (P.accumulate_out) {
diff --git a/kge_b200/csrc/presplit.cu b/kge_b200/csrc/presplit.cu
--- a/kge_b200/csrc/presplit.cu
+++ b/kge_b200/csrc/presplit.cu
@@ -7,71 +7,6 @@
 namespace {
 
 constexpr int PS_WARPS = 8;
-
-__device__ __forceinline__ void presplit_row(const SplitSet& S, int64_t r, int lane) {
-  if (r >= S.rows) {
-    if (r < S.rows_pad && lane == 0) S.inv_scale[r] = 0.f;
-    return;
-  }
-  const int64_t src_row = S.idx ? S.idx[r] : r;
-  const float* __restrict__ x = S.src + src_row * S.ld + S.col_off;
-  const int K = S.K, Kp = S.Kp;
-  const bool vec = (K % 4 == 0) && ((reinterpret_cast<uintptr_t>(x) & 15) == 0);
-  float amax = 0.f;
-  bool bad = false;
-  if (vec) {
-    for (int k = lane * 4; k < K; k += 128) {
-      const float4 v = __ldg(reinterpret_cast<const float4*>(x + k));
-      amax = fmaxf(amax, fmaxf(fmaxf(fabsf(v.x), fabsf(v.y)), fmaxf(fabsf(v.z), fabsf(v.w))));
-      bad |= !(isfinite(v.x) && isfinite(v.y) && isfinite(v.z) && isfinite(v.w));
-    }
-  } else {
-    for (int k = lane; k < K; k += 32) {
-      const float v = __ldg(x + k);
-      amax = fmaxf(amax, fabsf(v));
-      bad |= !isfinite(v);
-    }
-  }
-#pragma unroll
-  for (int o = 16; o > 0; o >>= 1) amax = fmaxf(amax, __shfl_xor_sync(0xffffffffu, amax, o));
-  bad = __any_sync(0xffffffffu, bad);
-  int e = 13;
-  if (amax > 0.f && !bad) {
-    e = ilogbf(amax);
-    e = e < -60 ? -60 : (e > 60 ? 60 : e);
-  }
-  const float mul = scalbnf(1.f, 13 - e), inv = scalbnf(1.f, e - 13);
-  __half* __restrict__ hi = reinterpret_cast<__half*>(S.hi) + r * Kp;
-  __half* __restrict__ lo = reinterpret_cast<__half*>(S.lo) + r * Kp;
-  if (vec) {
-    for (int k = lane * 4; k < Kp; k += 128) {
-      float4 v = make_float4(0.f, 0.f, 0.f, 0.f);
-      if (k < K) v = __ldg(reinterpret_cast<const float4*>(x + k));
-      const float s[4] = {v.x * mul, v.y * mul, v.z * mul, v.w * mul};
-      __half h[4], l[4];
-#pragma unroll
-      for (int i = 0; i < 4; ++i) {
-        h[i] = __float2half_rn(s[i]);
-        l[i] = __float2half_rn(s[i] - __half2float(h[i]));
-      }
-      uint2 ph, pl;
-      ph.x = (uint32_t)__half_as_ushort(h[0]) | ((uint32_t)__half_as_ushort(h[1]) << 16);
-      ph.y = (uint32_t)__half_as_ushort(h[2]) | ((uint32_t)__half_as_ushort(h[3]) << 16);
-      pl.x = (uint32_t)__half_as_ushort(l[0]) | ((uint32_t)__half_as_ushort(l[1]) << 16);
-      pl.y = (uint32_t)__half_as_ushort(l[2]) | ((uint32_t)__half_as_ushort(l[3]) << 16);
-      *reinterpret_cast<uint2*>(hi + k) = ph;
-      *reinterpret_cast<uint2*>(lo + k) = pl;
-    }
-  } else {
-    for (int k = lane; k < Kp; k += 32) {
-      const float s = (k < K) ? __ldg(x + k) * mul : 0.f;
-      const __half h = __float2half_rn(s);
-      hi[k] = h;
-      lo[k] = __float2half_rn(s - __half2float(h));
-    }
-  }
-  if (lane == 0) S.inv_scale[r] = inv;
-}
 
 __global__ void __launch_bounds__(PS_WARPS * 32)
 presplit_kernel(const SplitSet A, const SplitSet B, const int blocks_a) {
@@ -134,13 +69,15 @@
 template <int MODEL, bool RECIP>
 __global__ void __launch_bounds__(PQ_THREADS)
 prep_split_1vsall_kernel(Rows ent, Rows rel, const int64_t* __restrict__ tri, int64_t n, const SplitSet Qs,
-                         const SplitSet Ts, int64_t* __restrict__ labels2n, unsigned int* ticket, int K,
-                         int64_t num_rel) {
+                         const SplitSet Ts, int64_t t_rows, unsigned int* __restrict__ ready, int n_ready,
+                         int64_t* __restrict__ labels2n, unsigned int* ticket, int K, int64_t num_rel) {
   extern __shared__ float sh[];
   const int64_t b = blockIdx.x;
   const int warp = threadIdx.x >> 5, lane = threadIdx.x & 31;
+  for (int64_t t = b * PQ_THREADS + threadIdx.x; t < n_ready; t += (int64_t)gridDim.x * PQ_THREADS) ready[t] = 0u;
   if (b >= 2 * n) {
-    presplit_row(Ts, (b - 2 * n) * PS_WARPS + warp, lane);
+    const int64_t r = (b - 2 * n) * PS_WARPS + warp;
+    presplit_row(Ts, r < t_rows ? r : Ts.rows + (r - t_rows), lane);
     return;
   }
   __shared__ float red[PS_WARPS];
@@ -209,18 +146,19 @@
 }
 
 int launch_prep_split_1vsall(int model, const Rows& ent, const Rows& rel, const int64_t* triples, int64_t n,
-                             const SplitSet& Qs, const SplitSet& Ts, int64_t* labels2n, unsigned int* ticket,
-                             cudaStream_t st, int64_t num_rel) {
+                             const SplitSet& Qs, const SplitSet& Ts, int64_t t_rows, unsigned int* ready, int n_ready,
+                             int64_t* labels2n, unsigned int* ticket, cudaStream_t st, int64_t num_rel) {
   if (n == 0) return 0;
   const int D = ent.dim;
   const int K = (model == B200KGE_CP) ? D / 2 : D;
-  const int64_t tb = (Ts.rows_pad + PS_WARPS - 1) / PS_WARPS;
+  if (t_rows < 0 || t_rows > Ts.rows) { set_error("bad table row count for the fused prologue"); return B200KGE_ERR_INVALID; }
+  const int64_t tb = (t_rows + (Ts.rows_pad - Ts.rows) + PS_WARPS - 1) / PS_WARPS;
   if (2 * n + tb >= (1ll << 31)) { set_error("too many rows for the fused prologue"); return B200KGE_ERR_INVALID; }
   const size_t smem = ((size_t)Qs.Kp + (model == B200KGE_RESCAL ? D : 0)) * sizeof(float);
   if (smem > 48 * 1024) { set_error("embedding too wide for the fused prologue"); return B200KGE_ERR_UNSUPPORTED; }
   dim3 grid((unsigned)(2 * n + tb)), block(PQ_THREADS);
-#define B2K_PS(M) case M: prep_split_1vsall_kernel<M, false><<<grid, block, smem, st>>>(ent, rel, triples, n, Qs, Ts, labels2n, ticket, K, 0); break;
-#define B2K_PS_R(M) case M: prep_split_1vsall_kernel<M, true><<<grid, block, smem, st>>>(ent, rel, triples, n, Qs, Ts, labels2n, ticket, K, num_rel); break;
+#define B2K_PS(M) case M: prep_split_1vsall_kernel<M, false><<<grid, block, smem, st>>>(ent, rel, triples, n, Qs, Ts, t_rows, ready, n_ready, labels2n, ticket, K, 0); break;
+#define B2K_PS_R(M) case M: prep_split_1vsall_kernel<M, true><<<grid, block, smem, st>>>(ent, rel, triples, n, Qs, Ts, t_rows, ready, n_ready, labels2n, ticket, K, num_rel); break;
   if (num_rel > 0) {
     switch (model) {
       B2K_PS_R(B200KGE_COMPLEX) B2K_PS_R(B200KGE_DISTMULT) B2K_PS_R(B200KGE_SIMPLE) B2K_PS_R(B200KGE_CP)
diff --git a/kge_b200/csrc/ptx.cuh b/kge_b200/csrc/ptx.cuh
--- a/kge_b200/csrc/ptx.cuh
+++ b/kge_b200/csrc/ptx.cuh
@@ -50,6 +50,22 @@
 __device__ __forceinline__ void fence_proxy_async_smem() {
   asm volatile("fence.proxy.async.shared::cta;" ::: "memory");
 }
+__device__ __forceinline__ void fence_proxy_async_global() {
+  asm volatile("fence.proxy.async.global;" ::: "memory");
+}
+__device__ __forceinline__ void bulk_load(void* dst, const void* src, uint32_t bytes, uint64_t* bar) {
+  asm volatile("cp.async.bulk.shared::cluster.global.mbarrier::complete_tx::bytes [%0], [%1], %2, [%3];"
+               ::"r"(smem_u32(dst)), "l"(src), "r"(bytes), "r"(smem_u32(bar)) : "memory");
+}
+__device__ __forceinline__ void red_release_add(unsigned int* p, unsigned int v) {
+  asm volatile("red.release.gpu.global.add.u32 [%0], %1;" ::"l"(p), "r"(v) : "memory");
+}
+__device__ __forceinline__ unsigned int ld_relaxed(const unsigned int* p) {
+  unsigned int v;
+  asm volatile("ld.relaxed.gpu.global.u32 %0, [%1];" : "=r"(v) : "l"(p) : "memory");
+  return v;
+}
+__device__ __forceinline__ void fence_acq_rel_gpu() { asm volatile("fence.acq_rel.gpu;" ::: "memory"); }
 __device__ __forceinline__ void bar_sync(uint32_t id, uint32_t nthreads) {
   asm volatile("bar.sync %0, %1;" ::"r"(id), "r"(nthreads) : "memory");
 }
diff --git a/kge_b200/csrc/tc_common.cuh b/kge_b200/csrc/tc_common.cuh
--- a/kge_b200/csrc/tc_common.cuh
+++ b/kge_b200/csrc/tc_common.cuh
@@ -1,5 +1,6 @@
 #pragma once
 #include <cuda.h>
+#include <cuda_fp16.h>
 #include <cstdlib>
 #include "common.cuh"
 #include "ptx.cuh"
@@ -355,11 +356,94 @@
   int K, Kp;
   void* hi; void* lo; float* inv_scale;
 };
+
+template <bool LEAN = false>
+__device__ __forceinline__ void presplit_row(const SplitSet& S, int64_t r, int lane) {
+  if (r >= S.rows) {
+    if (r < S.rows_pad && lane == 0) S.inv_scale[r] = 0.f;
+    return;
+  }
+  const int64_t src_row = S.idx ? S.idx[r] : r;
+  const float* __restrict__ x = S.src + src_row * S.ld + S.col_off;
+  const int K = S.K, Kp = S.Kp;
+  const bool vec = (K % 4 == 0) && ((reinterpret_cast<uintptr_t>(x) & 15) == 0);
+  float amax = 0.f;
+  bool bad = false;
+  auto ld4 = [&](int k) { return LEAN ? *reinterpret_cast<const float4*>(x + k) : __ldg(reinterpret_cast<const float4*>(x + k)); };
+  auto amax4 = [&](int k) {
+    const float4 v = ld4(k);
+    amax = fmaxf(amax, fmaxf(fmaxf(fabsf(v.x), fabsf(v.y)), fmaxf(fabsf(v.z), fabsf(v.w))));
+    bad |= !(isfinite(v.x) && isfinite(v.y) && isfinite(v.z) && isfinite(v.w));
+  };
+  if (vec) {
+    if constexpr (LEAN) {
+#pragma unroll 1
+      for (int k = lane * 4; k < K; k += 128) amax4(k);
+    } else {
+      for (int k = lane * 4; k < K; k += 128) amax4(k);
+    }
+  } else {
+    for (int k = lane; k < K; k += 32) {
+      const float v = __ldg(x + k);
+      amax = fmaxf(amax, fabsf(v));
+      bad |= !isfinite(v);
+    }
+  }
+#pragma unroll
+  for (int o = 16; o > 0; o >>= 1) amax = fmaxf(amax, __shfl_xor_sync(0xffffffffu, amax, o));
+  bad = __any_sync(0xffffffffu, bad);
+  int e = 13;
+  if (amax > 0.f && !bad) {
+    e = ilogbf(amax);
+    e = e < -60 ? -60 : (e > 60 ? 60 : e);
+  }
+  const float mul = scalbnf(1.f, 13 - e), inv = scalbnf(1.f, e - 13);
+  __half* __restrict__ hi = reinterpret_cast<__half*>(S.hi) + r * Kp;
+  __half* __restrict__ lo = reinterpret_cast<__half*>(S.lo) + r * Kp;
+  auto convert4 = [&](int k) {
+      float4 v = make_float4(0.f, 0.f, 0.f, 0.f);
+      if (k < K) v = ld4(k);
+      const float s[4] = {v.x * mul, v.y * mul, v.z * mul, v.w * mul};
+      __half h[4], l[4];
+#pragma unroll
+      for (int i = 0; i < 4; ++i) {
+        h[i] = __float2half_rn(s[i]);
+        l[i] = __float2half_rn(s[i] - __half2float(h[i]));
+      }
+      uint2 ph, pl;
+      ph.x = (uint32_t)__half_as_ushort(h[0]) | ((uint32_t)__half_as_ushort(h[1]) << 16);
+      ph.y = (uint32_t)__half_as_ushort(h[2]) | ((uint32_t)__half_as_ushort(h[3]) << 16);
+      pl.x = (uint32_t)__half_as_ushort(l[0]) | ((uint32_t)__half_as_ushort(l[1]) << 16);
+      pl.y = (uint32_t)__half_as_ushort(l[2]) | ((uint32_t)__half_as_ushort(l[3]) << 16);
+      *reinterpret_cast<uint2*>(hi + k) = ph;
+      *reinterpret_cast<uint2*>(lo + k) = pl;
+  };
+  if (vec) {
+    if constexpr (LEAN) {
+#pragma unroll 1
+      for (int k = lane * 4; k < Kp; k += 128) convert4(k);
+    } else {
+      for (int k = lane * 4; k < Kp; k += 128) convert4(k);
+    }
+  } else {
+    for (int k = lane; k < Kp; k += 32) {
+      const float s = (k < K) ? __ldg(x + k) * mul : 0.f;
+      const __half h = __float2half_rn(s);
+      hi[k] = h;
+      lo[k] = __float2half_rn(s - __half2float(h));
+    }
+  }
+  if (lane == 0) S.inv_scale[r] = inv;
+}
+
 int launch_presplit(const SplitSet& A, const SplitSet& B, cudaStream_t st);
+struct TcSweep { int64_t r0; int nch; int e_tiles; };
+TcSweep tc_sweep_plan(int64_t nq, int64_t m);
 int launch_prep_split_1vsall(int model, const Rows& ent, const Rows& rel, const int64_t* triples, int64_t n,
-                             const SplitSet& Qs, const SplitSet& Ts, int64_t* labels2n, unsigned int* ticket,
-                             cudaStream_t st, int64_t num_rel = 0);
-int launch_pairwise_tc3(int epi_kind, const SplitSet& Q, const SplitSet& T, const EpiParams& P, cudaStream_t st);
+                             const SplitSet& Qs, const SplitSet& Ts, int64_t t_rows, unsigned int* ready, int n_ready,
+                             int64_t* labels2n, unsigned int* ticket, cudaStream_t st, int64_t num_rel = 0);
+int launch_pairwise_tc3(int epi_kind, const SplitSet& Q, const SplitSet& T, const EpiParams& P, cudaStream_t st,
+                        unsigned int* ready = nullptr);
 
 int launch_transpose(const float* src, int64_t lds, int64_t R, int64_t C, float* dst, int64_t ldd, cudaStream_t st);
 int launch_grad_planes(const float* z, int64_t ldz, int64_t nq, int64_t E, const int64_t* label_idx,
```

Measured after the change: 159.7 billion, median of 6. 1.04x the previous value.
